# AllenNeuralDynamics/aind-exaspim-neuron-segmentation

Hardware: AMD Instinct MI355X
Metric: affinity voxels/sec on 96^3 patches over a 1024x1024x1024 volume, 1 MI355X (higher is better)
Workload: dtype fp16; 1 GPU; 1024x1024x1024 uint16 volume, 96^3 patches, overlap 32, trim 8, batch 16, fp16 (IEEE half) storage of activations and weights / fp32 accumulate (BASELINE.json configs[2]); streams=1

## Files before the change

aind_exaspim_neuron_segmentation_amd/_native.py:

```python

import ctypes
import os

_HERE = os.path.dirname(os.path.abspath(__file__))
LIB_PATH = os.path.join(_HERE, "csrc", "libexaspim_affinity.so")

DT_F32, DT_BF16, DT_F16 = 0, 1, 2
DT_BF16X3 = 3
VOX_U8, VOX_U16, VOX_I16, VOX_F32, VOX_F64 = 0, 1, 2, 3, 4
IN_F32, IN_PADDED_F32, IN_PADDED_SPLIT_F16, IN_PADDED_SPLIT_BF16 = 0, 1, 2, 3
UP_CONVT = 0x100
OPT_SEPARATE_POOL, OPT_SEPARATE_DEEP_POOLS, OPT_PLAIN_UPSAMPLE, OPT_FIRST_PER_GROUP = 1, 2, 4, 8
OPT_UPSAMPLE_PER_THREAD = 16
OPT_PER_PATCH_ENCODER = 32
OPT_SEPARATE_HEAD = 64
OPT_ROW_SEPARATE_BORDERS = 256
OPT_CARRY_MAIN_ONLY = 512
OPT_CARRY_NO_ROWS = 2048
AFF_F32, AFF_F16 = 0, 1

DTYPE_CODES = {
    "fp32": DT_F32, "float32": DT_F32, "f32": DT_F32,
    "bf16": DT_BF16, "bfloat16": DT_BF16,
    "fp16": DT_F16, "float16": DT_F16, "f16": DT_F16,
    "bf16x3": DT_BF16X3,
}


class Block(ctypes.Structure):

    _fields_ = [
        ("dims", ctypes.c_int32 * 3),
        ("origin", ctypes.c_int32 * 3),
        ("global_", ctypes.c_int32 * 3),
    ]

    @classmethod
    def make(cls, dims, origin=None, global_shape=None):
        origin = (0, 0, 0) if origin is None else origin
        global_shape = dims if global_shape is None else global_shape
        b = cls()
        b.dims[:] = [int(v) for v in dims]
        b.origin[:] = [int(v) for v in origin]
        b.global_[:] = [int(v) for v in global_shape]
        return b


class Window(ctypes.Structure):

    _fields_ = [
        ("patch", ctypes.c_int32 * 3),
        ("overlap", ctypes.c_int32 * 3),
        ("trim", ctypes.c_int32),
    ]

    @classmethod
    def make(cls, patch, overlap, trim):
        w = cls()
        w.patch[:] = [int(v) for v in patch]
        w.overlap[:] = [int(v) for v in overlap]
        w.trim = int(trim)
        return w


class ComponentsStreamDesc(ctypes.Structure):

    _fields_ = [
        ("dims", ctypes.c_int32 * 3),
        ("channels", ctypes.c_int32),
        ("threshold", ctypes.c_float),
        ("capacity", ctypes.c_int32),
        ("min_size", ctypes.c_int64),
        ("next_z", ctypes.c_int32),
        ("reserved", ctypes.c_int32),
        ("id_parent_dev", ctypes.c_void_p),
        ("id_count_dev", ctypes.c_void_p),
        ("table_dev", ctypes.c_void_p),
        ("state_dev", ctypes.c_void_p),
        ("seam_ids_dev", ctypes.c_void_p),
        ("seam_bits_dev", ctypes.c_void_p),
    ]


class RegionGraphStreamDesc(ctypes.Structure):

    _fields_ = [
        ("dims", ctypes.c_int32 * 3),
        ("id_capacity", ctypes.c_int32),
        ("edge_capacity", ctypes.c_int64),
        ("next_z", ctypes.c_int32),
        ("reserved", ctypes.c_int32),
        ("keys_dev", ctypes.c_void_p),
        ("counts_dev", ctypes.c_void_p),
        ("sums_dev", ctypes.c_void_p),
        ("sizes_by_id_dev", ctypes.c_void_p),
        ("seam_ids_dev", ctypes.c_void_p),
        ("seam_q_dev", ctypes.c_void_p),
        ("state_dev", ctypes.c_void_p),
    ]


class UNetCarry(ctypes.Structure):

    _fields_ = [
        ("own_skip", ctypes.c_void_p),
        ("own_pool", ctypes.c_void_p),
        ("in_z", ctypes.c_int32 * 2),
        ("out_skip", ctypes.c_void_p),
        ("out_pool", ctypes.c_void_p),
        ("out_z", ctypes.c_int32 * 2),
        ("out_shift", ctypes.c_int32),
        ("reserved", ctypes.c_int32),
    ]


class UNetCarry1(ctypes.Structure):

    _fields_ = [
        ("own_mid1", ctypes.c_void_p),
        ("own_skip1", ctypes.c_void_p),
        ("own_pool2", ctypes.c_void_p),
        ("in_z", ctypes.c_int32 * 2),
        ("out_mid1", ctypes.c_void_p),
        ("out_skip1", ctypes.c_void_p),
        ("out_pool2", ctypes.c_void_p),
        ("out_z", ctypes.c_int32 * 2),
        ("out_shift", ctypes.c_int32),
        ("reserved", ctypes.c_int32),
    ]


class UNetCarryY(ctypes.Structure):

    _fields_ = [
        ("in_y", ctypes.c_int32 * 2),
        ("out_skip_y", ctypes.c_void_p),
        ("out_pool_y", ctypes.c_void_p),
        ("out_skip_d", ctypes.c_void_p),
        ("out_pool_d", ctypes.c_void_p),
        ("out_y", ctypes.c_int32 * 2),
        ("out_shift_y", ctypes.c_int32),
        ("reserved", ctypes.c_int32),
        ("encoder_event", ctypes.c_void_p),
    ]


_lib = None

_I32x5 = ctypes.c_int32 * 5
_I32x3 = ctypes.c_int32 * 3
_vp = ctypes.c_void_p
_sz = ctypes.c_size_t
_i32 = ctypes.c_int32

SIGNATURES = {
    "exaspim_abi_version": (_i32, []),
    "exaspim_last_error": (ctypes.c_char_p, []),
    "exaspim_unet_param_count": (_sz, [_I32x5, _i32, _i32]),
    "exaspim_unet_packed_bytes": (_sz, [_I32x5, _i32, _i32]),
    "exaspim_unet_pack_weights": (_i32, [_I32x5, _i32, _i32, _vp, _sz, _vp, _sz]),
    "exaspim_unet_create": (_i32, [_I32x5, _i32, _i32, _i32, _vp, _sz, ctypes.POINTER(_vp)]),
    "exaspim_unet_destroy": (None, [_vp]),
    "exaspim_unet_workspace_bytes": (_sz, [_vp, _i32, _i32, _i32, _i32]),
    "exaspim_unet_forward": (_i32, [_vp, _vp, _vp, _i32, _i32, _i32, _i32, _i32, _vp, _sz, _vp]),
    "exaspim_unet_forward_trimmed": (
        _i32, [_vp, _vp, _vp, _i32, _i32, _i32, _i32, _i32, _i32, _vp, _sz, _vp]
    ),
    "exaspim_unet_input_layout": (_i32, [_vp]),
    "exaspim_unet_forward_prepared": (
        _i32, [_vp, _vp, _vp, _i32, _i32, _i32, _i32, _i32, _i32, _vp, _sz, _vp]),
    "exaspim_unet_forward_prepared_row": (
# ... 139 lines not shown
```

aind_exaspim_neuron_segmentation_amd/csrc/common.h:

```cpp
#pragma once

#include <hip/hip_runtime.h>

#include <cstdarg>
#include <cstddef>
#include <cstdint>
#include <cstdio>

#include "../../include/exaspim_affinity.h"

namespace exaspim {

void set_error(const char* fmt, ...);
const char* get_error();

#define EXA_CHECK_ARG(cond, ...)                 \
    do {                                         \
        if (!(cond)) {                           \
            ::exaspim::set_error(__VA_ARGS__);   \
            return EXASPIM_E_INVALID;            \
        }                                        \
    } while (0)

#define EXA_CHECK_HIP(expr)                                                  \
// ... 30 lines not shown
    asm volatile("s_nop 1");
    __builtin_amdgcn_sched_barrier(0);
}

__device__ __forceinline__ float sat_f16(float v) {
    return v != v ? v : __builtin_amdgcn_fmed3f(v, -65504.f, 65504.f);
}

__device__ __forceinline__ float max_nan(float a, float b) {
    return (a != a || b != b) ? __uint_as_float(0x7fc00000u) : fmaxf(a, b);
}
__device__ __forceinline__ uint4 max_nan4(const uint4& a, const uint4& b) {
    return make_uint4(__float_as_uint(max_nan(__uint_as_float(a.x), __uint_as_float(b.x))),
                      __float_as_uint(max_nan(__uint_as_float(a.y), __uint_as_float(b.y))),
                      __float_as_uint(max_nan(__uint_as_float(a.z), __uint_as_float(b.z))),
                      __float_as_uint(max_nan(__uint_as_float(a.w), __uint_as_float(b.w))));
}
typedef short s16x2 __attribute__((ext_vector_type(2)));
typedef unsigned short u16x2 __attribute__((ext_vector_type(2)));
__device__ __forceinline__ unsigned key16x2(unsigned x) {
    const s16x2 m = __builtin_bit_cast(s16x2, x) >> (short)15;
    return x ^ (__builtin_bit_cast(unsigned, m) & 0x7fff7fffu);
}
template <unsigned INF16>
__device__ __forceinline__ unsigned okey16x2(unsigned x) {
    const u16x2 mag = __builtin_bit_cast(u16x2, x & 0x7fff7fffu);
    const auto nan = mag > (u16x2){(unsigned short)INF16, (unsigned short)INF16};
    return key16x2(x & ~(__builtin_bit_cast(unsigned, nan) & 0x80008000u));
}
__device__ __forceinline__ unsigned maxkey16x2(unsigned ka, unsigned kb) {
    return __builtin_bit_cast(
        unsigned, __builtin_elementwise_max(__builtin_bit_cast(s16x2, ka), __builtin_bit_cast(s16x2, kb)));
}
__device__ __forceinline__ uint4 key16(const uint4& v) {
    return make_uint4(key16x2(v.x), key16x2(v.y), key16x2(v.z), key16x2(v.w));
}
template <unsigned INF16>
__device__ __forceinline__ uint4 okey16(const uint4& v) {
    return make_uint4(okey16x2<INF16>(v.x), okey16x2<INF16>(v.y), okey16x2<INF16>(v.z), okey16x2<INF16>(v.w));
}
__device__ __forceinline__ uint4 maxkey16(const uint4& a, const uint4& b) {
    return make_uint4(maxkey16x2(a.x, b.x), maxkey16x2(a.y, b.y), maxkey16x2(a.z, b.z), maxkey16x2(a.w, b.w));
}

template <int N>
__device__ __forceinline__ float head_dot(float acc, const float (&f)[N], const float* w) {
#pragma clang fp contract(off)
#pragma unroll
    for (int j = 0; j < N; ++j) acc = fmaf(f[j], w[j], acc);
    return acc;
}
__device__ __forceinline__ float head_activation(float r, int apply_sigmoid) {
#pragma clang fp contract(off)
    if (apply_sigmoid) r = 1.f / (1.f + expf(-r));
    return r;
}

constexpr int kChannelPad = 32;
constexpr int kNumMfmaConvs = 17;

inline int pad_channels(int c) { return (c + kChannelPad - 1) / kChannelPad * kChannelPad; }
inline size_t align_up(size_t v, size_t a) { return (v + a - 1) / a * a; }
struct MergeBound {
    uint64_t m;
    bool merge_all;
};
inline MergeBound merge_bound(float threshold) {
    const double md = __builtin_rint((1.0 - (double)threshold) * 16777216.0);
    return MergeBound{md < 0.0 ? 0 : md > 16777216.0 ? 16777216ull : (uint64_t)md, md < 0.0};
}
inline int storage_dtype(int dtype) { return dtype == EXASPIM_DT_BF16X3 ? EXASPIM_DT_F32 : dtype; }
inline int dtype_size(int dtype) { return storage_dtype(dtype) == EXASPIM_DT_F32 ? 4 : 2; }

struct ConvLayer {
    int ca_real = 0, cb_real = 0;
    int ca = 0, cb = 0;
    int cout_real = 0, cout = 0;
    size_t w_off = 0;
    size_t b_off = 0;
    size_t p_off = 0;
};

struct ConvTLayer {
    int cin_real = 0, cin = 0;
    int cout_real = 0, cout = 0;
    size_t w_off = 0;
    size_t b_off = 0;
    size_t p_off = 0;
};

struct UNetPlan {
    int channels[5] = {0, 0, 0, 0, 0};
    int out_channels = 0;
    int dtype = 0;
    bool convt = false;
    ConvTLayer up[4];
    int c0 = 0, c0p = 0;
    size_t first_p_off = 0;
    size_t first_w_off = 0;
    size_t first_b_off = 0;
    ConvLayer conv[kNumMfmaConvs];
    size_t head_p_off = 0;
    size_t head_w_off = 0;
    size_t head_b_off = 0;
    size_t packed_bytes = 0;
    size_t n_params = 0;
};

bool make_plan(const int32_t channels[5], int32_t out_channels, int32_t dtype,
               UNetPlan* plan);

int pack_weights(const UNetPlan& plan, const float* params, void* packed_host);

struct ConvArgs {
    const void* src_a;
    const void* src_b;
    int ca, cb;
    const void* weights;
    void* carry_dst = nullptr;
    void* carry_pool_dst = nullptr;
    const float* bias;
    void* dst;
    int cout;
    int n, d, h, w;
    float slope;
    const float* head_w = nullptr;
    const float* head_b = nullptr;
    float* head_out = nullptr;
    int head_oc = 0;
    int head_sigmoid = 0;
    int org[3] = {0, 0, 0};
    int ext[3] = {0, 0, 0};
    void* pool_dst = nullptr;
    int row_stride = 0;
    unsigned short in_z0 = 0, in_z1 = 0;
    float* partial = nullptr;
    size_t partial_patch_bytes = 0;
    int ksplit = 1;
    unsigned char out_z0 = 0, out_z1 = 0;
    unsigned short out_shift = 0;
#ifdef EXASPIM_TRACE
    unsigned long long* trace = nullptr;
#endif
};

struct ConvCarryY {
    void* y_dst = nullptr;
    void* y_pool_dst = nullptr;
    void* d_dst = nullptr;
    void* d_pool_dst = nullptr;
    unsigned short in_y0 = 0, in_y1 = 0;
    unsigned short out_y0 = 0, out_y1 = 0;
    unsigned short out_shift_y = 0;
};
inline bool conv_has_carry_y(const ConvCarryY& y) {
    return y.y_dst || y.y_pool_dst || y.d_dst || y.d_pool_dst || y.in_y0 || y.in_y1 || y.out_y0 || y.out_y1 || y.out_shift_y;
}

struct ConvLaunchRecord {
    const char* config = "";
    int ksplit = 0;
    bool row = false;
    bool carry_y = false;
    bool carry = false;
};
ConvLaunchRecord& last_conv_launch();
const char*& last_layer_kernel();

int launch_conv3x3x3(int dtype, const ConvArgs& a, hipStream_t stream);
int launch_conv3x3x3_thin(int dtype, const ConvArgs& a, hipStream_t stream);
int conv_zcol_main_extent(int ext, int axis);
bool conv_can_fuse_head(int cout, int w, int head_oc, int dtype = EXASPIM_DT_F32);
int launch_conv3x3x3_x3_head(const ConvArgs& a, hipStream_t stream);
bool conv_x3_can_fuse_head(int cout, int w, int head_oc);
bool conv_can_fuse_pool(int dtype, int cout, int d, int h, int w);
bool conv_row_mode_ok(int dtype, int cout, int n, int w, int row_stride, bool fused_pool_whole_patch);
constexpr int kRowStageMain = 1, kRowStageThin = 2, kRowStagePool = 4;
constexpr int kRowStagesAll = kRowStageMain | kRowStageThin | kRowStagePool;
constexpr int kRowStageBorders = 8;
constexpr int kRowStagesFused = kRowStageMain | kRowStageBorders;
constexpr int kRowStageBordersCarry = 16;
constexpr int kRowStagesCarry = kRowStageMain | kRowStageBordersCarry;
int launch_conv3x3x3_row(int dtype, const ConvArgs& a, int stages, hipStream_t stream, const ConvCarryY* y = nullptr);
int conv_zcol_tile_depth(int d);
int conv_row_borders_tile_depth(int d);
constexpr int kCarryT14TZ = 4;
int conv_carry_t14_tile_depth(int dtype, const ConvArgs& a);
void carry1_span_of_tiles(int tz, int d, int shift_z, int32_t out[2]);
#ifndef EXASPIM_TRACE
static_assert(sizeof(ConvArgs) == 184, "ConvArgs: the carry fields fill padding, the argument block keeps its size");
#endif

int launch_conv_first(int dtype, const float* x, float* xpad, const float* w, const float* bias,
                      void* dst, int n, int d, int h, int wd, int c0p, float slope,
                      hipStream_t stream, bool first_no_strips = false, int skip_z0 = 0, int skip_z1 = 0);
void conv_first_skip_planes(int d, int in_z0, int in_z1, int32_t out[2]);
int launch_convt2(int dtype, const void* src, const void* weights, const float* bias, void* dst,
                  int n, int d, int h, int w, int cin, int cout, hipStream_t stream);
int launch_maxpool2(int dtype, const void* src, void* dst, int n, int d, int h, int w,
                    int c, hipStream_t stream);
int launch_maxpool2_xcols(int dtype, const void* src, void* dst, int n, int d, int h, int w,
                          int c, int ox0, int ox1, hipStream_t stream);
int launch_upsample2(int dtype, const void* src, void* dst, int n, int d, int h, int w,
                     int c, int margin, hipStream_t stream, bool plain_kernel = false, bool per_thread = false,
                     const int* margin_hi = nullptr);
int launch_absmax(int dtype, const void* src, size_t bytes, float* out, hipStream_t stream);
int launch_head(int dtype, const void* src, const float* w, const float* bias,
                float* out, int n, int d, int h, int wd, int c0p, int out_channels,
                int apply_sigmoid, hipStream_t stream);
int launch_dbf_pass(int axis, const int32_t* labels, const int32_t* in, int32_t* out, const int32_t dims[3],
                    int black_border, hipStream_t stream);
constexpr int kFillHolesPasses = 6;
int launch_fill_holes_passes(const int32_t* labels, const int32_t dims[3], int32_t* out, int64_t* counts,
                             void* workspace, int first, int last, hipStream_t stream);

}
```

aind_exaspim_neuron_segmentation_amd/csrc/conv3d.hip:

```cpp

#include <cstdlib>

#include "common.h"
#include "conv_device.h"
#include "conv_t14.h"
#include "conv_x3.h"
#include "conv_zcol.h"

namespace exaspim {

#ifdef EXASPIM_TRACE
int g_variant = 0;
#endif

ConvLaunchRecord& last_conv_launch() {
    static thread_local ConvLaunchRecord rec;
    return rec;
}

static int resident_workgroups(int per_cu) {
    static int cus = 0;
    if (cus == 0) {
        int dev = 0, n = 0;
        if (hipGetDevice(&dev) != hipSuccess ||
            hipDeviceGetAttribute(&n, hipDeviceAttributeMultiprocessorCount, dev) != hipSuccess || n <= 0)
            n = 256;
        cus = n;
    }
    return cus * per_cu;
}

static inline int cdiv(int a, int b) { return (a + b - 1) / b; }

struct TileGrid {
    int tz, ty, tx;
    long long blocks;
};
static int tile_grid(const ConvArgs& a, int TZ, int TY, int TX, int ex, int n, TileGrid& g) {
    g.tz = cdiv(a.ext[0], TZ), g.ty = cdiv(a.ext[1], TY), g.tx = cdiv(ex, TX);
    g.blocks = (long long)g.tz * g.ty * g.tx * n;
    if (g.blocks <= 0 || g.blocks > 0x7fffffffLL) {
        set_error("conv: grid of %lld blocks out of range", g.blocks);
        return EXASPIM_E_INVALID;
    }
    return EXASPIM_OK;
}

static int choose_ksplit(const ConvArgs& a, const TileGrid& g, int slices, int units) {
    const bool whole = a.ext[0] == a.d && a.ext[1] == a.h && a.ext[2] == a.w;
    constexpr int kNominalBatch = 16;
    const long long wgs = (long long)g.tz * g.ty * g.tx * kNominalBatch * slices;
    if (!a.partial || !whole || wgs * 2 > resident_workgroups(2)) return 1;
    int ks = (int)(resident_workgroups(2) / wgs);
    if (ks > 4) ks = 4;
    if (ks > units) ks = units;
    const size_t patch_vox = (size_t)a.d * a.h * a.w;
    while (ks > 1 && (size_t)ks * patch_vox * a.cout * sizeof(float) > a.partial_patch_bytes) --ks;
    return ks;
}

static bool conv_has_carry(const ConvArgs& a) {
    return a.carry_dst || a.carry_pool_dst || a.in_z0 || a.in_z1 || a.out_z0 || a.out_z1;
}

template <typename Tag, int TZ, int TY, int TX, int MINW, int D, int HEAD = 0, bool POOL = false>
static int launch_zpipe(const ConvArgs& a, hipStream_t stream) {
    const bool row = POOL && HEAD == 0 && Tag::kG == 8 && a.row_stride > 0;
    TileGrid g;
    if (int rc = row ? tile_grid(a, TZ, TY, TX, a.n * a.row_stride + a.w - a.row_stride, 1, g)
                     : tile_grid(a, TZ, TY, TX, a.ext[2], a.n, g))
        return rc;
    const bool carry = row && conv_has_carry(a);
    if (carry) {
        g.tz -= (a.in_z1 - a.in_z0) / TZ;
        g.blocks = (long long)g.tz * g.ty * g.tx;
    }
    const int tz = g.tz, ty = g.ty, tx = g.tx;
    const long long blocks = g.blocks;
    const int slices = a.cout / 32;
    long long wgs = resident_workgroups(MINW) / slices / 8 * 8;
    if (wgs < 8) wgs = 8;
    if (wgs > blocks) wgs = blocks;
#ifdef EXASPIM_TRACE
    if (g_variant >= 10 && g_variant < 20) wgs = blocks;
    if (const char* e = getenv("EXASPIM_TRACE_WGS_PER_CU")) wgs = resident_workgroups(1) * (long long)atoi(e) / slices / 8 * 8;
#endif
    dim3 grid((unsigned)wgs, slices);
    last_conv_launch() = {__PRETTY_FUNCTION__, 1};
    if constexpr (POOL && HEAD == 0 && Tag::kG == 8) {
        if (carry) {
            last_conv_launch().carry = true;
            conv3x3x3_zpipe_rowz<Tag, TZ, TY, TX, MINW, D><<<grid, TY * TX * 2, 0, stream>>>(a, tz, ty, tx);
            EXA_CHECK_HIP(hipGetLastError());
            return EXASPIM_OK;
        }
        if (row) {
            last_conv_launch().row = true;
            conv3x3x3_zpipe_row<Tag, TZ, TY, TX, MINW, D><<<grid, TY * TX * 2, 0, stream>>>(a, tz, ty, tx);
            EXA_CHECK_HIP(hipGetLastError());
            return EXASPIM_OK;
        }
    }
    conv3x3x3_zpipe<Tag, TZ, TY, TX, MINW, D, HEAD, POOL><<<grid, TY * TX * 2, 0, stream>>>(a, tz, ty, tx);
    EXA_CHECK_HIP(hipGetLastError());
    return EXASPIM_OK;
}

template <typename Tag, int TZ>
static int launch_zpipe_rowzy(const ConvArgs& a, const ConvCarryY& y, hipStream_t stream) {
    constexpr int TY = 8, TX = 16, MINW = 2, D = 4;
    TileGrid g;
    if (int rc = tile_grid(a, TZ, TY, TX, a.n * a.row_stride + a.w - a.row_stride, 1, g)) return rc;
    g.tz -= (a.in_z1 - a.in_z0) / TZ;
    g.ty -= (y.in_y1 - y.in_y0) / TY;
    g.blocks = (long long)g.tz * g.ty * g.tx;
    const int slices = a.cout / 32;
    long long wgs = resident_workgroups(MINW) / slices / 8 * 8;
    if (wgs < 8) wgs = 8;
    if (wgs > g.blocks) wgs = g.blocks;
    dim3 grid((unsigned)wgs, slices);
    last_conv_launch() = {__PRETTY_FUNCTION__, 1};
    last_conv_launch().carry = true;
    last_conv_launch().carry_y = true;
    conv3x3x3_zpipe_rowzy<Tag, TZ, TY, TX, MINW, D><<<grid, TY * TX * 2, 0, stream>>>(a, y, g.tz, g.ty, g.tx);
    EXA_CHECK_HIP(hipGetLastError());
    return EXASPIM_OK;
}


template <typename Tag, int TZ, int TY, int TX, int WAVES_M, int WAVES_N, int MT, int NT, int MINW, int PD = 3,
          bool ZORD = false, bool POOL = false>
static int launch_cfg(const ConvArgs& a, hipStream_t stream) {
    constexpr int NWG = WAVES_N * NT * 32;
    if (a.cout % NWG != 0) {
        set_error("conv: cout %d not a multiple of the %d-channel tile", a.cout, NWG);
        return EXASPIM_E_INVALID;
    }
    TileGrid g;
    if (int rc = tile_grid(a, TZ, TY, TX, a.ext[2], a.n, g)) return rc;
    ConvArgs b = a;
    b.ksplit = a.head_out ? 1 : choose_ksplit(a, g, a.cout / NWG, (a.ca + a.cb) / (2 * Tag::kG));
    constexpr bool kCarryCfg = Tag::kG == 8 && TZ == kCarryT14TZ && TY == 8 && TX == 16 && WAVES_M == 4 && WAVES_N == 1 &&
                               MT == 4 && NT == 2 && MINW == 2 && PD == 3 && !ZORD;
    const bool carry = conv_has_carry(a);
    if (carry) {
        EXA_CHECK_ARG(kCarryCfg && b.ksplit == 1, "conv: this launch has no carried planes (tile configuration%s)",
                      b.ksplit > 1 ? ", split-K" : "");
        g.tz -= (a.in_z1 - a.in_z0) / TZ;
        g.blocks = (long long)g.tz * g.ty * g.tx * a.n;
    }
    const int tz = g.tz, ty = g.ty, tx = g.tx;
    const size_t nvox_all = (size_t)a.n * a.d * a.h * a.w;
    dim3 grid((unsigned)g.blocks, a.cout / NWG, b.ksplit);
    last_conv_launch() = {__PRETTY_FUNCTION__, b.ksplit};
    if constexpr (kCarryCfg) {
        if (carry) {
            last_conv_launch().carry = true;
            conv3x3x3_t14_carry<Tag, TZ, TY, TX, WAVES_M, WAVES_N, MT, NT, MINW, PD, POOL>
                <<<grid, WAVES_M * WAVES_N * 64, 0, stream>>>(b, tz, ty, tx);
            EXA_CHECK_HIP(hipGetLastError());
            return EXASPIM_OK;
        }
    }
    if (POOL && b.ksplit > 1) {
        b.pool_dst = nullptr;
        conv3x3x3_t14<Tag, TZ, TY, TX, WAVES_M, WAVES_N, MT, NT, MINW, PD, ZORD, false>
            <<<grid, WAVES_M * WAVES_N * 64, 0, stream>>>(b, tz, ty, tx);
    } else {
        conv3x3x3_t14<Tag, TZ, TY, TX, WAVES_M, WAVES_N, MT, NT, MINW, PD, ZORD, POOL>
            <<<grid, WAVES_M * WAVES_N * 64, 0, stream>>>(b, tz, ty, tx);
    }
    EXA_CHECK_HIP(hipGetLastError());
    if (b.ksplit > 1) {
        const size_t items = nvox_all * (a.cout / 4);
        splitk_reduce_kernel<Tag><<<(unsigned)((items + 255) / 256), 256, 0, stream>>>(
            a.partial, a.bias, a.dst, nvox_all, (size_t)a.d * a.h * a.w, a.cout, b.ksplit, a.slope);
        EXA_CHECK_HIP(hipGetLastError());
        if (POOL)
            return launch_maxpool2(Tag::kCode, a.dst, a.pool_dst, a.n, a.d, a.h, a.w, a.cout, stream);
    }
    return EXASPIM_OK;
}

template <typename Tag> struct ES_of { static constexpr int value = 16 / Tag::kG; };

template <typename Tag, int TZ, int TY, int TX, int WAVES_M, int WAVES_N, int MT, int NT, int MINW>
static int launch_cfg_pool(const ConvArgs& a, hipStream_t stream) {
    if constexpr (ES_of<Tag>::value == 2) {
        if (a.pool_dst)
            return launch_cfg<Tag, TZ, TY, TX, WAVES_M, WAVES_N, MT, NT, MINW, 3, false, true>(a, stream);
    }
    return launch_cfg<Tag, TZ, TY, TX, WAVES_M, WAVES_N, MT, NT, MINW>(a, stream);
}

template <typename Tag, int TZ, int D>
static int launch_zpipe_head(const ConvArgs& a, hipStream_t stream) {
    if (a.head_out && a.cout == 32) {
        switch (a.head_oc) {
            case 1: return launch_zpipe<Tag, TZ, 8, 16, 2, D, 1>(a, stream);
            case 2: return launch_zpipe<Tag, TZ, 8, 16, 2, D, 2>(a, stream);
            case 3: return launch_zpipe<Tag, TZ, 8, 16, 2, D, 3>(a, stream);
            case 4: return launch_zpipe<Tag, TZ, 8, 16, 2, D, 4>(a, stream);
        }
    }
    if (a.pool_dst) return launch_zpipe<Tag, TZ, 8, 16, 2, D, 0, true>(a, stream);
    return launch_zpipe<Tag, TZ, 8, 16, 2, D>(a, stream);
}

template <typename Tag, int TZ>
static int launch_zpipe_d(const ConvArgs& a, hipStream_t stream) {
#ifdef EXASPIM_TRACE
    if (g_variant % 10 == 3) return launch_zpipe_head<Tag, TZ, 3>(a, stream);
    if (g_variant % 10 == 5) return launch_zpipe_head<Tag, TZ, 5>(a, stream);
#endif
    return launch_zpipe_head<Tag, TZ, 4>(a, stream);
}

template <typename Tag>
static int launch_typed(const ConvArgs& a, hipStream_t stream) {
    if (a.w >= 16 && a.w % 16 == 0) {
#ifdef EXASPIM_TRACE
        if (g_variant >= 20) return launch_zpipe_d<Tag, 6>(a, stream);
#endif
        if (a.cout % 64 != 0) {
            if (a.head_out && a.cout == 32 && a.ext[0] % 6 != 0 && a.ext[0] % kHeadTZ == 0) {
                switch (a.head_oc) {
                    case 1: return launch_zpipe<Tag, kHeadTZ, 8, 16, 2, 4, 1>(a, stream);
                    case 2: return launch_zpipe<Tag, kHeadTZ, 8, 16, 2, 4, 2>(a, stream);
                    case 3: return launch_zpipe<Tag, kHeadTZ, 8, 16, 2, 4, 3>(a, stream);
                    case 4: return launch_zpipe<Tag, kHeadTZ, 8, 16, 2, 4, 4>(a, stream);
                }
            }
            if (conv_zcol_tile_depth(a.d) == 6) return launch_zpipe_d<Tag, 6>(a, stream);
            return launch_zpipe_d<Tag, 4>(a, stream);
        }
        if (a.pool_dst) return launch_cfg_pool<Tag, 4, 8, 16, 4, 1, 4, 2, 2>(a, stream);
        return launch_cfg<Tag, 4, 8, 16, 4, 1, 4, 2, 2>(a, stream);
    }
    if (a.w > 12) {
        if (a.cout % 64 == 0) return launch_cfg_pool<Tag, 4, 4, 24, 4, 1, 3, 2, 2>(a, stream);
        return launch_cfg_pool<Tag, 4, 4, 24, 4, 1, 3, 1, 2>(a, stream);
    }
    if (a.w > 6) {
        if (a.cout % 256 == 0) return launch_cfg_pool<Tag, 4, 4, 12, 2, 1, 3, 1, 2>(a, stream);
        if (a.cout % 128 == 0) return launch_cfg_pool<Tag, 4, 4, 12, 2, 2, 3, 2, 2>(a, stream);
        if (a.cout % 64 == 0) return launch_cfg_pool<Tag, 4, 4, 12, 2, 2, 3, 1, 2>(a, stream);
        return launch_cfg_pool<Tag, 4, 4, 12, 2, 1, 3, 1, 2>(a, stream);
    }
    return launch_cfg<Tag, 6, 6, 6, 4, 1, 2, 1, 2>(a, stream);
}

template <int TZ, int TY, int TX, int WAVES_M, int WAVES_N, int MT, int NT, int MINW, int PD>
static int launch_x3(const ConvArgs& a, hipStream_t stream) {
    constexpr int NWG = WAVES_N * NT * 32;
    if (a.cout % NWG != 0) {
        set_error("conv: cout %d not a multiple of the %d-channel tile", a.cout, NWG);
        return EXASPIM_E_INVALID;
    }
    TileGrid g;
    if (int rc = tile_grid(a, TZ, TY, TX, a.ext[2], a.n, g)) return rc;
    const int tz = g.tz, ty = g.ty, tx = g.tx;
    ConvArgs b = a;
    b.ksplit = choose_ksplit(a, g, a.cout / NWG, (a.ca + a.cb) / 16);
    const size_t patch_vox_all = (size_t)a.d * a.h * a.w;
    const size_t nvox_all = (size_t)a.n * patch_vox_all;
    dim3 grid((unsigned)g.blocks, a.cout / NWG, b.ksplit);
    last_conv_launch() = {__PRETTY_FUNCTION__, b.ksplit};
    conv3x3x3_x3<TZ, TY, TX, WAVES_M, WAVES_N, MT, NT, MINW, PD>
        <<<grid, WAVES_M * WAVES_N * 64, 0, stream>>>(b, tz, ty, tx);
    EXA_CHECK_HIP(hipGetLastError());
    if (b.ksplit > 1) {
        const size_t items = nvox_all * (a.cout / 4);
        splitk_reduce_kernel<F32Tag><<<(unsigned)((items + 255) / 256), 256, 0, stream>>>(
            a.partial, a.bias, a.dst, nvox_all, patch_vox_all, a.cout, b.ksplit, a.slope);
        EXA_CHECK_HIP(hipGetLastError());
    }
    return EXASPIM_OK;
}

static int launch_typed_x3(const ConvArgs& a, hipStream_t stream) {
    if (a.w >= 16 && a.w % 16 == 0) {
        if (a.cout % 64 == 0) return launch_x3<2, 8, 16, 4, 1, 2, 2, 2, 3>(a, stream);
        return launch_x3<4, 8, 16, 4, 1, 4, 1, 2, 3>(a, stream);
    }
    if (a.w > 12) {
        if (a.cout % 64 == 0) return launch_x3<4, 4, 24, 4, 1, 3, 2, 2, 1>(a, stream);
        return launch_x3<4, 4, 24, 4, 1, 3, 1, 2, 3>(a, stream);
    }
    if (a.w > 6) {
        if (a.cout % 256 == 0) return launch_x3<4, 4, 12, 2, 1, 3, 1, 2, 3>(a, stream);
        if (a.cout % 128 == 0) return launch_x3<4, 4, 12, 2, 2, 3, 2, 2, 2>(a, stream);
        if (a.cout % 64 == 0) return launch_x3<4, 4, 12, 2, 2, 3, 1, 2, 3>(a, stream);
        return launch_x3<4, 4, 12, 2, 1, 3, 1, 2, 3>(a, stream);
    }
    return launch_x3<6, 6, 6, 4, 1, 2, 1, 2, 3>(a, stream);
}

static int launch_thin_typed_x3(const ConvArgs& a, hipStream_t stream) {
    if (a.ext[1] <= a.ext[2]) return launch_x3<8, 2, 16, 4, 1, 2, 1, 2, 3>(a, stream);
    return launch_x3<8, 16, 2, 4, 1, 2, 1, 2, 3>(a, stream);
}

template <int HEAD>
static int launch_x3_head(const ConvArgs& a, hipStream_t stream) {
    TileGrid g;
    if (int rc = tile_grid(a, kX3HeadTZ, kX3HeadTY, kX3HeadTX, a.ext[2], a.n, g)) return rc;
    last_conv_launch() = {__PRETTY_FUNCTION__, 1};
    conv3x3x3_x3_head<HEAD><<<dim3((unsigned)g.blocks, 1, 1), 256, 0, stream>>>(a, g.tz, g.ty, g.tx);
    EXA_CHECK_HIP(hipGetLastError());
    return EXASPIM_OK;
}

bool conv_can_fuse_pool(int dtype, int cout, int d, int h, int w) {
    if (d % 2 != 0 || h % 2 != 0 || w % 2 != 0) return false;
    if (dtype == EXASPIM_DT_BF16X3) return false;
    if (cout % 64 != 0 && w >= 16 && w % 16 == 0) return true;
    return dtype != EXASPIM_DT_F32 && w > 6;
}

static bool head_shape_ok(int cout, int w, int head_oc) {
    return cout == 32 && w >= 16 && w % 16 == 0 && head_oc >= 1 && head_oc <= 4;
}
bool conv_can_fuse_head(int cout, int w, int head_oc, int dtype) {
    return dtype != EXASPIM_DT_BF16X3 && head_shape_ok(cout, w, head_oc);
}
bool conv_x3_can_fuse_head(int cout, int w, int head_oc) { return head_shape_ok(cout, w, head_oc); }

static int resolve_region(ConvArgs& a) {
    const int dims[3] = {a.d, a.h, a.w};
    for (int i = 0; i < 3; ++i) {
        if (a.ext[i] == 0 && a.org[i] == 0) a.ext[i] = dims[i];
        EXA_CHECK_ARG(a.org[i] >= 0 && a.ext[i] > 0 && a.org[i] + a.ext[i] <= dims[i],
                      "conv: region [%d, %d) outside axis %d of a %dx%dx%d patch", a.org[i],
                      a.org[i] + a.ext[i], i, a.d, a.h, a.w);
    }
    return EXASPIM_OK;
}

int conv_zcol_tile_depth(int d) { return d % 6 == 0 ? 6 : 4; }

int conv_carry_t14_tile_depth(int dtype, const ConvArgs& a) {
    if (dtype_size(dtype) != 2 || dtype == EXASPIM_DT_BF16X3 || a.head_out || a.row_stride != 0) return 0;
    if (!(a.w >= 16 && a.w % 16 == 0 && a.cout % 64 == 0 && a.d % kCarryT14TZ == 0)) return 0;
    ConvArgs b = a;
    for (int i = 0; i < 3; ++i) b.org[i] = b.ext[i] = 0;
    if (resolve_region(b) != EXASPIM_OK) return 0;
    TileGrid g;
    if (tile_grid(b, kCarryT14TZ, 8, 16, b.ext[2], b.n, g) != EXASPIM_OK) return 0;
    return choose_ksplit(b, g, b.cout / 64, (b.ca + b.cb) / 16) == 1 ? kCarryT14TZ : 0;
}

int conv_zcol_main_extent(int ext, int axis) {
    const int tile = axis == 1 ? 8 : 16;
    const int rem = ext % tile;
    return (axis != 0 && ext > tile && rem >= 1 && rem <= 4) ? ext - rem : ext;
}

bool conv_row_mode_ok(int dtype, int cout, int n, int w, int row_stride, bool fused_pool_whole_patch) {
    const int o = w - row_stride;
    return dtype_size(dtype) == 2 && fused_pool_whole_patch && cout % 64 != 0 &&
           w % 16 == 0 && n >= 2 && row_stride > 0 && o > 0 && o % 32 == 0 && row_stride >= o;
}

static int check_row_args(int dtype, const ConvArgs& a) {
    const bool whole = a.ext[0] == a.d && a.ext[1] == a.h && a.ext[2] == a.w;
    EXA_CHECK_ARG(conv_row_mode_ok(dtype, a.cout, a.n, a.w, a.row_stride,
                                   a.pool_dst && !a.head_out && whole &&
                                       conv_can_fuse_pool(dtype, a.cout, a.d, a.h, a.w)),
                  "conv: row mode needs a 16-bit fused-pool z-column layer, whole patches, n >= 2 and "
                  "an overlap that is a multiple of 32 and at most the stride (w %d, stride %d, n %d)",
                  a.w, a.row_stride, a.n);
    const int tzd = conv_zcol_tile_depth(a.d);
    EXA_CHECK_ARG(a.in_z0 <= a.in_z1 && a.in_z0 % 2 == 0 && a.in_z1 % 2 == 0 && a.in_z0 % tzd == 0 && a.in_z1 % tzd == 0 &&
                      (a.in_z0 == a.in_z1 || (a.in_z0 >= 2 && a.in_z1 <= a.d - 2)),
                  "conv: carry in [%d, %d) must be whole %d-plane tiles with even bounds inside [2, %d)", (int)a.in_z0,
                  (int)a.in_z1, tzd, a.d - 2);
    const bool out = a.carry_dst || a.carry_pool_dst || a.out_z0 || a.out_z1;
    EXA_CHECK_ARG(!out || (a.carry_dst && a.carry_pool_dst && a.out_z0 < a.out_z1 && a.out_z0 % 2 == 0 && a.out_z1 % 2 == 0 &&
                           a.out_z0 >= 2 && a.out_z1 <= a.d - 2 && a.out_shift > 0 && a.out_shift % 2 == 0 &&
                           (int)a.out_z0 - a.out_shift >= 2),
                  "conv: carry out [%d, %d) shifted by %d needs both targets, even bounds and source and target planes "
                  "inside [2, %d)", (int)a.out_z0, (int)a.out_z1, a.out_shift, a.d - 2);
    return EXASPIM_OK;
}

static int check_row_y_args(const ConvArgs& a, const ConvCarryY& y) {
    constexpr int TY = 8;
    EXA_CHECK_ARG(y.in_y0 <= y.in_y1 && y.in_y0 % TY == 0 && y.in_y1 % TY == 0 &&
                      (y.in_y0 == y.in_y1 || (y.in_y0 >= 2 && y.in_y1 <= a.h - 2)),
                  "conv: y carry in [%d, %d) must be whole %d-row tiles inside [2, %d)", (int)y.in_y0, (int)y.in_y1, TY,
                  a.h - 2);
    const bool out = y.y_dst || y.y_pool_dst || y.d_dst || y.d_pool_dst || y.out_y0 || y.out_y1 || y.out_shift_y;
    EXA_CHECK_ARG(!out || (y.y_dst && y.y_pool_dst && y.out_y0 < y.out_y1 && y.out_y0 % 2 == 0 && y.out_y1 % 2 == 0 &&
                           y.out_y0 >= 2 && y.out_y1 <= a.h - 2 && y.out_shift_y > 0 && y.out_shift_y % 2 == 0 &&
                           (int)y.out_y0 - y.out_shift_y >= 2),
                  "conv: y carry out [%d, %d) shifted by %d needs both targets, even bounds and source and target rows "
                  "inside [2, %d)", (int)y.out_y0, (int)y.out_y1, (int)y.out_shift_y, a.h - 2);
    EXA_CHECK_ARG(!out || y.in_y0 == y.in_y1 || y.out_y0 >= y.in_y1 || y.out_y1 <= y.in_y0,
                  "conv: y carry out [%d, %d) overlaps the rows carried in, [%d, %d)", (int)y.out_y0, (int)y.out_y1,
                  (int)y.in_y0, (int)y.in_y1);
    EXA_CHECK_ARG(!y.d_dst == !y.d_pool_dst && (!y.d_dst || (out && a.carry_dst)),
                  "conv: the diagonal carry out needs both targets and both the z and the y carry out");
    EXA_CHECK_ARG(!y.d_dst || a.in_z0 == a.in_z1 || a.out_z0 >= a.in_z1 || a.out_z1 <= a.in_z0,
                  "conv: carry out [%d, %d) overlaps the planes carried in, [%d, %d)", (int)a.out_z0, (int)a.out_z1,
                  (int)a.in_z0, (int)a.in_z1);
    return EXASPIM_OK;
}

static int check_carry_args(int dtype, const ConvArgs& a, bool whole) {
    const int tzd = conv_carry_t14_tile_depth(dtype, a);
    EXA_CHECK_ARG(tzd > 0 && whole,
                  "conv: carried planes need row mode or a whole-patch 16-bit 64-cout-slice layer on 16-wide rows "
                  "that is not split (%dx%dx%d, cout %d)", a.d, a.h, a.w, a.cout);
    EXA_CHECK_ARG(a.in_z0 <= a.in_z1 && a.in_z0 % 2 == 0 && a.in_z1 % 2 == 0 && a.in_z0 % tzd == 0 && a.in_z1 % tzd == 0 &&
                      (a.in_z0 == a.in_z1 || (a.in_z0 >= 2 && a.in_z1 <= a.d - 2)),
                  "conv: carry in [%d, %d) must be whole %d-plane tiles with even bounds inside [2, %d)", (int)a.in_z0,
                  (int)a.in_z1, tzd, a.d - 2);
    const bool out = a.carry_dst || a.carry_pool_dst || a.out_z0 || a.out_z1;
    EXA_CHECK_ARG(!out || (a.carry_dst && !a.carry_pool_dst == !a.pool_dst && a.out_z0 < a.out_z1 && a.out_z0 % 2 == 0 &&
                           a.out_z1 % 2 == 0 && a.out_z0 >= 2 && a.out_z1 <= a.d - 2 && a.out_shift > 0 &&
                           a.out_shift % 2 == 0 && (int)a.out_z0 - a.out_shift >= 2),
                  "conv: carry out [%d, %d) shifted by %d needs a target (a pooled one exactly with a fused max-pool), "
                  "even bounds and source and target planes inside [2, %d)", (int)a.out_z0, (int)a.out_z1, a.out_shift,
                  a.d - 2);
    return EXASPIM_OK;
}

enum : unsigned { kCheckPadded = 1, kCheckEmpty = 2, kCheckSlope = 4, kCheckPatchBytes = 8, kCheckAll = 15 };
static int check_conv_args(int dtype, const ConvArgs& a, unsigned checks) {
    const int kc = dtype == EXASPIM_DT_F32 ? 8 : 16;
    EXA_CHECK_ARG(!(checks & kCheckPadded) || (a.ca % kc == 0 && a.cb % kc == 0 && a.cout % 32 == 0 && a.ca > 0),
                  "conv: channels (%d,%d)->%d not padded", a.ca, a.cb, a.cout);
    EXA_CHECK_ARG(!(checks & kCheckEmpty) || (a.n > 0 && a.d > 0 && a.h > 0 && a.w > 0), "conv: empty input");
    EXA_CHECK_ARG(!(checks & kCheckSlope) || (a.slope >= 0.f && a.slope <= 1.f),
                  "conv: LeakyReLU slope %g outside [0, 1]", a.slope);
    const unsigned long long rec = (unsigned long long)a.d * a.h * a.w * (a.ca > a.cb ? a.ca : a.cb) * dtype_size(dtype);
    EXA_CHECK_ARG(!(checks & kCheckPatchBytes) || rec < 0x80000000ULL,
                  "conv: one patch of one source is %llu bytes (>= 2 GiB)", rec);
    return EXASPIM_OK;
}

int launch_conv3x3x3(int dtype, const ConvArgs& a_in, hipStream_t stream) {
    ConvArgs a = a_in;
    if (int rc = check_conv_args(dtype, a, kCheckAll)) return rc;
    if (int rc = resolve_region(a)) return rc;
    const bool whole = a.ext[0] == a.d && a.ext[1] == a.h && a.ext[2] == a.w;
    EXA_CHECK_ARG(!a.pool_dst || (conv_can_fuse_pool(dtype, a.cout, a.d, a.h, a.w) && !a.head_out && whole),
                  "conv: fused max-pool needs an even, untrimmed patch (16-bit modes: wider than 6 voxels; "
                  "float32: a 32-cout-slice layer)");
    EXA_CHECK_ARG(!a.head_out || conv_can_fuse_head(a.cout, a.w, a.head_oc, dtype),
                  "conv: fused head needs cout 32, w %% 16 == 0, 1..4 outputs (and not bf16x3)");
    if (a.row_stride > 0) {
        if (int rc = check_row_args(dtype, a)) return rc;
    } else if (conv_has_carry(a)) {
        if (int rc = check_carry_args(dtype, a, whole)) return rc;
    }
    switch (dtype) {
        case EXASPIM_DT_F32: return launch_typed<F32Tag>(a, stream);
        case EXASPIM_DT_BF16: return launch_typed<BF16Tag>(a, stream);
        case EXASPIM_DT_F16: return launch_typed<F16Tag>(a, stream);
        case EXASPIM_DT_BF16X3: return launch_typed_x3(a, stream);
    }
    set_error("conv: unknown dtype %d", dtype);
    return EXASPIM_E_INVALID;
}

int launch_conv3x3x3_x3_head(const ConvArgs& a_in, hipStream_t stream) {
    ConvArgs a = a_in;
    if (int rc = check_conv_args(EXASPIM_DT_BF16X3, a, kCheckAll)) return rc;
    EXA_CHECK_ARG(conv_x3_can_fuse_head(a.cout, a.w, a.head_oc),
                  "conv: bf16x3 fused head needs cout 32, w %% 16 == 0 and 1..4 outputs (cout %d, w %d, %d outputs)",
                  a.cout, a.w, a.head_oc);
    EXA_CHECK_ARG(a.head_out && a.head_w && a.head_b, "conv: bf16x3 fused head: NULL head pointer");
    EXA_CHECK_ARG(!a.pool_dst && a.row_stride == 0, "conv: bf16x3 fused head has no fused max-pool or row mode");
    if (int rc = resolve_region(a)) return rc;
    a.partial = nullptr;
    a.ksplit = 1;
    switch (a.head_oc) {
        case 1: return launch_x3_head<1>(a, stream);
        case 2: return launch_x3_head<2>(a, stream);
        case 3: return launch_x3_head<3>(a, stream);
        default: return launch_x3_head<4>(a, stream);
    }
}

template <typename Tag>
static int launch_thin_typed(const ConvArgs& a, hipStream_t stream) {
    const int ez = a.ext[0];
    auto planes = [&](int tz) { return (ez + tz - 1) / tz * tz; };
    if (a.ext[1] <= a.ext[2]) {
        const float c4 = planes(4) * 1.00f, c8 = planes(8) * 0.76f, c12 = planes(12) * 0.66f;
        if (c12 <= c8 && c12 <= c4) return launch_cfg<Tag, 12, 2, 16, 4, 1, 3, 1, 3, 3, true>(a, stream);
        if (c8 <= c4) return launch_cfg<Tag, 8, 2, 16, 4, 1, 2, 1, 4, 3, true>(a, stream);
        return launch_cfg<Tag, 4, 2, 16, 4, 1, 1, 1, 4, 3, true>(a, stream);
    }
    if (planes(8) * 0.78f <= planes(4) * 1.00f) return launch_cfg<Tag, 8, 16, 2, 4, 1, 2, 1, 4, 3, true>(a, stream);
    return launch_cfg<Tag, 4, 16, 2, 4, 1, 1, 1, 4, 3, true>(a, stream);
}

int launch_conv3x3x3_thin(int dtype, const ConvArgs& a_in, hipStream_t stream) {
    ConvArgs a = a_in;
    if (int rc = check_conv_args(dtype, a, kCheckPadded | kCheckEmpty)) return rc;
    EXA_CHECK_ARG(!a.pool_dst && !a.head_out && a.row_stride == 0 && !conv_has_carry(a),
                  "conv: thin tiles have no fused pool, head, row mode or carried planes");
    if (int rc = resolve_region(a)) return rc;
    a.partial = nullptr;
    switch (dtype) {
        case EXASPIM_DT_F32: return launch_thin_typed<F32Tag>(a, stream);
        case EXASPIM_DT_BF16: return launch_thin_typed<BF16Tag>(a, stream);
        case EXASPIM_DT_F16: return launch_thin_typed<F16Tag>(a, stream);
        case EXASPIM_DT_BF16X3: return launch_thin_typed_x3(a, stream);
    }
    set_error("conv: unknown dtype %d", dtype);
    return EXASPIM_E_INVALID;
}

template <typename Tag, int TZ, int MT>
static int launch_row_borders_cfg(const ConvArgs& a, hipStream_t stream) {
    const int tz = cdiv(a.d, TZ), ty = cdiv(a.h, 16);
    const long long blocks = (long long)tz * ty * 2 * (a.n - 1);
    if (blocks <= 0 || blocks > 0x7fffffffLL) {
        set_error("conv: grid of %lld blocks out of range", blocks);
        return EXASPIM_E_INVALID;
    }
    last_conv_launch() = {__PRETTY_FUNCTION__, 1};
    conv3x3x3_t14<Tag, TZ, 16, 2, 4, 1, MT, 1, 4, 3, true, true>
        <<<dim3((unsigned)blocks, a.cout / 32, 1), 256, 0, stream>>>(a, tz, ty, 2);
    EXA_CHECK_HIP(hipGetLastError());
    return EXASPIM_OK;
}

int conv_row_borders_tile_depth(int d) {
    auto planes = [&](int tz) { return (d + tz - 1) / tz * tz; };
    return planes(8) * 0.78f <= planes(4) * 1.00f ? 8 : 4;
}

template <typename Tag, int TZ, int MT>
static int launch_row_borders_carry_cfg(const ConvArgs& a, hipStream_t stream) {
    const int tz = cdiv(a.in_z0, TZ) + cdiv(a.d - a.in_z1, TZ), ty = cdiv(a.h, 16);
    const long long blocks = (long long)tz * ty * 2 * (a.n - 1);
    if (blocks <= 0 || blocks > 0x7fffffffLL) {
        set_error("conv: grid of %lld blocks out of range", blocks);
        return EXASPIM_E_INVALID;
    }
    last_conv_launch() = {__PRETTY_FUNCTION__, 1};
    last_conv_launch().carry = true;
    conv3x3x3_t14_borders_carry<Tag, TZ, MT>
        <<<dim3((unsigned)blocks, a.cout / 32, 1), 256, 0, stream>>>(a, tz, ty, 2);
    EXA_CHECK_HIP(hipGetLastError());
    return EXASPIM_OK;
}

template <typename Tag>
static int launch_row_borders(const ConvArgs& a_in, hipStream_t stream) {
    ConvArgs a = a_in;
    a.partial = nullptr;
    a.ksplit = 1;
    a.row_stride = 0;
    const bool deep = conv_row_borders_tile_depth(a.d) == 8;
    if (conv_has_carry(a))
        return deep ? launch_row_borders_carry_cfg<Tag, 8, 2>(a, stream) : launch_row_borders_carry_cfg<Tag, 4, 1>(a, stream);
    if (deep) return launch_row_borders_cfg<Tag, 8, 2>(a, stream);
    return launch_row_borders_cfg<Tag, 4, 1>(a, stream);
}

int launch_conv3x3x3_row(int dtype, const ConvArgs& a, int stages, hipStream_t stream, const ConvCarryY* y) {
    ConvArgs b = a;
    if (int rc = check_conv_args(dtype, a, kCheckEmpty)) return rc;
    if (int rc = resolve_region(b)) return rc;
    if (int rc = check_row_args(dtype, b)) return rc;
    const bool carry_y = y && conv_has_carry_y(*y);
    if (carry_y) {
        if (int rc = check_row_y_args(b, *y)) return rc;
    }
    EXA_CHECK_ARG(!(stages & kRowStageBordersCarry) || a.in_z0 == a.in_z1 || a.out_z0 == a.out_z1 ||
                      a.out_z0 >= a.in_z1 || a.out_z1 <= a.in_z0,
                  "conv: carry out [%d, %d) overlaps the planes carried in, [%d, %d)", (int)a.out_z0, (int)a.out_z1,
                  (int)a.in_z0, (int)a.in_z1);
    int r = EXASPIM_OK;
    if ((stages & kRowStageMain) && carry_y) {
        r = check_conv_args(dtype, a, kCheckAll);
        const bool six = conv_zcol_tile_depth(a.d) == 6;
        if (r == EXASPIM_OK)
            r = dtype == EXASPIM_DT_F16 ? (six ? launch_zpipe_rowzy<F16Tag, 6>(b, *y, stream) : launch_zpipe_rowzy<F16Tag, 4>(b, *y, stream))
                                        : (six ? launch_zpipe_rowzy<BF16Tag, 6>(b, *y, stream) : launch_zpipe_rowzy<BF16Tag, 4>(b, *y, stream));
    } else if (stages & kRowStageMain) {
        r = launch_conv3x3x3(dtype, a, stream);
    }
    b.pool_dst = nullptr;
    b.row_stride = 0;
    b.carry_dst = b.carry_pool_dst = nullptr;
    b.in_z0 = b.in_z1 = b.out_z0 = b.out_z1 = 0;
    b.out_shift = 0;
    b.n = a.n - 1;
    b.ext[2] = 2;
    if (r == EXASPIM_OK && (stages & kRowStageThin)) {
        const size_t vox = (size_t)a.d * a.h * a.w;
        b.src_a = static_cast<const char*>(a.src_a) + vox * a.ca * dtype_size(dtype);
        b.dst = static_cast<char*>(a.dst) + vox * a.cout * dtype_size(dtype);
        r = launch_conv3x3x3_thin(dtype, b, stream);
        if (r == EXASPIM_OK) {
            b.org[2] = a.w - 2;
            b.src_a = a.src_a;
            b.dst = a.dst;
            r = launch_conv3x3x3_thin(dtype, b, stream);
        }
    }
    if (r == EXASPIM_OK && (stages & kRowStagePool))
        r = launch_maxpool2_xcols(dtype, a.dst, a.pool_dst, a.n, a.d, a.h, a.w, a.cout, 0, a.w / 2 - 1, stream);
    if (r == EXASPIM_OK && (stages & kRowStageBorders)) {
        r = check_conv_args(dtype, a, kCheckPadded);
        ConvArgs c = a;
        for (int i = 0; i < 3; ++i) { c.org[i] = b.org[i]; c.ext[i] = b.ext[i]; }
        c.carry_dst = c.carry_pool_dst = nullptr;
        c.in_z0 = c.in_z1 = c.out_z0 = c.out_z1 = 0;
        c.out_shift = 0;
        c.org[2] = 0;
        if (r == EXASPIM_OK)
            r = dtype == EXASPIM_DT_F16 ? launch_row_borders<F16Tag>(c, stream) : launch_row_borders<BF16Tag>(c, stream);
    }
    if (r == EXASPIM_OK && (stages & kRowStageBordersCarry)) {
        r = check_conv_args(dtype, a, kCheckPadded);
        ConvArgs c = a;
        for (int i = 0; i < 3; ++i) { c.org[i] = b.org[i]; c.ext[i] = b.ext[i]; }
        c.org[2] = 0;
        if (r == EXASPIM_OK)
            r = dtype == EXASPIM_DT_F16 ? launch_row_borders<F16Tag>(c, stream) : launch_row_borders<BF16Tag>(c, stream);
    }
    return r;
}

}
```

aind_exaspim_neuron_segmentation_amd/csrc/conv_t14.h:

```cpp
#pragma once

#include "conv_device.h"

namespace exaspim {

template <typename Tag, int TZ, int TY, int TX, int WAVES_M, int WAVES_N, int MT, int NT, int MINW, int PD,
          bool ZORD = false, bool POOL = false>
__global__ __launch_bounds__(WAVES_M* WAVES_N * 64, MINW) void conv3x3x3_t14(
    ConvArgs a, int tiles_z, int tiles_y, int tiles_x) {
    constexpr bool CARRY = false;
#include "conv_t14_body.inc"
}

template <typename Tag, int TZ, int TY, int TX, int WAVES_M, int WAVES_N, int MT, int NT, int MINW, int PD, bool POOL>
__global__ __launch_bounds__(WAVES_M* WAVES_N * 64, MINW) void conv3x3x3_t14_carry(
    ConvArgs a, int tiles_z, int tiles_y, int tiles_x) {
    constexpr bool ZORD = false, CARRY = true;
#include "conv_t14_body.inc"
}

template <typename Tag, int TZ, int MT>
__global__ __launch_bounds__(256, 4) void conv3x3x3_t14_borders_carry(
    ConvArgs a, int tiles_z, int tiles_y, int tiles_x) {
    constexpr int TY = 16, TX = 2, WAVES_M = 4, WAVES_N = 1, NT = 1, PD = 3;
    constexpr bool ZORD = true, POOL = true, CARRY = true;
#include "conv_t14_body.inc"
}

template <typename Tag>
__global__ __launch_bounds__(256) void splitk_reduce_kernel(const float* __restrict__ partial,
                                                            const float* __restrict__ bias,
                                                            void* __restrict__ dst, size_t nvox_all,
                                                            size_t patch_vox, int cout, int ksplit,
                                                            float slope) {
    constexpr int ES = 16 / Tag::kG;
    constexpr int KC = 2 * Tag::kG;
    const size_t i = (size_t)blockIdx.x * blockDim.x + threadIdx.x;
    const int quads = cout >> 2;
    if (i >= nvox_all * quads) return;
    const size_t v = i / quads;
    const int c = (int)(i - v * quads) * 4;
    float4 s = *reinterpret_cast<const float4*>(bias + c);
    for (int k = 0; k < ksplit; ++k) {
        const float4 p = *reinterpret_cast<const float4*>(partial + ((size_t)k * nvox_all + v) * cout + c);
        s.x += p.x; s.y += p.y; s.z += p.z; s.w += p.w;
    }
    const size_t nb = v / patch_vox, vox = v - nb * patch_vox;
    char* out = static_cast<char*>(dst) + (((size_t)nb * (cout / KC) + c / KC) * patch_vox + vox) * 32 +
                (c % KC) * ES;
    store4<Tag>(out, 0, leaky(s.x, slope), leaky(s.y, slope), leaky(s.z, slope), leaky(s.w, slope));
}

}
```

aind_exaspim_neuron_segmentation_amd/csrc/conv_t14_body.inc:

```
    constexpr int G = Tag::kG;
    constexpr int KC = 2 * G;
    constexpr int ES = 16 / G;
    constexpr int HZ = TZ + 2, HY = TY + 2, HX = TX + 2;
    constexpr int HXS = TX == 24 ? 40 : HX;
    constexpr int PLS = HY * HXS;
    constexpr int HV = HZ * PLS;
    constexpr int HVD = HZ * HY * HX;
    constexpr int NWAVES = WAVES_M * WAVES_N;
    constexpr int NTHREADS = NWAVES * 64;
    constexpr int TILE_VOX = TZ * TY * TX;
    constexpr int NITEMS = (2 * HVD + NTHREADS - 1) / NTHREADS;
    constexpr int RECB = NT * 32 * ES;
    constexpr int RECP = RECB + 16;
    constexpr int EPI_UNITS = NWAVES * (POOL ? MT : 1) * 32 * RECP / 16;
    constexpr int IMG = 2 * HV;
    constexpr int LDS_UNITS = IMG > EPI_UNITS ? IMG : EPI_UNITS;
    static_assert(!POOL || (WAVES_M * MT * 32 == TZ * TY * TX && TZ % 2 == 0 && TY % 2 == 0 && TX % 2 == 0),
                  "pooled tile shape");
    constexpr int ISSUE_T = 26 - PD > 0 ? 26 - PD : 0;
    static_assert(WAVES_M * MT * 32 >= TILE_VOX, "tile not covered by the waves");

    __shared__ __attribute__((aligned(16))) uint4 lds[LDS_UNITS];

    const int tid = threadIdx.x;
    const int lane = tid & 63;
    const int wave = __builtin_amdgcn_readfirstlane(tid >> 6);
    const int wm = wave / WAVES_N;
    const int wn = wave % WAVES_N;
    const int half = lane >> 5;
    const int r = (TX == 16 && (lane & 16)) ? 16 + (((lane & 15) - HX) & 15) : (lane & 31);

    int bid;
    {
        const int nblk = gridDim.x, q = nblk >> 3, rem = nblk & 7;
        const int xcd = blockIdx.x & 7, slot = blockIdx.x >> 3;
        bid = (xcd < rem ? xcd * (q + 1) : rem * (q + 1) + (xcd - rem) * q) + slot;
    }
    const int tx = bid % tiles_x; bid /= tiles_x;
    const int ty = bid % tiles_y; bid /= tiles_y;
    int tz = bid % tiles_z; bid /= tiles_z;
    constexpr bool BORDERS = ZORD && POOL;
    constexpr bool BCARRY = CARRY && BORDERS;
    if (CARRY && !BORDERS && tz >= a.in_z0 / TZ) tz += (a.in_z1 - a.in_z0) / TZ;
    static_assert(!CARRY || (ES == 2 && (!ZORD || BORDERS)), "carry: 16-bit types, whole-patch or border tiles");
    const int nb = BORDERS && tx == 0 ? bid + 1 : bid;
    const int seg0 = BCARRY ? (a.in_z0 + TZ - 1) / TZ : 0;
    const bool low = BCARRY && tz < seg0;
    const int z0 = BCARRY && !low ? a.in_z1 + (tz - seg0) * TZ : a.org[0] + tz * TZ, y0 = a.org[1] + ty * TY;
    const int x0 = BORDERS ? (tx == 0 ? 0 : a.w - TX) : a.org[2] + tx * TX;
    const int zend = low ? (int)a.in_z0 : a.org[0] + a.ext[0], yend = a.org[1] + a.ext[1];
    const int xend = BORDERS ? x0 + TX : a.org[2] + a.ext[2];

    const int ntiles = a.cout >> 5;
    const int ntile0 = (blockIdx.y * WAVES_N + wn) * NT;

    int base[MT];
#pragma unroll
    for (int mt = 0; mt < MT; ++mt) {
        int m = (wm * MT + mt) * 32 + r;
        m = m < TILE_VOX ? m : TILE_VOX - 1;
        const int z = m / (TY * TX), y = (m / TX) % TY, x = m % TX;
        base[mt] = z * PLS + y * HXS + x + half * HV;
    }

    const size_t patch_vox = (size_t)a.d * a.h * a.w;
    unsigned voffs[NITEMS];
#pragma unroll
    for (int it = 0; it < NITEMS; ++it) {
        const int i = tid + it * NTHREADS;
        const int hv = i >> 1;
        const int hz = hv / (HY * HX), hy = (hv / HX) % HY, hx = hv % HX;
        const int gz = z0 + hz - 1, gy = y0 + hy - 1, gx = x0 + hx - 1;
        const bool ok = i < 2 * HVD && (unsigned)gz < (unsigned)a.d &&
                        (unsigned)gy < (unsigned)a.h && (unsigned)gx < (unsigned)a.w;
        voffs[it] = ok ? (unsigned)((gz * a.h + gy) * a.w + gx) * 32u + (i & 1) * 16u : kOutOfRange;
    }

    f32x16 acc[MT][NT];
#pragma unroll
    for (int nt = 0; nt < NT; ++nt)
#pragma unroll
        for (int q = 0; q < 4; ++q) {
            float4 b = *reinterpret_cast<const float4*>(a.bias + (ntile0 + nt) * 32 + 8 * q + 4 * half);
            if (a.ksplit > 1) b = make_float4(0.f, 0.f, 0.f, 0.f);
#pragma unroll
            for (int mt = 0; mt < MT; ++mt) {
                acc[mt][nt][4 * q + 0] = b.x; acc[mt][nt][4 * q + 1] = b.y;
                acc[mt][nt][4 * q + 2] = b.z; acc[mt][nt][4 * q + 3] = b.w;
            }
        }

    const int nchunks_all = (a.ca + a.cb) / KC;
    const int cbeg = (int)blockIdx.z * nchunks_all / a.ksplit;
    const int nchunks = ((int)blockIdx.z + 1) * nchunks_all / a.ksplit;
    uint4 stg[NITEMS];

    auto stage_load = [&](int c) {
        const char* src;
        int cs, ch0;
        if (c * KC < a.ca) {
            src = static_cast<const char*>(a.src_a); cs = a.ca; ch0 = c * KC;
        } else {
            src = static_cast<const char*>(a.src_b); cs = a.cb; ch0 = c * KC - a.ca;
        }
        const size_t patchb = patch_vox * cs * ES;
        const __amdgpu_buffer_rsrc_t rsrc = make_rsrc(src + (size_t)nb * patchb, patchb);
        const unsigned cbase = (unsigned)(ch0 / KC) * (unsigned)patch_vox * 32u;
#pragma unroll
        for (int it = 0; it < NITEMS; ++it) stg[it] = buf_load16(rsrc, voffs[it], cbase);
    };
    auto stage_store = [&]() {
#pragma unroll
        for (int it = 0; it < NITEMS; ++it) {
            const int i = tid + it * NTHREADS;
            const int hv = i >> 1;
            if (i < 2 * HVD) lds[(i & 1) * HV + (hv / (HY * HX)) * PLS + ((hv / HX) % HY) * HXS + hv % HX] = stg[it];
        }
    };

#ifdef EXASPIM_TRACE
    const size_t trace_rec = ((size_t)blockIdx.x * NWAVES + wave) * 16;
    if (a.trace && lane == 0)
        a.trace[trace_rec + 15] = ((unsigned long long)__builtin_amdgcn_s_getreg((31 << 11) | 20) << 32) |
                                  (unsigned)__builtin_amdgcn_s_getreg((31 << 11) | 4);
#endif
    constexpr auto tap_of = [](int t) { return ZORD ? (t % 3) * 9 + t / 3 : t; };
    uint4 wring[PD + 1][NT];
    auto prime_weights = [&](int c) {
        const uint4* wp = static_cast<const uint4*>(a.weights) + ((size_t)c * 27 * ntiles + ntile0) * 64 + lane;
#pragma unroll
        for (int t = 0; t < PD; ++t)
#pragma unroll
            for (int nt = 0; nt < NT; ++nt) wring[t][nt] = wp[((size_t)tap_of(t) * ntiles + nt) * 64];
    };
    EXA_TRACE(0);
    stage_load(cbeg);
    prime_weights(cbeg);
    EXA_TRACE(1);
    stage_store();
    __syncthreads();
    EXA_TRACE(2);

    for (int c = cbeg; c < nchunks; ++c) {
        const uint4* wp = static_cast<const uint4*>(a.weights) +
                          ((size_t)c * 27 * ntiles + ntile0) * 64 + lane;

        uint4 xf[2][MT];
        {
            constexpr int t0 = tap_of(0);
            constexpr int tapoff0 = (t0 / 9) * PLS + ((t0 / 3) % 3) * HXS + t0 % 3;
#pragma unroll
            for (int mt = 0; mt < MT; ++mt) xf[0][mt] = lds[base[mt] + tapoff0];
        }

        const bool more = c + 1 < nchunks;
        if (ES == 2) __builtin_amdgcn_s_setprio(kSetprioT14);
#pragma unroll
        for (int t = 0; t < 27; ++t) {
            if (t + PD < 27) {
#pragma unroll
                for (int nt = 0; nt < NT; ++nt)
                    wring[(t + PD) % (PD + 1)][nt] = wp[((size_t)tap_of(t + PD) * ntiles + nt) * 64];
            }
            if (t == ISSUE_T && more) stage_load(c + 1);
#ifdef EXASPIM_TRACE
            if (nchunks_all == 2 && c == cbeg && t > 0 && t % 7 == 0 && t / 7 <= 3) EXA_TRACE(8 + t / 7);
#endif
            if (t + 1 < 27) {
                const int tn = tap_of(t + 1);
                const int tapoff = (tn / 9) * PLS + ((tn / 3) % 3) * HXS + tn % 3;
#pragma unroll
                for (int mt = 0; mt < MT; ++mt) xf[(t + 1) & 1][mt] = lds[base[mt] + tapoff];
            }
#pragma unroll
            for (int mt = 0; mt < MT; ++mt)
#pragma unroll
                for (int nt = 0; nt < NT; ++nt)
                    mma<Tag>(acc[mt][nt], wring[t % (PD + 1)][nt], xf[t & 1][mt]);
            __builtin_amdgcn_sched_barrier(0);
        }
        if (ES == 2) __builtin_amdgcn_s_setprio(0);
        if (more) prime_weights(c + 1);
        if (c - cbeg < 4) EXA_TRACE(3 + 3 * (c - cbeg));
        __syncthreads();
        if (c - cbeg < 4) EXA_TRACE(4 + 3 * (c - cbeg));
        if (more) {
            stage_store();
            __syncthreads();
            if (c - cbeg < 3) EXA_TRACE(5 + 3 * (c - cbeg));
        }
    }

    if (a.ksplit > 1) {
        float* const part = a.partial + ((size_t)blockIdx.z * a.n + nb) * patch_vox * a.cout;
#pragma unroll
        for (int mt = 0; mt < MT; ++mt) {
            const int m = (wm * MT + mt) * 32 + r;
            const int z = m / (TY * TX), y = (m / TX) % TY, x = m % TX;
            const int gz = z0 + z, gy = y0 + y, gx = x0 + x;
            if (m < TILE_VOX && gz < zend && gy < yend && gx < xend) {
                float* rec = part + (((size_t)gz * a.h + gy) * a.w + gx) * a.cout;
#pragma unroll
                for (int nt = 0; nt < NT; ++nt)
#pragma unroll
                    for (int q = 0; q < 4; ++q)
                        *reinterpret_cast<float4*>(rec + (ntile0 + nt) * 32 + 8 * q + 4 * half) =
                            make_float4(acc[mt][nt][4 * q], acc[mt][nt][4 * q + 1], acc[mt][nt][4 * q + 2],
                                        acc[mt][nt][4 * q + 3]);
            }
        }
        EXA_TRACE(14);
        return;
    }

    const bool cz_on = CARRY && a.carry_dst != nullptr;
    char* wl = reinterpret_cast<char*>(lds) + wave * ((POOL ? MT : 1) * 32 * RECP);
    if (POOL) {
#pragma unroll
        for (int mt = 0; mt < MT; ++mt)
#pragma unroll
            for (int nt = 0; nt < NT; ++nt)
#pragma unroll
                for (int q = 0; q < 4; ++q) {
                    const int cl = nt * 32 + 8 * q + 4 * half;
                    store4<Tag>(wl + mt * (32 * RECP), (size_t)(r * RECP) / ES + cl,
                                leaky(acc[mt][nt][4 * q + 0], a.slope), leaky(acc[mt][nt][4 * q + 1], a.slope),
                                leaky(acc[mt][nt][4 * q + 2], a.slope), leaky(acc[mt][nt][4 * q + 3], a.slope));
                }
        __syncthreads();
        constexpr int NPL = RECB / 32;
        {
            const int vv = lane >> 1, sub = lane & 1;
            char* const dplane = static_cast<char*>(a.dst) +
                                 ((size_t)nb * (a.cout / KC) + ntile0 * (32 / KC)) * patch_vox * 32;
            char* const cplane = static_cast<char*>(a.carry_dst) - (size_t)a.out_shift * a.h * a.w * 32 +
                                 ((size_t)nb * (a.cout / KC) + ntile0 * (32 / KC)) * patch_vox * 32;
#pragma unroll
            for (int mt = 0; mt < MT; ++mt) {
                const int m = (wm * MT + mt) * 32 + vv;
                const int z = m / (TY * TX), y = (m / TX) % TY, x = m % TX;
                const int gz = z0 + z, gy = y0 + y, gx = x0 + x;
                const bool ok = gz < zend && gy < yend && gx < xend;
                const size_t vox = ((size_t)gz * a.h + gy) * a.w + gx;
#pragma unroll
                for (int ck = 0; ck < NPL; ++ck) {
                    const uint4 val = *reinterpret_cast<const uint4*>(
                        wl + mt * (32 * RECP) + vv * RECP + (ck * 2 + sub) * 16);
                    if (ok)
                        *reinterpret_cast<uint4*>(dplane + ((size_t)ck * patch_vox + vox) * 32 + sub * 16) = val;
                    if (CARRY && ok && cz_on && gz >= a.out_z0 && gz < a.out_z1)
                        *reinterpret_cast<uint4*>(cplane + ((size_t)ck * patch_vox + vox) * 32 + sub * 16) = val;
                }
            }
        }
        constexpr int PX = TX / 2, PY = TY / 2, PZ = TZ / 2;
        constexpr int NPIECE = 2 * PX * PY * PZ * NPL * WAVES_N;
        const int pd = a.d >> 1, ph = a.h >> 1, pw2 = a.w >> 1;
        const size_t pvox = (size_t)pd * ph * pw2;
        const char* const lb = reinterpret_cast<const char*>(lds);
#pragma unroll
// ... 104 lines not shown
```

aind_exaspim_neuron_segmentation_amd/csrc/conv_zcol.h:

```cpp
#pragma once

#include "conv_device.h"

namespace exaspim {

template <typename Tag, int TZ, int TY, int TX, int MINW, int D, int HEAD, bool POOL, bool ROW, bool CARRY = false,
          bool CARRYY = false>
__device__ __forceinline__ void zpipe_body(const ConvArgs& a, int tiles_z, int tiles_y, int tiles_x,
                                           const ConvCarryY& cy = ConvCarryY{}) {
    constexpr int G = Tag::kG;
    constexpr int KC = 2 * G;
    constexpr int ES = 16 / G;
    constexpr int HZ = TZ + 2, HY = TY + 2, HX = TX + 2;
    constexpr int HXP = HX;
    constexpr int PLANE = HY * HXP;
    constexpr int HVP = HZ * PLANE;
    constexpr int GS = HVP + (24 - HVP % 16) % 16;
    constexpr int NWAVES = TY * TX / 32;
    constexpr int NTHREADS = NWAVES * 64;
    constexpr int NPAIR = 2 * HY * HX;
    constexpr int REM = NPAIR > NTHREADS ? NPAIR - NTHREADS : 0;
    constexpr int SEC = (REM * HZ + NTHREADS - 1) / NTHREADS;
    constexpr int NITEMS = HZ + SEC;
    constexpr int RECB = 32 * ES;
    constexpr int RECP = RECB + 16;
    constexpr int EPI_UNITS = NWAVES * 32 * RECP / 16;
    constexpr int WUNITS = 27 * 64;
    constexpr int WITEMS = (WUNITS + NTHREADS - 1) / NTHREADS;
    constexpr int XUNITS = 2 * GS > EPI_UNITS ? 2 * GS : EPI_UNITS;
    constexpr int LDS_UNITS = XUNITS + WUNITS;
    constexpr int NS = 9 * HZ;
    constexpr int R = D + 1;
    constexpr int kLoadStride = 2;
    constexpr int LOAD_STRIDE = kLoadStride * (NITEMS + WITEMS) <= NS ? kLoadStride : 1;
    static_assert(TY * TX % 32 == 0 && NPAIR <= 2 * NTHREADS, "tile shape");
    static_assert(LOAD_STRIDE * (NITEMS + WITEMS) <= NS, "the staged pieces fit into the steps");

    __shared__ __attribute__((aligned(16))) uint4 lds[LDS_UNITS];

    const int tid = threadIdx.x;
    const int lane = tid & 63;
    const int wave = __builtin_amdgcn_readfirstlane(tid >> 6);
    const int half = lane >> 5;
    const int r = (TX == 16 && (lane & 16)) ? 16 + (((lane & 15) - HXP) & 15) : (lane & 31);

    constexpr bool row = ROW;
    static_assert(!ROW || (POOL && ES == 2 && HEAD == 0), "row mode: 16-bit fused-pool epilogue");
    static_assert(!CARRY || ROW, "carry: row mode only");
    static_assert(!CARRYY || (CARRY && TY % 2 == 0 && TX == 16), "y carry: on top of the z carry, a wave owns a row pair");
    const int total = tiles_z * tiles_y * tiles_x * (row ? 1 : a.n);
    int t_first, t_count, t_step;
    {
        const int q = total >> 3, rem = total & 7;
        const int xcd = blockIdx.x & 7, slot = blockIdx.x >> 3;
        t_first = (xcd < rem ? xcd * (q + 1) : rem * (q + 1) + (xcd - rem) * q) + slot;
        t_count = q + (xcd < rem ? 1 : 0) - slot;
        t_step = (gridDim.x + 7 - xcd) >> 3;
    }
    if (t_count <= 0) return;
    const int ntiles = a.cout >> 5;
    const int ntile0 = blockIdx.y;

    struct Tile {
        int z0, y0, x0, nb;
    };
    auto row_tile_at = [&](int id) {
        Tile t;
        const int s = a.row_stride, ho = (a.w - s) >> 1;
        const int rx = (id % tiles_x) * TX; id /= tiles_x;
        const int nb = min(max(rx - ho, 0) / s, a.n - 1);
        t.x0 = __builtin_amdgcn_readfirstlane(rx - nb * s);
        if constexpr (CARRYY) {
            int ty = id % tiles_y; id /= tiles_y;
            if (ty >= cy.in_y0 / TY) ty += (cy.in_y1 - cy.in_y0) / TY;
            t.y0 = __builtin_amdgcn_readfirstlane(ty * TY);
        } else {
            t.y0 = __builtin_amdgcn_readfirstlane((id % tiles_y) * TY); id /= tiles_y;
        }
        int tz = id % tiles_z;
        if (CARRY && tz >= a.in_z0 / TZ) tz += (a.in_z1 - a.in_z0) / TZ;
        t.z0 = __builtin_amdgcn_readfirstlane(tz * TZ);
        t.nb = __builtin_amdgcn_readfirstlane(nb);
        return t;
    };
    auto tile_at = [&](int id) {
        if (row) return row_tile_at(id);
        Tile t;
        t.x0 = __builtin_amdgcn_readfirstlane(a.org[2] + (id % tiles_x) * TX); id /= tiles_x;
        t.y0 = __builtin_amdgcn_readfirstlane(a.org[1] + (id % tiles_y) * TY); id /= tiles_y;
        t.z0 = __builtin_amdgcn_readfirstlane(a.org[0] + (id % tiles_z) * TZ); id /= tiles_z;
        id = __builtin_amdgcn_readfirstlane(id);
        t.nb = id;
        return t;
    };

    const int pos = wave * 32 + r;
    const int col = (pos / TX) * HXP + (pos % TX) + half * GS;

    const int plane_vox = a.h * a.w;
    const size_t patch_vox = (size_t)a.d * plane_vox;
    const bool p_ok = tid < NPAIR;
    const int p_hy = (tid >> 1) / HX, p_hx = (tid >> 1) % HX, p_kg = tid & 1;
    const int p_slot = p_kg * GS + p_hy * HXP + p_hx;
    unsigned p_voff;
    unsigned s_voff[SEC > 0 ? SEC : 1];
    int s_slot[SEC > 0 ? SEC : 1];
#pragma unroll
    for (int k = 0; k < SEC; ++k) {
        const int q = tid + k * NTHREADS;
        const int pr = NTHREADS + q % REM, hz = q / REM;
        const int c = pr >> 1, kg = pr & 1;
        s_slot[k] = q < REM * HZ ? kg * GS + hz * PLANE + (c / HX) * HXP + c % HX : -1;
    }
    auto set_offsets = [&](const Tile& t) {
        if constexpr (CARRY) {
            const int ft = wave * 64 + fresh_lane();
            const int gy = t.y0 + (ft >> 1) / HX - 1, gx = t.x0 + (ft >> 1) % HX - 1;
            const bool in = ft < NPAIR && (unsigned)gy < (unsigned)a.h && (unsigned)gx < (unsigned)a.w;
            p_voff = in ? (unsigned)(gy * a.w + gx) * 32u + (ft & 1) * 16u : kOutOfRange;
        } else {
            const int gy = t.y0 + p_hy - 1, gx = t.x0 + p_hx - 1;
            const bool in = p_ok && (unsigned)gy < (unsigned)a.h && (unsigned)gx < (unsigned)a.w;
            p_voff = in ? (unsigned)(gy * a.w + gx) * 32u + p_kg * 16u : kOutOfRange;
        }
#pragma unroll
        for (int k = 0; k < SEC; ++k) {
            const int q = tid + k * NTHREADS;
            const int pr = NTHREADS + q % REM, hz = q / REM;
            const int c = pr >> 1, kg = pr & 1;
            const int gz = t.z0 + hz - 1, gy = t.y0 + c / HX - 1, gx = t.x0 + c % HX - 1;
            const bool in = q < REM * HZ && (unsigned)gz < (unsigned)a.d &&
                            (unsigned)gy < (unsigned)a.h && (unsigned)gx < (unsigned)a.w;
            s_voff[k] = in ? (unsigned)((gz * a.h + gy) * a.w + gx) * 32u + kg * 16u : kOutOfRange;
        }
    };
    const unsigned wvoff = (((tid >> 6) * ntiles) * 64 + (tid & 63)) * 16u;

    __shared__ __attribute__((aligned(16))) float bias_s[32];
    if (tid < 32) bias_s[tid] = a.bias[ntile0 * 32 + tid];
    __shared__ __attribute__((aligned(16))) float head_s[HEAD > 0 ? HEAD * 32 + 4 : 4];
    if (HEAD > 0) {
        if (tid < HEAD * 32) head_s[tid] = a.head_w[tid];
        if (tid < HEAD) head_s[HEAD * 32 + tid] = a.head_b[tid];
    }

    const int nchunks = (a.ca + a.cb) / KC;
    uint4 stg[NITEMS + WITEMS];
    uint4* const wlds = lds + XUNITS;
    const __amdgpu_buffer_rsrc_t wrsrc = make_rsrc(a.weights, (size_t)nchunks * 27 * ntiles * 1024);

    struct ChunkSrc {
        __amdgpu_buffer_rsrc_t rsrc;
        __amdgpu_buffer_rsrc_t none;
        unsigned cbase;
    };
    auto chunk_src = [&](int c, int nb) {
        const char* src;
        int cs, ch0;
        if (c * KC < a.ca) {
            src = static_cast<const char*>(a.src_a); cs = a.ca; ch0 = c * KC;
        } else {
            src = static_cast<const char*>(a.src_b); cs = a.cb; ch0 = c * KC - a.ca;
        }
        const size_t patchb = patch_vox * cs * ES;
        return ChunkSrc{make_rsrc(src + (size_t)nb * patchb, patchb), make_rsrc(src + (size_t)nb * patchb, 0),
                        (unsigned)(ch0 / KC) * (unsigned)patch_vox * 32u};
    };
    auto load_piece = [&](const ChunkSrc& cs, int c, int z0, int i) {
        if (i < NITEMS) {
            if (i < HZ) {
                const int gz = z0 + i - 1;
                stg[i] = (unsigned)gz < (unsigned)a.d
                             ? buf_load16(cs.rsrc, p_voff, cs.cbase + (unsigned)gz * plane_vox * 32u)
                             : buf_load16(cs.none, p_voff, 0);
            } else {
                stg[i] = buf_load16(cs.rsrc, s_voff[i - HZ], cs.cbase);
            }
        } else {
            const int it = i - NITEMS;
            stg[i] = it * NWAVES + wave < 27
                         ? buf_load16(wrsrc, wvoff, ((c * 27 + it * NWAVES) * ntiles + ntile0) * 1024)
                         : make_uint4(0, 0, 0, 0);
        }
    };
    auto stage_store = [&]() {
        if ((EXASPIM_ABLATE & 4) && stg[0].x != 0x12345u) return;
        if (p_ok) {
#pragma unroll
            for (int hz = 0; hz < HZ; ++hz) lds[p_slot + hz * PLANE] = stg[hz];
        }
#pragma unroll
        for (int k = 0; k < SEC; ++k)
            if (s_slot[k] >= 0) lds[s_slot[k]] = stg[HZ + k];
#pragma unroll
        for (int it = 0; it < WITEMS; ++it) {
            const int i = tid + it * NTHREADS;
            if (i < WUNITS) wlds[i] = stg[NITEMS + it];
        }
    };

    int tile_id = t_first;
    Tile cur = tile_at(tile_id);
    set_offsets(cur);
    {
        const ChunkSrc cs0 = chunk_src(0, cur.nb);
#pragma unroll
        for (int i = 0; i < NITEMS + WITEMS; ++i) load_piece(cs0, 0, cur.z0, i);
    }
    stage_store();

    for (;;) {
#ifdef EXASPIM_TRACE
        const size_t trace_rec = ((size_t)tile_id * NWAVES + wave) * 16;
        if (a.trace && lane == 0)
            a.trace[trace_rec + 15] =
                ((unsigned long long)__builtin_amdgcn_s_getreg((31 << 11) | 20) << 32) |
                (unsigned)__builtin_amdgcn_s_getreg((31 << 11) | 4);
#endif
        EXA_TRACE(0);
        EXA_TRACE(1);
        __syncthreads();
        f32x16 acc[TZ];
        const int half_t = fresh_lane() >> 5;
#pragma unroll
        for (int q = 0; q < 4; ++q) {
            const float4 b = *reinterpret_cast<const float4*>(bias_s + 8 * q + 4 * half_t);
#pragma unroll
            for (int mt = 0; mt < TZ; ++mt) {
                acc[mt][4 * q + 0] = b.x; acc[mt][4 * q + 1] = b.y;
                acc[mt][4 * q + 2] = b.z; acc[mt][4 * q + 3] = b.w;
            }
        }
        EXA_TRACE(2);

        t_count -= t_step;
        const bool has_next = t_count > 0;
        Tile nxt = cur;
        for (int c = 0; c < nchunks; ++c) {
            const bool more = c + 1 < nchunks;
            const bool pre = more || has_next;
            if (!more && has_next) {
                nxt = tile_at(tile_id + t_step);
                set_offsets(nxt);
            }
            const ChunkSrc csn = chunk_src(more ? c + 1 : 0, more ? cur.nb : nxt.nb);
            const int cn = more ? c + 1 : 0, zn = more ? cur.z0 : nxt.z0;
            uint4 xr[R];
            uint4 wb[3];
#pragma unroll
            for (int dz = 0; dz < 3; ++dz) wb[dz] = wlds[(dz * 9) * 64 + lane];
#pragma unroll
            for (int s = 0; s < D; ++s)
                xr[s % R] = lds[col + (s % HZ) * PLANE + ((s / HZ) / 3) * HXP + (s / HZ) % 3];
            __builtin_amdgcn_sched_barrier(0);
            if (ES == 2) __builtin_amdgcn_s_setprio(kSetprio);
#pragma unroll
            for (int s = 0; s < NS; ++s) {
                const int g = s / HZ, zin = s % HZ;
                if (s + D < NS) {
                    const int g2 = (s + D) / HZ, z2 = (s + D) % HZ;
                    xr[(s + D) % R] = lds[col + z2 * PLANE + (g2 / 3) * HXP + g2 % 3];
                }
#ifdef EXASPIM_TRACE
                if (nchunks == 2 && c == 0 && s > 0 && s % (NS / 4) == 0 && s / (NS / 4) <= 3) EXA_TRACE(8 + s / (NS / 4));
#endif
                if (g + 1 < 9 && zin >= TZ) wb[zin - TZ] = wlds[((zin - TZ) * 9 + g + 1) * 64 + lane];
                if (g > 0 && zin == 0) wb[2] = wlds[(2 * 9 + g) * 64 + lane];
                if (!(EXASPIM_ABLATE & 1) && pre && s % LOAD_STRIDE == 0 && s / LOAD_STRIDE < NITEMS + WITEMS)
                    load_piece(csn, cn, zn, s / LOAD_STRIDE);
#pragma unroll
                for (int dz = 0; dz < 3; ++dz) {
                    const int z = zin - dz;
                    if (z >= 0 && z < TZ) mma_inplace<Tag>(acc[z], wb[dz], xr[s % R]);
                }
                __builtin_amdgcn_sched_barrier(0);
            }
            if (ES == 2) __builtin_amdgcn_s_setprio(0);
            if (ES == 2) asm volatile("s_nop 7\n\ts_nop 7\n\ts_nop 1");
            if (c < 4) EXA_TRACE(3 + 3 * c);
            __syncthreads();
            if (c < 4) EXA_TRACE(4 + 3 * c);
            if (more) {
                stage_store();
                __syncthreads();
                if (c < 3) EXA_TRACE(5 + 3 * c);
            }
        }
        if (has_next) {
#pragma unroll
            for (int i = 0; i < NITEMS + WITEMS; ++i)
                asm volatile("" : "+v"(stg[i].x), "+v"(stg[i].y), "+v"(stg[i].z), "+v"(stg[i].w));
        }

        const int lane_e = fresh_lane();
        const int half_e = lane_e >> 5;
        const int r_e = (TX == 16 && (lane_e & 16)) ? 16 + (((lane_e & 15) - HXP) & 15) : (lane_e & 31);
        const int pos_e = wave * 32 + r_e;
        if (HEAD > 0) {
            float part[TZ][HEAD > 0 ? HEAD : 1];
#pragma unroll
            for (int z = 0; z < TZ; ++z)
#pragma unroll
                for (int o = 0; o < HEAD; ++o) part[z][o] = 0.f;
#pragma unroll
            for (int q = 0; q < 4; ++q) {
                float4 hw[HEAD > 0 ? HEAD : 1];
#pragma unroll
                for (int o = 0; o < HEAD; ++o)
                    hw[o] = *reinterpret_cast<const float4*>(head_s + o * 32 + 8 * q + 4 * half_e);
#pragma unroll
                for (int z = 0; z < TZ; ++z) {
                    float v0 = acc[z][4 * q + 0], v1 = acc[z][4 * q + 1];
                    float v2 = acc[z][4 * q + 2], v3 = acc[z][4 * q + 3];
                    v0 = leaky(v0, a.slope);
                    v1 = leaky(v1, a.slope);
                    v2 = leaky(v2, a.slope);
                    v3 = leaky(v3, a.slope);
#pragma unroll
                    for (int o = 0; o < HEAD; ++o)
                        part[z][o] = fmaf(v3, hw[o].w, fmaf(v2, hw[o].z, fmaf(v1, hw[o].y, fmaf(v0, hw[o].x, part[z][o]))));
                }
            }
            const size_t plane = (size_t)a.h * a.w;
            const int gy = cur.y0 + pos_e / TX, gx = cur.x0 + pos_e % TX;
            const bool okyx = gy < a.org[1] + a.ext[1] && gx < a.org[2] + a.ext[2];
            float* const hpatch = a.head_out + (size_t)cur.nb * HEAD * a.d * plane;
            const size_t hbytes = (size_t)HEAD * a.d * plane * sizeof(float);
            const unsigned hvoff[2] = {okyx && half_e == 0 ? (unsigned)(gy * a.w + gx) * 4u : kOutOfRange,
                                       okyx && half_e == 1 ? (unsigned)(gy * a.w + gx) * 4u : kOutOfRange};
#pragma unroll
            for (int z = 0; z < TZ; ++z) {
                const int gz = cur.z0 + z;
                const __amdgpu_buffer_rsrc_t hrsrc = make_rsrc(hpatch, gz < a.org[0] + a.ext[0] ? hbytes : (size_t)0);
#pragma unroll
                for (int o = 0; o < HEAD; ++o) {
                    float t = part[z][o] + __shfl_xor(part[z][o], 32) + head_s[HEAD * 32 + o];
                    if (a.head_sigmoid) t = 1.f / (1.f + expf(-t));
                    __builtin_amdgcn_raw_buffer_store_b32(__float_as_uint(t), hrsrc, (int)hvoff[o & 1],
                                                          (int)((unsigned)(o * a.d + gz) * (unsigned)plane * 4u), 0);
                }
            }
        } else if (ES == 2 && !POOL) {
            char* const dplane = static_cast<char*>(a.dst) +
                                 ((size_t)cur.nb * (a.cout / KC) + ntile0 * 2) * patch_vox * 32;
            const int gy = cur.y0 + pos_e / TX, gx = cur.x0 + pos_e % TX;
            const bool okyx = gy < a.org[1] + a.ext[1] && gx < a.org[2] + a.ext[2];
            const unsigned ovoff = okyx ? (unsigned)(gy * a.w + gx) * 32u + half_e * 16u : kOutOfRange;
#pragma unroll
            for (int z = 0; z < TZ; ++z) {
                uint2 grp[4];
#pragma unroll
                for (int q = 0; q < 4; ++q)
                    grp[q] = pack4<Tag>(leaky(acc[z][4 * q + 0], a.slope), leaky(acc[z][4 * q + 1], a.slope),
                                        leaky(acc[z][4 * q + 2], a.slope), leaky(acc[z][4 * q + 3], a.slope));
                const int gz = cur.z0 + z;
#pragma unroll
                for (int ck = 0; ck < 2; ++ck) {
                    const uint4 rec = record_half(grp[2 * ck], grp[2 * ck + 1]);
                    const unsigned soff = ((unsigned)ck * (unsigned)patch_vox + (unsigned)gz * (unsigned)plane_vox) * 32u;
                    const __amdgpu_buffer_rsrc_t orsrc =
                        make_rsrc(dplane, gz < a.org[0] + a.ext[0] ? (size_t)2 * patch_vox * 32 : (size_t)0);
                    buf_store16(rec, orsrc, ovoff, soff);
                }
            }
        } else if (ES == 2 && POOL) {
            static_assert(!(ES == 2 && POOL) || (TZ % 2 == 0 && TY % 2 == 0 && TX == 16), "pooled tile shape");
            constexpr int CPT = 2;
            char* wl = reinterpret_cast<char*>(lds) + wave * ((TZ / 2) * 32 * RECP);
            char* const dplane = static_cast<char*>(a.dst) +
                                 ((size_t)cur.nb * (a.cout / KC) + ntile0 * 2) * patch_vox * 32;
            const int gy = cur.y0 + pos_e / TX, gx = cur.x0 + pos_e % TX;
            const bool okyx = gy < a.org[1] + a.ext[1] && gx < a.org[2] + a.ext[2];
            const unsigned ovoff = okyx ? (unsigned)(gy * a.w + gx) * 32u + half_e * 16u : kOutOfRange;
            const int rs = a.row_stride, rho = (a.w - rs) >> 1;
            const bool nnext = row && cur.x0 >= rs && cur.x0 < rs + rho && cur.nb + 1 < a.n;
            const bool nprev = row && cur.x0 >= rho && cur.x0 < 2 * rho && cur.nb >= 1;
            const bool shared = nnext || nprev;
            const int nshift = nnext ? -rs : nprev ? rs : 0;
            const int nnb = cur.nb + (nnext ? 1 : nprev ? -1 : 0);
            const int ngx = gx + nshift;
            const bool nlane = ngx >= 2 && ngx < a.w - 2;
            const int nbase = nshift * 32;
            char* const nplane = static_cast<char*>(a.dst) + nbase +
                                 ((size_t)nnb * (a.cout / KC) + ntile0 * 2) * patch_vox * 32;
            const size_t nbytes = (size_t)((long long)2 * patch_vox * 32 - nbase);
            const bool cout_on = CARRY && a.carry_dst != nullptr;
            const long long cshift = (long long)a.out_shift * plane_vox * 32;
            char* const cplane = static_cast<char*>(a.carry_dst) - cshift +
                                 ((size_t)cur.nb * (a.cout / KC) + ntile0 * 2) * patch_vox * 32;
            char* const cnplane = static_cast<char*>(a.carry_dst) - cshift + nbase +
                                  ((size_t)nnb * (a.cout / KC) + ntile0 * 2) * patch_vox * 32;
            bool y_on = false, d_on = false;
            long long yshift = 0;
            if constexpr (CARRYY) {
                const int wy = cur.y0 + 2 * wave;
                const bool yrow = wy >= cy.out_y0 && wy < cy.out_y1;
                y_on = cy.y_dst != nullptr && yrow;
                d_on = cy.d_dst != nullptr && yrow;
                yshift = (long long)cy.out_shift_y * a.w * 32;
            }
#pragma unroll
            for (int zp = 0; zp < TZ / 2; ++zp) {
                uint2 grp[2][4];
#pragma unroll
                for (int zz = 0; zz < 2; ++zz)
#pragma unroll
                    for (int q = 0; q < 4; ++q)
                        grp[zz][q] = pack4<Tag>(leaky(acc[2 * zp + zz][4 * q + 0], a.slope), leaky(acc[2 * zp + zz][4 * q + 1], a.slope),
                                                leaky(acc[2 * zp + zz][4 * q + 2], a.slope), leaky(acc[2 * zp + zz][4 * q + 3], a.slope));
#pragma unroll
                for (int q = 0; q < 4; ++q) {
                    const uint2 km = make_uint2(maxkey16x2(okey16x2<Tag::kInf16>(grp[0][q].x), okey16x2<Tag::kInf16>(grp[1][q].x)),
                                                maxkey16x2(okey16x2<Tag::kInf16>(grp[0][q].y), okey16x2<Tag::kInf16>(grp[1][q].y)));
                    *reinterpret_cast<uint2*>(wl + zp * (32 * RECP) + r_e * RECP + (8 * q + 4 * half_e) * ES) = km;
                }
#pragma unroll
                for (int zz = 0; zz < 2; ++zz) {
                    const int gz = cur.z0 + 2 * zp + zz;
                    const __amdgpu_buffer_rsrc_t orsrc =
                        make_rsrc(dplane, gz < a.org[0] + a.ext[0] ? (size_t)2 * patch_vox * 32 : (size_t)0);
                    const __amdgpu_buffer_rsrc_t nrsrc = make_rsrc(nplane, gz < a.org[0] + a.ext[0] ? nbytes : (size_t)0);
#pragma unroll
                    for (int ck = 0; ck < 2; ++ck) {
                        const uint4 rec = record_half(grp[zz][2 * ck], grp[zz][2 * ck + 1]);
                        buf_store16(rec, orsrc, ovoff, ((unsigned)ck * (unsigned)patch_vox + (unsigned)gz * (unsigned)plane_vox) * 32u);
                        if (shared)
                            buf_store16(rec, nrsrc, nlane ? ovoff : kOutOfRange, ((unsigned)ck * (unsigned)patch_vox + (unsigned)gz * (unsigned)plane_vox) * 32u);
                        if (CARRY && cout_on) {
                            const bool cz = gz >= a.out_z0 && gz < a.out_z1;
                            buf_store16(rec, make_rsrc(cplane, cz ? (size_t)2 * patch_vox * 32 : (size_t)0), ovoff,
                                        ((unsigned)ck * (unsigned)patch_vox + (unsigned)gz * (unsigned)plane_vox) * 32u);
                            if (shared)
                                buf_store16(rec, make_rsrc(cnplane, cz ? nbytes : (size_t)0), nlane ? ovoff : kOutOfRange,
                                            ((unsigned)ck * (unsigned)patch_vox + (unsigned)gz * (unsigned)plane_vox) * 32u);
                        }
                        if constexpr (CARRYY) if (y_on) {
                            const bool yz = gz < a.org[0] + a.ext[0];
                            const size_t poff = ((size_t)cur.nb * (a.cout / KC) + ntile0 * 2) * patch_vox * 32;
                            buf_store16(rec, make_rsrc(static_cast<char*>(cy.y_dst) - yshift + poff, yz ? (size_t)2 * patch_vox * 32 : (size_t)0),
                                        ovoff, ((unsigned)ck * (unsigned)patch_vox + (unsigned)gz * (unsigned)plane_vox) * 32u);
                            if (shared) {
                                const size_t npoff = ((size_t)nnb * (a.cout / KC) + ntile0 * 2) * patch_vox * 32;
                                buf_store16(rec, make_rsrc(static_cast<char*>(cy.y_dst) - yshift + nbase + npoff, yz ? nbytes : (size_t)0),
                                            nlane ? ovoff : kOutOfRange,
                                            ((unsigned)ck * (unsigned)patch_vox + (unsigned)gz * (unsigned)plane_vox) * 32u);
                            }
                        }
                        if constexpr (CARRYY) if (d_on) {
                            const bool dz = gz >= a.out_z0 && gz < a.out_z1;
                            const size_t poff = ((size_t)cur.nb * (a.cout / KC) + ntile0 * 2) * patch_vox * 32;
                            buf_store16(rec, make_rsrc(static_cast<char*>(cy.d_dst) - cshift - yshift + poff, dz ? (size_t)2 * patch_vox * 32 : (size_t)0),
                                        ovoff, ((unsigned)ck * (unsigned)patch_vox + (unsigned)gz * (unsigned)plane_vox) * 32u);
                            if (shared) {
                                const size_t npoff = ((size_t)nnb * (a.cout / KC) + ntile0 * 2) * patch_vox * 32;
                                buf_store16(rec, make_rsrc(static_cast<char*>(cy.d_dst) - cshift - yshift + nbase + npoff, dz ? nbytes : (size_t)0),
                                            nlane ? ovoff : kOutOfRange,
                                            ((unsigned)ck * (unsigned)patch_vox + (unsigned)gz * (unsigned)plane_vox) * 32u);
                            }
                        }
                    }
                }
            }
            __builtin_amdgcn_fence(__ATOMIC_RELEASE, "wavefront");
            __builtin_amdgcn_wave_barrier();
            {
                constexpr int NP = (TZ / 2) * 8 * CPT * 2;
                const int pd = a.d >> 1, ph = a.h >> 1, pw2 = a.w >> 1;
                const size_t pvox = (size_t)pd * ph * pw2;
                char* const pplane = static_cast<char*>(a.pool_dst) +
                                     ((size_t)cur.nb * (a.cout / KC) + ntile0 * CPT) * pvox * 32;
                const __amdgpu_buffer_rsrc_t prsrc = make_rsrc(pplane, (size_t)CPT * pvox * 32);
                char* const npplane = static_cast<char*>(a.pool_dst) + nbase / 2 +
                                      ((size_t)nnb * (a.cout / KC) + ntile0 * CPT) * pvox * 32;
                const __amdgpu_buffer_rsrc_t nprsrc = make_rsrc(npplane, (size_t)((long long)CPT * pvox * 32 - nbase / 2));
                const long long cpshift = (long long)(a.out_shift >> 1) * ph * pw2 * 32;
                char* const cpplane = static_cast<char*>(a.carry_pool_dst) - cpshift +
                                      ((size_t)cur.nb * (a.cout / KC) + ntile0 * CPT) * pvox * 32;
                char* const cnpplane = static_cast<char*>(a.carry_pool_dst) - cpshift + nbase / 2 +
                                       ((size_t)nnb * (a.cout / KC) + ntile0 * CPT) * pvox * 32;
#pragma unroll
                for (int p0 = 0; p0 < NP; p0 += 64) {
                    const int p = p0 + lane_e;
                    const bool live = p < NP;
                    const int pc = live ? p : 0;
                    const int zp = pc / (8 * CPT * 2), rem = pc % (8 * CPT * 2);
                    const int ck = rem / 16, xp = (rem % 16) >> 1, sb = rem & 1;
                    const char* rec = wl + zp * (32 * RECP) + (2 * xp) * RECP + (ck * 2 + sb) * 16;
                    uint4 m = *reinterpret_cast<const uint4*>(rec);
#pragma unroll
                    for (int k = 1; k < 4; ++k)
                        m = maxkey16(m, *reinterpret_cast<const uint4*>(rec + (k >> 1) * 16 * RECP + (k & 1) * RECP));
                    m = key16(m);
                    const int qz = cur.z0 / 2 + zp, qy = cur.y0 / 2 + wave, qx = cur.x0 / 2 + xp;
                    const unsigned pvoff = live && qz < pd && qy < ph && qx < pw2
                                               ? (unsigned)((ck * (int)pvox + (qz * ph + qy) * pw2 + qx) * 32 + sb * 16)
                                               : kOutOfRange;
                    buf_store16(m, prsrc, pvoff, 0u);
                    if (shared) {
                        const int nqx = qx + nshift / 2;
                        buf_store16(m, nprsrc, nqx >= 1 && nqx < pw2 - 1 ? pvoff : kOutOfRange, 0u);
                    }
                    if (CARRY && cout_on) {
                        const unsigned cpvoff = 2 * qz >= a.out_z0 && 2 * qz < a.out_z1 ? pvoff : kOutOfRange;
                        buf_store16(m, make_rsrc(cpplane, (size_t)CPT * pvox * 32), cpvoff, 0u);
                        if (shared) {
                            const int nqx = qx + nshift / 2;
                            buf_store16(m, make_rsrc(cnpplane, (size_t)((long long)CPT * pvox * 32 - nbase / 2)),
                                        nqx >= 1 && nqx < pw2 - 1 ? cpvoff : kOutOfRange, 0u);
                        }
                    }
                    if constexpr (CARRYY) if (y_on || d_on) {
                        const long long ypshift = (long long)(cy.out_shift_y >> 1) * pw2 * 32;
                        const size_t ppoff = ((size_t)cur.nb * (a.cout / KC) + ntile0 * CPT) * pvox * 32;
                        const size_t nppoff = ((size_t)nnb * (a.cout / KC) + ntile0 * CPT) * pvox * 32;
                        const int nqx = qx + nshift / 2;
                        const bool nq = nqx >= 1 && nqx < pw2 - 1;
                        if (y_on) {
                            buf_store16(m, make_rsrc(static_cast<char*>(cy.y_pool_dst) - ypshift + ppoff, (size_t)CPT * pvox * 32), pvoff, 0u);
                            if (shared)
                                buf_store16(m, make_rsrc(static_cast<char*>(cy.y_pool_dst) - ypshift + nbase / 2 + nppoff,
                                                         (size_t)((long long)CPT * pvox * 32 - nbase / 2)),
                                            nq ? pvoff : kOutOfRange, 0u);
                        }
                        if (d_on) {
                            const unsigned dpvoff = 2 * qz >= a.out_z0 && 2 * qz < a.out_z1 ? pvoff : kOutOfRange;
                            buf_store16(m, make_rsrc(static_cast<char*>(cy.d_pool_dst) - cpshift - ypshift + ppoff, (size_t)CPT * pvox * 32), dpvoff, 0u);
                            if (shared)
                                buf_store16(m, make_rsrc(static_cast<char*>(cy.d_pool_dst) - cpshift - ypshift + nbase / 2 + nppoff,
                                                         (size_t)((long long)CPT * pvox * 32 - nbase / 2)),
                                            nq ? dpvoff : kOutOfRange, 0u);
                        }
                    }
                }
            }
            __builtin_amdgcn_fence(__ATOMIC_ACQUIRE, "wavefront");
            __builtin_amdgcn_wave_barrier();
        } else {
            constexpr int CPT = RECB / 32;
            constexpr int TB_MAX = LDS_UNITS * 16 / (NWAVES * 32 * RECP);
            constexpr int TB = POOL ? ((TB_MAX >= TZ ? TZ : TB_MAX) & ~1)
                                    : (TB_MAX >= TZ ? TZ : (TB_MAX >= (TZ + 1) / 2 ? (TZ + 1) / 2 : 1));
            static_assert(!POOL || (TB >= 2 && TZ % 2 == 0 && TY % 2 == 0 && TX == 16), "pooled tile shape");
            char* wl = reinterpret_cast<char*>(lds) + wave * (TB * 32 * RECP);
            char* const dplane = static_cast<char*>(a.dst) +
                                 ((size_t)cur.nb * (a.cout / KC) + ntile0 * CPT) * patch_vox * 32;
            const int vv = lane_e >> 1, sub = lane_e & 1;
            const int po = wave * 32 + vv;
            const int ogy = cur.y0 + po / TX, ogx = cur.x0 + po % TX;
#pragma unroll
            for (int zb = 0; zb < TZ; zb += TB) {
#pragma unroll
                for (int z = zb; z < zb + TB && z < TZ; ++z) {
#pragma unroll
                    for (int q = 0; q < 4; ++q) {
                        const int cl = 8 * q + 4 * half_e;
                        float v0 = acc[z][4 * q + 0], v1 = acc[z][4 * q + 1];
                        float v2 = acc[z][4 * q + 2], v3 = acc[z][4 * q + 3];
                        v0 = leaky(v0, a.slope);
                        v1 = leaky(v1, a.slope);
                        v2 = leaky(v2, a.slope);
                        v3 = leaky(v3, a.slope);
                        store4<Tag>(wl + (z - zb) * (32 * RECP), (size_t)(r_e * RECP) / ES + cl, v0, v1, v2, v3);
                    }
                }
                __builtin_amdgcn_fence(__ATOMIC_RELEASE, "wavefront");
                __builtin_amdgcn_wave_barrier();
#pragma unroll
                for (int z = zb; z < zb + TB && z < TZ; ++z) {
                    const int gz = cur.z0 + z;
                    const bool tokyx = ogy < a.org[1] + a.ext[1] && ogx < a.org[2] + a.ext[2];
                    const unsigned tvoff = tokyx ? (unsigned)(ogy * a.w + ogx) * 32u + sub * 16u : kOutOfRange;
                    const __amdgpu_buffer_rsrc_t trsrc =
                        make_rsrc(dplane, gz < a.org[0] + a.ext[0] ? (size_t)CPT * patch_vox * 32 : (size_t)0);
#pragma unroll
                    for (int ck = 0; ck < CPT; ++ck) {
                        const uint4 val = *reinterpret_cast<const uint4*>(
                            wl + (z - zb) * (32 * RECP) + vv * RECP + (ck * 2 + sub) * 16);
                        buf_store16(val, trsrc, tvoff,
                                    ((unsigned)ck * (unsigned)patch_vox + (unsigned)gz * (unsigned)plane_vox) * 32u);
                    }
                }
                if (POOL) {
                    constexpr int NP = (TB / 2) * 8 * CPT * 2;
                    const int pd = a.d >> 1, ph = a.h >> 1, pw2 = a.w >> 1;
                    const size_t pvox = (size_t)pd * ph * pw2;
                    char* const pplane = static_cast<char*>(a.pool_dst) +
                                         ((size_t)cur.nb * (a.cout / KC) + ntile0 * CPT) * pvox * 32;
                    const __amdgpu_buffer_rsrc_t prsrc = make_rsrc(pplane, (size_t)CPT * pvox * 32);
#pragma unroll
                    for (int p0 = 0; p0 < NP; p0 += 64) {
                        const int p = p0 + lane_e;
                        const bool live0 = p < NP;
                        const int pc = live0 ? p : 0;
                        const int zp = pc / (8 * CPT * 2), rem = pc % (8 * CPT * 2);
                        const int ck = rem / 16, xp = (rem % 16) >> 1, sb = rem & 1;
                        const bool live = live0 && zb + 2 * zp + 1 < TZ;
                        const int zr = zb + 2 * zp + 1 < TZ ? zp : 0;
                        const char* rec = wl + (2 * zr) * (32 * RECP) + (2 * xp) * RECP + (ck * 2 + sb) * 16;
                        uint4 m = *reinterpret_cast<const uint4*>(rec);
                        if (ES == 2) m = okey16<Tag::kInf16>(m);
#pragma unroll
                        for (int k = 1; k < 8; ++k) {
                            const uint4 v = *reinterpret_cast<const uint4*>(
                                rec + (k >> 2) * (32 * RECP) + ((k >> 1) & 1) * 16 * RECP + (k & 1) * RECP);
                            m = ES == 2 ? maxkey16(m, okey16<Tag::kInf16>(v)) : max16<Tag>(m, v);
                        }
                        if (ES == 2) m = key16(m);
                        const int qz = (cur.z0 + zb) / 2 + zp, qy = cur.y0 / 2 + wave, qx = cur.x0 / 2 + xp;
                        const unsigned pvoff =
                            live && qz < pd && qy < ph && qx < pw2
                                ? (unsigned)((ck * (int)pvox + (qz * ph + qy) * pw2 + qx) * 32 + sb * 16)
                                : kOutOfRange;
                        buf_store16(m, prsrc, pvoff, 0u);
                    }
                }
                __builtin_amdgcn_fence(__ATOMIC_ACQUIRE, "wavefront");
                __builtin_amdgcn_wave_barrier();
            }
        }
        EXA_TRACE(14);
        if (!has_next) break;
        if (!(HEAD > 0 || (ES == 2 && !POOL))) __syncthreads();
        stage_store();
        tile_id += t_step;
        cur = nxt;
    }
}

template <typename Tag, int TZ, int TY, int TX, int MINW, int D, int HEAD = 0, bool POOL = false>
__global__ __launch_bounds__(TY* TX * 2, MINW) void conv3x3x3_zpipe(
    ConvArgs a, int tiles_z, int tiles_y, int tiles_x) {
    zpipe_body<Tag, TZ, TY, TX, MINW, D, HEAD, POOL, false>(a, tiles_z, tiles_y, tiles_x);
}

template <typename Tag, int TZ, int TY, int TX, int MINW, int D>
__global__ __launch_bounds__(TY* TX * 2, MINW) void conv3x3x3_zpipe_row(
    ConvArgs a, int tiles_z, int tiles_y, int tiles_x) {
    zpipe_body<Tag, TZ, TY, TX, MINW, D, 0, true, true>(a, tiles_z, tiles_y, tiles_x);
}

template <typename Tag, int TZ, int TY, int TX, int MINW, int D>
__global__ __launch_bounds__(TY* TX * 2, MINW) void conv3x3x3_zpipe_rowz(
    ConvArgs a, int tiles_z, int tiles_y, int tiles_x) {
    zpipe_body<Tag, TZ, TY, TX, MINW, D, 0, true, true, true>(a, tiles_z, tiles_y, tiles_x);
}

template <typename Tag, int TZ, int TY, int TX, int MINW, int D>
__global__ __launch_bounds__(TY* TX * 2, MINW) void conv3x3x3_zpipe_rowzy(
    ConvArgs a, ConvCarryY cy, int tiles_z, int tiles_y, int tiles_x) {
    zpipe_body<Tag, TZ, TY, TX, MINW, D, 0, true, true, true, true>(a, tiles_z, tiles_y, tiles_x, cy);
}

}
```

aind_exaspim_neuron_segmentation_amd/csrc/engine.hip:

```cpp

#include <algorithm>
#include <cstdlib>
#include <new>
#include <string_view>

#include "common.h"

namespace exaspim {

constexpr float kLeakySlope = 0.01f;

struct Workspace {
    size_t skip[5], a[5], b[5];
    size_t xpad;
    size_t bytes;
};

}

struct LayerTimer {
    static constexpr int kRing = 16384;
    uint32_t mask = 0;
    int next = 0, used = 0;
    hipEvent_t start[kRing], stop[kRing];
// ... 51 lines not shown
        !conv_can_fuse_pool(p.dtype, p.conv[2].cout, d >> 1, h >> 1, w >> 1))
        return 0;
    int tz = 0;
    for (int idx = 1; idx <= 2; ++idx) {
        static float scratch;
        ConvArgs a{};
        a.ca = p.conv[idx].ca; a.cb = p.conv[idx].cb; a.cout = p.conv[idx].cout;
        a.n = n; a.d = d >> 1; a.h = h >> 1; a.w = w >> 1;
        a.partial = &scratch;
        a.partial_patch_bytes = (size_t)(d + 2) * (h + 2) * (w + 2) * sizeof(float);
        const int t = conv_carry_t14_tile_depth(p.dtype, a);
        if (t == 0 || (tz != 0 && t != tz)) return 0;
        tz = t;
    }
    return tz;
}

void carry1_span_of_tiles(int tz, int d, int shift_z, int32_t out[2]) {
    out[0] = out[1] = 0;
    int32_t l0[2];
    carry_span(d, shift_z, l0);
    if (l0[0] >= l0[1] || shift_z % 4 != 0 || tz <= 0 || tz % 2 != 0) return;
    const int d1 = d / 2, s1 = shift_z / 2;
    const int lo = (3 + tz - 1) / tz * tz, hi = (d1 - s1 - 3) / tz * tz;
    if (lo < hi && hi + s1 <= 254) { out[0] = lo; out[1] = hi; }
}
static void carry1_span(const exaspim_unet* e, int n, int d, int h, int w, int shift_z, int32_t out[2]) {
    carry1_span_of_tiles(carry1_tile_depth(e, n, d, h, w), d, shift_z, out);
}

static Workspace make_workspace(const UNetPlan& p, int n, int d, int h, int w) {
    int maxc[5] = {p.c0p, 0, 0, 0, 0};
    for (int i = 0; i < kNumMfmaConvs; ++i) {
        const ConvLayer& L = p.conv[i];
        int& m = maxc[conv_level(i)];
        m = std::max(m, std::max(std::max(L.ca, L.cb), L.cout));
    }
    const size_t es = dtype_size(p.dtype);
    Workspace ws;
    size_t off = 0;
    for (int l = 0; l < 5; ++l) {
        const size_t vox = (size_t)n * (d >> l) * (h >> l) * (w >> l);
        const size_t sz = align_up(vox * maxc[l] * es, 256);
        ws.skip[l] = off; off += (l < 4 ? sz : 0);
        ws.a[l] = off; off += sz;
        ws.b[l] = off; off += sz;
    }
    ws.xpad = off;
    off += align_up((size_t)n * (d + 2) * (h + 2) * (w + 2) * sizeof(float), 256);
    ws.bytes = off;
    return ws;
}

static int forward(exaspim_unet* e, const float* x, float* out, int n, int d, int h, int w,
                   int apply_sigmoid, int trim, void* workspace, size_t workspace_bytes,
                   hipStream_t stream, const void* x_prepared = nullptr, float* absmax = nullptr,
                   int row_stride = 0, const int32_t* keep_hi = nullptr, const exaspim_unet_carry* carry = nullptr,
                   const exaspim_unet_carry1* carry1 = nullptr, const exaspim_unet_carry_y* carry_y = nullptr) {
    const UNetPlan& p = e->plan;
    const Workspace ws = make_workspace(p, n, d, h, w);
    if (workspace_bytes < ws.bytes) {
        set_error("forward: workspace %zu bytes < required %zu", workspace_bytes, ws.bytes);
        return EXASPIM_E_WORKSPACE;
    }
    char* base = static_cast<char*>(workspace);
    auto skip = [&](int l) { return (void*)(base + ws.skip[l]); };
    auto A = [&](int l) { return (void*)(base + ws.a[l]); };
    auto B = [&](int l) { return (void*)(base + ws.b[l]); };
    const int dt = p.dtype;
    int rc;

    const bool x3 = dt == EXASPIM_DT_BF16X3;
    const int last_cout = p.conv[kNumMfmaConvs - 1].cout;
    const bool fuse_head = !absmax && !(e->options & EXASPIM_OPT_SEPARATE_HEAD) &&
                           (x3 ? conv_x3_can_fuse_head(last_cout, w, p.out_channels)
                               : conv_can_fuse_head(last_cout, w, p.out_channels, dt));
    const bool trimmed = fuse_head && trim > 0 && 2 * trim < d && 2 * trim < h && 2 * trim < w;
    int khi[3] = {d - trim, h - trim, w - trim};
    if (trimmed && keep_hi)
        for (int i = 0; i < 3; ++i) khi[i] = keep_hi[i];
    const bool separate_pool = (e->options & EXASPIM_OPT_SEPARATE_POOL) != 0;
    const bool separate_deep = (e->options & EXASPIM_OPT_SEPARATE_DEEP_POOLS) != 0;
    bool fuse_pool[4];
    for (int l = 0; l < 4; ++l)
        fuse_pool[l] = !separate_pool && !(separate_deep && l > 0) && conv_can_fuse_pool(p.dtype, p.conv[2 * l].cout, d >> l, h >> l, w >> l);
    const bool row = !absmax && !(e->options & EXASPIM_OPT_PER_PATCH_ENCODER) &&
                     conv_row_mode_ok(dt, p.conv[0].cout, n, w, row_stride, fuse_pool[0]);
    if (carry) {
        int32_t span[2];
        const int shift = carry->out_skip ? carry->out_shift : 0;
        const bool in = carry->in_z[0] != 0 || carry->in_z[1] != 0;
        EXA_CHECK_ARG(row && carry->own_skip && carry->own_pool && carry->reserved == 0,
                      "forward: carried planes need row mode at this geometry and both own buffers");
        EXA_CHECK_ARG(!carry->out_skip == !carry->out_pool, "forward: carry out needs both targets or neither");
        const int tzd = conv_zcol_tile_depth(d);
        if (in)
            EXA_CHECK_ARG(carry->in_z[0] >= 2 && carry->in_z[0] < carry->in_z[1] && carry->in_z[1] <= d - 2 &&
                              carry->in_z[0] % tzd == 0 && carry->in_z[1] % tzd == 0 && carry->in_z[0] % 2 == 0 &&
                              carry->in_z[1] % 2 == 0,
                          "forward: carry in [%d, %d) is not whole %d-plane tiles with even bounds inside [2, %d)",
                          carry->in_z[0], carry->in_z[1], tzd, d - 2);
        if (shift || carry->out_skip) {
            carry_span(d, shift, span);
            EXA_CHECK_ARG(shift > 0 && span[0] < span[1] && carry->out_z[0] == span[0] + shift &&
                              carry->out_z[1] == span[1] + shift && carry->out_z[1] <= 254,
                          "forward: carry out [%d, %d) shifted by %d is not the range a forward %d planes down takes over",
                          carry->out_z[0], carry->out_z[1], shift, shift);
            EXA_CHECK_ARG(!in || carry->out_z[0] >= carry->in_z[1] || carry->out_z[1] <= carry->in_z[0],
                          "forward: carry out [%d, %d) overlaps the planes carried in, [%d, %d)", carry->out_z[0],
                          carry->out_z[1], carry->in_z[0], carry->in_z[1]);
        }
    }
    ConvCarryY cy;
    if (carry_y) {
        const bool in = carry_y->in_y[0] != 0 || carry_y->in_y[1] != 0;
        const bool out_y = carry_y->out_skip_y || carry_y->out_pool_y || carry_y->out_shift_y || carry_y->out_y[0] || carry_y->out_y[1];
        EXA_CHECK_ARG(carry && row && carry_y->reserved == 0,
                      "forward: carried rows need the first level's carry struct and row mode at this geometry");
        EXA_CHECK_ARG(!carry_y->out_skip_y == !carry_y->out_pool_y && !carry_y->out_skip_d == !carry_y->out_pool_d,
                      "forward: y and diagonal carry out need both targets or neither");
        if (in)
            EXA_CHECK_ARG(carry_y->in_y[0] >= 2 && carry_y->in_y[0] < carry_y->in_y[1] && carry_y->in_y[1] <= h - 2 &&
                              carry_y->in_y[0] % 8 == 0 && carry_y->in_y[1] % 8 == 0,
                          "forward: y carry in [%d, %d) is not whole 8-row tiles inside [2, %d)", carry_y->in_y[0],
                          carry_y->in_y[1], h - 2);
        if (out_y) {
            int32_t span[2];
            const int shift = carry_y->out_skip_y ? carry_y->out_shift_y : 0;
            carry_row_span(h, shift, span);
            EXA_CHECK_ARG(shift > 0 && span[0] < span[1] && carry_y->out_y[0] == span[0] + shift &&
                              carry_y->out_y[1] == span[1] + shift,
                          "forward: y carry out [%d, %d) shifted by %d is not the range a forward %d rows on takes over",
                          carry_y->out_y[0], carry_y->out_y[1], shift, shift);
            EXA_CHECK_ARG(!in || carry_y->out_y[0] >= carry_y->in_y[1] || carry_y->out_y[1] <= carry_y->in_y[0],
                          "forward: y carry out [%d, %d) overlaps the rows carried in, [%d, %d)", carry_y->out_y[0],
                          carry_y->out_y[1], carry_y->in_y[0], carry_y->in_y[1]);
        }
        EXA_CHECK_ARG(!carry_y->out_skip_d || (carry->out_skip && carry_y->out_skip_y),
                      "forward: the diagonal carry out needs both the z and the y carry out");
        if (!(e->options & EXASPIM_OPT_CARRY_NO_ROWS)) {
            cy.in_y0 = (unsigned short)carry_y->in_y[0];
            cy.in_y1 = (unsigned short)carry_y->in_y[1];
            if (carry_y->out_skip_y) {
                cy.y_dst = carry_y->out_skip_y;
                cy.y_pool_dst = carry_y->out_pool_y;
                cy.d_dst = carry_y->out_skip_d;
                cy.d_pool_dst = carry_y->out_pool_d;
                cy.out_y0 = (unsigned short)carry_y->out_y[0];
                cy.out_y1 = (unsigned short)carry_y->out_y[1];
                cy.out_shift_y = (unsigned short)carry_y->out_shift_y;
            }
        }
    }
    const bool carry_borders = carry && !(e->options & (EXASPIM_OPT_CARRY_MAIN_ONLY | EXASPIM_OPT_ROW_SEPARATE_BORDERS));
    int32_t first_skip[2] = {0, 0};
    if (carry_borders) conv_first_skip_planes(d, carry->in_z[0], carry->in_z[1], first_skip);
    void* const x1 = carry ? carry->own_skip : skip(0);
    void* const x1_pool = carry ? carry->own_pool : A(1);
    if (carry1) {
        EXA_CHECK_ARG(carry && carry1->own_mid1 && carry1->own_skip1 && carry1->own_pool2 && carry1->reserved == 0,
                      "forward: carried planes of the second level need those of the first and all three own buffers");
        EXA_CHECK_ARG(!carry1->out_mid1 == !carry1->out_skip1 && !carry1->out_mid1 == !carry1->out_pool2,
                      "forward: second-level carry out needs all three targets or none");
        const int tz1 = carry1_tile_depth(e, n, d, h, w);
        EXA_CHECK_ARG(tz1 > 0, "forward: down1.0 and down1.3 cannot carry planes at this geometry, dtype or option set");
        if (carry1->in_z[0] != 0 || carry1->in_z[1] != 0)
            EXA_CHECK_ARG((carry->in_z[0] != 0 || carry->in_z[1] != 0) && carry1->in_z[0] >= 3 &&
                              carry1->in_z[0] < carry1->in_z[1] && carry1->in_z[1] <= d / 2 - 3 &&
                              carry1->in_z[0] % tz1 == 0 && carry1->in_z[1] % tz1 == 0,
                          "forward: second-level carry in [%d, %d) needs a first-level carry in and whole %d-plane tiles "
                          "inside [3, %d)", carry1->in_z[0], carry1->in_z[1], tz1, d / 2 - 3);
        if (carry1->out_mid1 || carry1->out_shift) {
            int32_t span[2];
            const int shift1 = carry1->out_mid1 ? carry1->out_shift : 0;
            carry1_span(e, n, d, h, w, 2 * shift1, span);
            EXA_CHECK_ARG(shift1 > 0 && carry->out_skip && carry->out_shift == 2 * shift1 && span[0] < span[1] &&
                              carry1->out_z[0] == span[0] + shift1 && carry1->out_z[1] == span[1] + shift1,
                          "forward: second-level carry out [%d, %d) shifted by %d is not the range a forward %d planes down "
                          "takes over, or the first level does not carry out by twice the shift",
                          carry1->out_z[0], carry1->out_z[1], shift1, 2 * shift1);
            EXA_CHECK_ARG(carry1->out_z[0] >= carry1->in_z[1] || carry1->out_z[1] <= carry1->in_z[0],
                          "forward: second-level carry out [%d, %d) overlaps the planes carried in, [%d, %d)",
                          carry1->out_z[0], carry1->out_z[1], carry1->in_z[0], carry1->in_z[1]);
        }
    }
    void* const mid1 = carry1 ? carry1->own_mid1 : B(1);
    void* const skip1 = carry1 ? carry1->own_skip1 : skip(1);
    void* const pool2 = carry1 ? carry1->own_pool2 : A(2);
    auto conv = [&](int idx, const void* sa, const void* sb, void* dst, int l) -> int {
        const ConvLayer& L = p.conv[idx];
        ConvArgs a;
        a.partial = reinterpret_cast<float*>(base + ws.xpad);
        a.partial_patch_bytes = (size_t)(d + 2) * (h + 2) * (w + 2) * sizeof(float);
        if (idx <= 6 && idx % 2 == 0 && fuse_pool[idx / 2]) a.pool_dst = idx == 0 ? x1_pool : idx == 2 ? pool2 : A(idx / 2 + 1);
        const bool last = idx == kNumMfmaConvs - 1, last_but_one = idx == kNumMfmaConvs - 2;
        const int margin = !trimmed ? 0 : last ? trim : last_but_one ? trim - 1 : 0;
        const int full[3] = {d >> l, h >> l, w >> l};
        for (int i = 0; i < 3; ++i) {
            a.org[i] = margin;
            a.ext[i] = trimmed && (last || last_but_one) ? khi[i] + (last ? 0 : 1) - margin : full[i];
        }
        int rem_y = 0, rem_x = 0;
        const bool has_head = idx == kNumMfmaConvs - 1 && fuse_head;
        if (margin > 0 && !has_head && L.cout % 64 != 0 && full[2] % 16 == 0) {
            rem_y = a.ext[1] - conv_zcol_main_extent(a.ext[1], 1);
            rem_x = a.ext[2] - conv_zcol_main_extent(a.ext[2], 2);
            a.ext[1] -= rem_y;
            a.ext[2] -= rem_x;
        }
        if (idx == kNumMfmaConvs - 1 && fuse_head) {
            a.head_w = reinterpret_cast<const float*>(e->packed + p.head_w_off);
            a.head_b = reinterpret_cast<const float*>(e->packed + p.head_b_off);
            a.head_out = out;
            a.head_oc = p.out_channels;
            a.head_sigmoid = apply_sigmoid;
        }
        a.src_a = sa; a.src_b = sb; a.ca = L.ca; a.cb = L.cb;
        a.weights = e->packed + L.w_off;
        a.bias = reinterpret_cast<const float*>(e->packed + L.b_off);
        a.dst = dst; a.cout = L.cout;
        a.n = n; a.d = d >> l; a.h = h >> l; a.w = w >> l;
        a.slope = kLeakySlope;
        if (idx == 0 && row) a.row_stride = row_stride;
        if (idx == 0 && carry) {
            a.in_z0 = (unsigned short)carry->in_z[0];
            a.in_z1 = (unsigned short)carry->in_z[1];
            if (carry->out_skip) {
                a.carry_dst = carry->out_skip;
                a.carry_pool_dst = carry->out_pool;
                a.out_z0 = (unsigned char)carry->out_z[0];
                a.out_z1 = (unsigned char)carry->out_z[1];
                a.out_shift = (unsigned short)carry->out_shift;
            }
        }
        if ((idx == 1 || idx == 2) && carry1) {
            a.in_z0 = (unsigned short)carry1->in_z[0];
            a.in_z1 = (unsigned short)carry1->in_z[1];
            if (carry1->out_mid1) {
                a.carry_dst = idx == 1 ? carry1->out_mid1 : carry1->out_skip1;
                a.carry_pool_dst = idx == 1 ? nullptr : carry1->out_pool2;
                a.out_z0 = (unsigned char)carry1->out_z[0];
                a.out_z1 = (unsigned char)carry1->out_z[1];
                a.out_shift = (unsigned short)carry1->out_shift;
            }
        }
        LayerTimer* t = e->timer;
        const bool timed = t && (t->mask >> idx & 1u) && t->used < LayerTimer::kRing;
        int slot = 0;
        if (timed) {
            slot = t->next;
            EXA_CHECK_HIP(hipEventRecord(t->start[slot], stream));
        }
        int r = x3 && has_head      ? launch_conv3x3x3_x3_head(a, stream)
                : a.row_stride > 0 ? launch_conv3x3x3_row(dt, a, (e->options & EXASPIM_OPT_ROW_SEPARATE_BORDERS) ? kRowStagesAll
                                                                 : carry_borders ? kRowStagesCarry : kRowStagesFused, stream,
                                                        idx == 0 ? &cy : nullptr)
                                   : launch_conv3x3x3(dt, a, stream);
        if (timed && r == EXASPIM_OK) {
            EXA_CHECK_HIP(hipEventRecord(t->stop[slot], stream));
            t->layer[slot] = idx;
            t->next = (slot + 1) % LayerTimer::kRing;
            t->used++;
        }
        if (r == EXASPIM_OK && rem_y > 0) {
            ConvArgs b = a;
            b.org[1] = a.org[1] + a.ext[1]; b.ext[1] = rem_y;
            b.ext[2] = a.ext[2] + rem_x;
            r = launch_conv3x3x3_thin(dt, b, stream);
        }
        if (r == EXASPIM_OK && rem_x > 0) {
            ConvArgs b = a;
            b.org[2] = a.org[2] + a.ext[2]; b.ext[2] = rem_x;
            r = launch_conv3x3x3_thin(dt, b, stream);
        }
        if (r == EXASPIM_OK && absmax)
            r = launch_absmax(dt, dst, (size_t)n * (d >> l) * (h >> l) * (w >> l) * L.cout * dtype_size(dt),
                              absmax + 1 + idx, stream);
        return r;
    };
#define RUN(expr) do { rc = (expr); if (rc) return rc; } while (0)

    RUN(launch_conv_first(dt, x, x ? reinterpret_cast<float*>(base + ws.xpad)
                                   : const_cast<float*>(static_cast<const float*>(x_prepared)),
                          reinterpret_cast<const float*>(e->packed + p.first_w_off),
                          reinterpret_cast<const float*>(e->packed + p.first_b_off), A(0), n, d,
                          h, w, p.c0p, kLeakySlope, stream, (e->options & EXASPIM_OPT_FIRST_PER_GROUP) != 0,
                          first_skip[0], first_skip[1]));
    if (absmax) RUN(launch_absmax(dt, A(0), (size_t)n * d * h * w * p.c0p * dtype_size(dt), absmax, stream));
    RUN(conv(0, A(0), nullptr, x1, 0));
    if (carry_y && carry_y->encoder_event)
        EXA_CHECK_HIP(hipEventRecord(static_cast<hipEvent_t>(carry_y->encoder_event), stream));
    for (int l = 1; l <= 4; ++l) {
        const ConvLayer& L0 = p.conv[2 * l - 1];
        const void* prev = l == 1 ? x1 : l == 2 ? skip1 : skip(l - 1);
        if (!fuse_pool[l - 1])
            RUN(launch_maxpool2(dt, prev, A(l), n, d >> (l - 1), h >> (l - 1), w >> (l - 1), L0.ca,
                                stream));
        void* const mid = l == 1 ? mid1 : B(l);
        RUN(conv(2 * l - 1, l == 1 ? x1_pool : l == 2 ? pool2 : A(l), nullptr, mid, l));
        RUN(conv(2 * l, mid, nullptr, l == 1 ? skip1 : l < 4 ? skip(l) : A(l), l));
    }
    const void* prev = A(4);
    for (int l = 3; l >= 0; --l) {
        const int i0 = 9 + 2 * (3 - l);
        const ConvLayer& L0 = p.conv[i0];
        if (p.convt) {
            const ConvTLayer& U = p.up[3 - l];
            RUN(launch_convt2(dt, prev, e->packed + U.w_off,
                              reinterpret_cast<const float*>(e->packed + U.b_off), A(l), n,
                              d >> (l + 1), h >> (l + 1), w >> (l + 1), U.cin, U.cout, stream));
            if (absmax)
                RUN(launch_absmax(dt, A(l), (size_t)n * (d >> l) * (h >> l) * (w >> l) * U.cout * dtype_size(dt),
                                  absmax + 1 + kNumMfmaConvs + (3 - l), stream));
        } else {
            const bool ups_trimmed = trimmed && l == 0 && trim > 2;
            const int ups_hi[3] = {std::max(d - khi[0] - 2, 0), std::max(h - khi[1] - 2, 0), std::max(w - khi[2] - 2, 0)};
            RUN(launch_upsample2(dt, prev, A(l), n, d >> (l + 1), h >> (l + 1), w >> (l + 1), L0.cb,
                                 ups_trimmed ? trim - 2 : 0, stream,
                                 (e->options & EXASPIM_OPT_PLAIN_UPSAMPLE) != 0,
                                 (e->options & EXASPIM_OPT_UPSAMPLE_PER_THREAD) != 0, ups_trimmed ? ups_hi : nullptr));
        }
        RUN(conv(i0, l == 0 ? x1 : l == 1 ? skip1 : skip(l), A(l), B(l), l));
        RUN(conv(i0 + 1, B(l), nullptr, A(l), l));
        prev = A(l);
    }
    if (!fuse_head)
    RUN(launch_head(dt, prev, reinterpret_cast<const float*>(e->packed + p.head_w_off),
                    reinterpret_cast<const float*>(e->packed + p.head_b_off), out, n, d, h, w,
                    p.c0p, p.out_channels, apply_sigmoid, stream));
#undef RUN
    return EXASPIM_OK;
}

}

using namespace exaspim;

extern "C" int exaspim_abi_version(void) { return EXASPIM_ABI_VERSION; }
extern "C" const char* exaspim_last_error(void) { return get_error(); }

extern "C" size_t exaspim_unet_param_count(const int32_t channels[5], int32_t out_channels,
                                           int32_t dtype) {
    UNetPlan p;
    if (!make_plan(channels, out_channels, dtype, &p)) return 0;
    return p.n_params;
}

extern "C" size_t exaspim_unet_packed_bytes(const int32_t channels[5], int32_t out_channels,
                                            int32_t dtype) {
    UNetPlan p;
    if (!make_plan(channels, out_channels, dtype, &p)) return 0;
    return p.packed_bytes;
}

extern "C" int exaspim_unet_pack_weights(const int32_t channels[5], int32_t out_channels,
                                         int32_t dtype, const float* params, size_t n_params,
                                         void* packed_host, size_t packed_bytes) {
    UNetPlan p;
    if (!make_plan(channels, out_channels, dtype, &p)) return EXASPIM_E_INVALID;
    EXA_CHECK_ARG(params && packed_host, "pack_weights: NULL pointer");
    EXA_CHECK_ARG(n_params == p.n_params, "pack_weights: got %zu parameters, expected %zu",
                  n_params, p.n_params);
    EXA_CHECK_ARG(packed_bytes == p.packed_bytes, "pack_weights: buffer %zu bytes, expected %zu",
                  packed_bytes, p.packed_bytes);
    return pack_weights(p, params, packed_host);
}

extern "C" int exaspim_unet_create(const int32_t channels[5], int32_t out_channels,
                                   int32_t dtype, int32_t device, const void* packed_dev,
                                   size_t packed_bytes, exaspim_unet** out) {
    EXA_CHECK_ARG(out != nullptr && packed_dev != nullptr, "create: NULL pointer");
    UNetPlan p;
    if (!make_plan(channels, out_channels, dtype, &p)) return EXASPIM_E_INVALID;
    EXA_CHECK_ARG(packed_bytes == p.packed_bytes, "create: packed image %zu bytes, expected %zu",
                  packed_bytes, p.packed_bytes);
    int ndev = 0;
    if (hipGetDeviceCount(&ndev) != hipSuccess || ndev <= 0 || device < 0 || device >= ndev) {
        set_error("create: device %d not available (%d HIP devices visible)", device, ndev);
        return EXASPIM_E_NODEVICE;
    }
    hipDeviceProp_t prop;
    EXA_CHECK_HIP(hipGetDeviceProperties(&prop, device));
    if (std::string_view(prop.gcnArchName).substr(0, 6) != "gfx950") {
        set_error("create: device %d is %s; this library is built for gfx950 only", device,
                  prop.gcnArchName);
        return EXASPIM_E_NODEVICE;
    }
    exaspim_unet* e = new (std::nothrow) exaspim_unet;
    EXA_CHECK_ARG(e != nullptr, "create: out of host memory");
    e->plan = p;
    e->device = device;
    e->packed = static_cast<const char*>(packed_dev);
    *out = e;
    return EXASPIM_OK;
}

extern "C" void exaspim_unet_destroy(exaspim_unet* h) {
    if (!h) return;
    if (h->timer) {
        if (h->timer->created)
            for (int i = 0; i < LayerTimer::kRing; ++i) {
                (void)hipEventDestroy(h->timer->start[i]);
                (void)hipEventDestroy(h->timer->stop[i]);
            }
        delete h->timer;
    }
    delete h;
}

extern "C" int exaspim_unet_timing_begin(exaspim_unet* h, uint32_t conv_mask) {
    EXA_CHECK_ARG(h != nullptr, "timing_begin: NULL handle");
    if (!h->timer) h->timer = new (std::nothrow) LayerTimer;
    EXA_CHECK_ARG(h->timer != nullptr, "timing_begin: out of host memory");
    LayerTimer* t = h->timer;
    if (!t->created) {
        for (int i = 0; i < LayerTimer::kRing; ++i) {
            EXA_CHECK_HIP(hipEventCreate(&t->start[i]));
            EXA_CHECK_HIP(hipEventCreate(&t->stop[i]));
        }
        t->created = true;
    }
    t->mask = conv_mask;
    t->next = 0;
    t->used = 0;
    return EXASPIM_OK;
}
// ... 68 lines not shown
                                                 int32_t n, int32_t d, int32_t hgt, int32_t w,
                                                 int32_t apply_sigmoid, int32_t trim, int32_t row_stride,
                                                 void* workspace_dev, size_t workspace_bytes,
                                                 void* stream) {
    EXA_CHECK_ARG(h && x_prepared_dev && out_dev && workspace_dev, "forward: NULL pointer");
    EXA_CHECK_ARG(n > 0, "forward: empty batch");
    EXA_CHECK_ARG(trim >= 0, "forward: negative trim %d", trim);
    EXA_CHECK_ARG(row_stride >= 0, "forward: negative row stride %d", row_stride);
    EXA_CHECK_ARG(level_dims_ok(d, hgt, w),
                  "forward: patch %dx%dx%d: every dimension must be a positive multiple of 16",
                  d, hgt, w);
    return forward(h, nullptr, out_dev, n, d, hgt, w, apply_sigmoid, trim, workspace_dev,
                   workspace_bytes, (hipStream_t)stream, x_prepared_dev, nullptr, row_stride);
}

extern "C" int exaspim_unet_forward_prepared_clipped(exaspim_unet* h, const void* x_prepared_dev, float* out_dev,
                                                     int32_t n, int32_t d, int32_t hgt, int32_t w,
                                                     int32_t apply_sigmoid, int32_t trim, int32_t row_stride,
                                                     const int32_t keep_hi[3], void* workspace_dev,
                                                     size_t workspace_bytes, void* stream) {
    EXA_CHECK_ARG(h && x_prepared_dev && out_dev && workspace_dev && keep_hi, "forward: NULL pointer");
    EXA_CHECK_ARG(n > 0, "forward: empty batch");
    EXA_CHECK_ARG(trim >= 0, "forward: negative trim %d", trim);
    EXA_CHECK_ARG(row_stride >= 0, "forward: negative row stride %d", row_stride);
    EXA_CHECK_ARG(level_dims_ok(d, hgt, w),
                  "forward: patch %dx%dx%d: every dimension must be a positive multiple of 16",
                  d, hgt, w);
    const int size[3] = {d, hgt, w};
    for (int i = 0; i < 3; ++i)
        EXA_CHECK_ARG(keep_hi[i] > trim && keep_hi[i] <= size[i] - trim,
                      "forward: keep_hi[%d] = %d outside (%d, %d] (trim %d of %d voxels)", i, keep_hi[i], trim,
                      size[i] - trim, trim, size[i]);
    return forward(h, nullptr, out_dev, n, d, hgt, w, apply_sigmoid, trim, workspace_dev,
                   workspace_bytes, (hipStream_t)stream, x_prepared_dev, nullptr, row_stride, keep_hi);
}

extern "C" int exaspim_unet_carry_planes(const exaspim_unet* h, int32_t n, int32_t d, int32_t hgt, int32_t w,
                                         int32_t row_stride, int32_t shift_z, int32_t out[2]) {
    EXA_CHECK_ARG(h && out, "carry_planes: NULL pointer");
    out[0] = out[1] = 0;
    EXA_CHECK_ARG(n > 0 && level_dims_ok(d, hgt, w) && row_stride >= 0 && shift_z > 0,
                  "carry_planes: bad arguments (n %d, patch %dx%dx%d, row stride %d, shift %d)", n, d, hgt, w,
                  row_stride, shift_z);
    const UNetPlan& p = h->plan;
    const bool fused = !(h->options & EXASPIM_OPT_SEPARATE_POOL) && conv_can_fuse_pool(p.dtype, p.conv[0].cout, d, hgt, w);
    if ((h->options & EXASPIM_OPT_PER_PATCH_ENCODER) || !conv_row_mode_ok(p.dtype, p.conv[0].cout, n, w, row_stride, fused))
        return EXASPIM_OK;
    carry_span(d, shift_z, out);
    return EXASPIM_OK;
}

extern "C" int exaspim_unet_carry_rows(const exaspim_unet* h, int32_t n, int32_t d, int32_t hgt, int32_t w,
                                       int32_t row_stride, int32_t shift_y, int32_t out[2]) {
    EXA_CHECK_ARG(h && out, "carry_rows: NULL pointer");
    out[0] = out[1] = 0;
    EXA_CHECK_ARG(n > 0 && level_dims_ok(d, hgt, w) && row_stride >= 0 && shift_y > 0,
                  "carry_rows: bad arguments (n %d, patch %dx%dx%d, row stride %d, shift %d)", n, d, hgt, w,
                  row_stride, shift_y);
    const UNetPlan& p = h->plan;
    const bool fused = !(h->options & EXASPIM_OPT_SEPARATE_POOL) && conv_can_fuse_pool(p.dtype, p.conv[0].cout, d, hgt, w);
    if ((h->options & (EXASPIM_OPT_PER_PATCH_ENCODER | EXASPIM_OPT_CARRY_NO_ROWS)) ||
        !conv_row_mode_ok(p.dtype, p.conv[0].cout, n, w, row_stride, fused))
        return EXASPIM_OK;
    carry_row_span(hgt, shift_y, out);
    return EXASPIM_OK;
}

extern "C" int exaspim_unet_carry1_planes(const exaspim_unet* h, int32_t n, int32_t d, int32_t hgt, int32_t w,
                                          int32_t row_stride, int32_t shift_z, int32_t out[2]) {
    int32_t l0[2];
    EXA_CHECK_ARG(out, "carry_planes: NULL pointer");
    out[0] = out[1] = 0;
    if (int rc = exaspim_unet_carry_planes(h, n, d, hgt, w, row_stride, shift_z, l0)) return rc;
    if (l0[0] < l0[1]) carry1_span(h, n, d, hgt, w, shift_z, out);
    return EXASPIM_OK;
}

extern "C" int exaspim_unet_forward_prepared_carry(exaspim_unet* h, const void* x_prepared_dev, float* out_dev,
                                                   int32_t n, int32_t d, int32_t hgt, int32_t w,
                                                   int32_t apply_sigmoid, int32_t trim, int32_t row_stride,
                                                   const int32_t keep_hi[3], const exaspim_unet_carry* carry,
                                                   void* workspace_dev, size_t workspace_bytes, void* stream) {
    return exaspim_unet_forward_prepared_carry1(h, x_prepared_dev, out_dev, n, d, hgt, w, apply_sigmoid, trim, row_stride,
                                                keep_hi, carry, nullptr, workspace_dev, workspace_bytes, stream);
}

extern "C" int exaspim_unet_forward_prepared_carry1(exaspim_unet* h, const void* x_prepared_dev, float* out_dev,
                                                    int32_t n, int32_t d, int32_t hgt, int32_t w,
                                                    int32_t apply_sigmoid, int32_t trim, int32_t row_stride,
                                                    const int32_t keep_hi[3], const exaspim_unet_carry* carry,
                                                    const exaspim_unet_carry1* carry1, void* workspace_dev,
                                                    size_t workspace_bytes, void* stream) {
    return exaspim_unet_forward_prepared_carry_y(h, x_prepared_dev, out_dev, n, d, hgt, w, apply_sigmoid, trim, row_stride,
                                                 keep_hi, carry, carry1, nullptr, workspace_dev, workspace_bytes, stream);
}

extern "C" int exaspim_unet_forward_prepared_carry_y(exaspim_unet* h, const void* x_prepared_dev, float* out_dev,
                                                     int32_t n, int32_t d, int32_t hgt, int32_t w,
                                                     int32_t apply_sigmoid, int32_t trim, int32_t row_stride,
                                                     const int32_t keep_hi[3], const exaspim_unet_carry* carry,
                                                     const exaspim_unet_carry1* carry1,
                                                     const exaspim_unet_carry_y* carry_y, void* workspace_dev,
                                                     size_t workspace_bytes, void* stream) {
    EXA_CHECK_ARG(h && x_prepared_dev && out_dev && workspace_dev && keep_hi && carry, "forward: NULL pointer");
    EXA_CHECK_ARG(n > 0, "forward: empty batch");
    EXA_CHECK_ARG(trim >= 0, "forward: negative trim %d", trim);
    EXA_CHECK_ARG(row_stride >= 0, "forward: negative row stride %d", row_stride);
    EXA_CHECK_ARG(level_dims_ok(d, hgt, w),
                  "forward: patch %dx%dx%d: every dimension must be a positive multiple of 16",
                  d, hgt, w);
    const int size[3] = {d, hgt, w};
    for (int i = 0; i < 3; ++i)
        EXA_CHECK_ARG(keep_hi[i] > trim && keep_hi[i] <= size[i] - trim,
                      "forward: keep_hi[%d] = %d outside (%d, %d] (trim %d of %d voxels)", i, keep_hi[i], trim,
                      size[i] - trim, trim, size[i]);
    return forward(h, nullptr, out_dev, n, d, hgt, w, apply_sigmoid, trim, workspace_dev,
                   workspace_bytes, (hipStream_t)stream, x_prepared_dev, nullptr, row_stride, keep_hi, carry, carry1,
                   carry_y);
}

extern "C" int exaspim_unet_forward_trimmed(exaspim_unet* h, const float* x_dev, float* out_dev,
                                            int32_t n, int32_t d, int32_t hgt, int32_t w,
                                            int32_t apply_sigmoid, int32_t trim,
                                            void* workspace_dev, size_t workspace_bytes,
                                            void* stream) {
    EXA_CHECK_ARG(h && x_dev && out_dev && workspace_dev, "forward: NULL pointer");
    EXA_CHECK_ARG(n > 0, "forward: empty batch");
    EXA_CHECK_ARG(trim >= 0, "forward: negative trim %d", trim);
    EXA_CHECK_ARG(level_dims_ok(d, hgt, w),
                  "forward: patch %dx%dx%d: every dimension must be a positive multiple of 16",
                  d, hgt, w);
    return forward(h, x_dev, out_dev, n, d, hgt, w, apply_sigmoid, trim, workspace_dev,
                   workspace_bytes, (hipStream_t)stream);
}

extern "C" int exaspim_unet_forward_absmax(exaspim_unet* h, const float* x_dev, float* out_dev,
                                           int32_t n, int32_t d, int32_t hgt, int32_t w,
                                           int32_t apply_sigmoid, float* absmax_dev,
                                           void* workspace_dev, size_t workspace_bytes, void* stream) {
    EXA_CHECK_ARG(h && x_dev && out_dev && workspace_dev && absmax_dev, "forward_absmax: NULL pointer");
    EXA_CHECK_ARG(n > 0, "forward: empty batch");
    EXA_CHECK_ARG(level_dims_ok(d, hgt, w),
                  "forward: patch %dx%dx%d: every dimension must be a positive multiple of 16",
                  d, hgt, w);
    return forward(h, x_dev, out_dev, n, d, hgt, w, apply_sigmoid, 0, workspace_dev, workspace_bytes,
                   (hipStream_t)stream, nullptr, absmax_dev);
}

extern "C" int exaspim_unet_set_options(exaspim_unet* h, uint32_t options) {
    EXA_CHECK_ARG(h != nullptr, "set_options: NULL handle");
    EXA_CHECK_ARG((options & ~(uint32_t)(EXASPIM_OPT_SEPARATE_POOL | EXASPIM_OPT_SEPARATE_DEEP_POOLS | EXASPIM_OPT_PLAIN_UPSAMPLE | EXASPIM_OPT_FIRST_PER_GROUP |
                                          EXASPIM_OPT_UPSAMPLE_PER_THREAD | EXASPIM_OPT_PER_PATCH_ENCODER |
                                          EXASPIM_OPT_SEPARATE_HEAD | EXASPIM_OPT_ROW_SEPARATE_BORDERS |
                                          EXASPIM_OPT_CARRY_MAIN_ONLY | EXASPIM_OPT_CARRY_NO_ROWS)) == 0,
                  "set_options: unknown option bits 0x%x", options);
    h->options = options;
    return EXASPIM_OK;
}
```

aind_exaspim_neuron_segmentation_amd/csrc/layer_probe.hip:

```cpp

#include "common.h"

using namespace exaspim;

extern "C" {

const char* probe_last_error(void) { return get_error(); }

const char* probe_last_config(void) { return last_conv_launch().config; }
int probe_last_ksplit(void) { return last_conv_launch().ksplit; }
void probe_reset_config(void) {
    last_conv_launch() = ConvLaunchRecord{};
    last_layer_kernel() = "";
}
int probe_last_row(void) { return last_conv_launch().row ? 1 : 0; }
const char* probe_last_layer_kernel(void) { return last_layer_kernel(); }

int probe_conv3x3x3(int thin, int dtype, const void* src_a, const void* src_b, int ca, int cb,
                    const void* weights, const float* bias, void* dst, int cout, int n, int d, int h,
                    int w, float slope, const int32_t* region, void* pool_dst, float* partial,
                    size_t partial_patch_bytes, const float* head_w, const float* head_b,
                    float* head_out, int head_oc, int head_sigmoid, hipStream_t stream) {
    ConvArgs a{};
    a.src_a = src_a;
// ... 4 lines not shown
    a.bias = bias;
    a.dst = dst;
    a.cout = cout;
    a.n = n;
    a.d = d;
    a.h = h;
    a.w = w;
    a.slope = slope;
    for (int i = 0; i < 3; ++i) {
        a.org[i] = region ? region[i] : 0;
        a.ext[i] = region ? region[3 + i] : 0;
    }
    a.pool_dst = pool_dst;
    a.partial = partial;
    a.partial_patch_bytes = partial_patch_bytes;
    a.head_w = head_w;
    a.head_b = head_b;
    a.head_out = head_out;
    a.head_oc = head_oc;
    a.head_sigmoid = head_sigmoid;
    return thin ? launch_conv3x3x3_thin(dtype, a, stream) : launch_conv3x3x3(dtype, a, stream);
}

int probe_conv3x3x3_x3_head(int thin, int dtype, const void* src_a, const void* src_b, int ca, int cb,
                            const void* weights, const float* bias, void* dst, int cout, int n, int d, int h,
                            int w, float slope, const int32_t* region, void* pool_dst, float* partial,
                            size_t partial_patch_bytes, const float* head_w, const float* head_b,
                            float* head_out, int head_oc, int head_sigmoid, hipStream_t stream) {
    EXA_CHECK_ARG(!thin && dtype == EXASPIM_DT_BF16X3 && !partial,
                  "probe: the bf16x3 head launcher has no thin tiles, no other dtype and no split-K");
    ConvArgs a{};
    a.src_a = src_a;
    a.src_b = src_b;
    a.ca = ca;
    a.cb = cb;
    a.weights = weights;
    a.bias = bias;
    a.dst = dst;
    a.cout = cout;
    a.n = n;
    a.d = d;
    a.h = h;
    a.w = w;
    a.slope = slope;
    for (int i = 0; i < 3; ++i) {
        a.org[i] = region ? region[i] : 0;
        a.ext[i] = region ? region[3 + i] : 0;
    }
    a.pool_dst = pool_dst;
    a.head_w = head_w;
    a.head_b = head_b;
    a.head_out = head_out;
    a.head_oc = head_oc;
    a.head_sigmoid = head_sigmoid;
    return launch_conv3x3x3_x3_head(a, stream);
}

int probe_conv3x3x3_row(int dtype, const void* src, int ca, const void* weights, const float* bias, void* dst,
                        int cout, int n, int d, int h, int w, float slope, int row_stride, void* pool_dst,
                        int stages, hipStream_t stream) {
    ConvArgs a{};
    a.src_a = src;
    a.ca = ca;
    a.weights = weights;
    a.bias = bias;
    a.dst = dst;
    a.cout = cout;
    a.n = n;
    a.d = d;
    a.h = h;
    a.w = w;
    a.slope = slope;
    a.row_stride = row_stride;
    a.pool_dst = pool_dst;
    return launch_conv3x3x3_row(dtype, a, stages, stream);
}

int probe_conv3x3x3_row_carry(int dtype, const void* src, int ca, const void* weights, const float* bias, void* dst,
                              int cout, int n, int d, int h, int w, float slope, int row_stride, void* pool_dst,
                              const int32_t* carry, void* carry_dst, void* carry_pool_dst, int stages,
                              hipStream_t stream) {
    EXA_CHECK_ARG(carry != nullptr, "probe: NULL carry");
    for (int i = 0; i < 5; ++i)
        EXA_CHECK_ARG(carry[i] >= 0 && carry[i] <= (i == 2 || i == 3 ? 254 : 65534), "probe: carry[%d] = %d out of range", i, carry[i]);
    ConvArgs a{};
    a.src_a = src;
    a.ca = ca;
    a.weights = weights;
    a.bias = bias;
    a.dst = dst;
    a.cout = cout;
    a.n = n;
    a.d = d;
    a.h = h;
    a.w = w;
    a.slope = slope;
    a.row_stride = row_stride;
    a.pool_dst = pool_dst;
    a.in_z0 = (unsigned short)carry[0];
    a.in_z1 = (unsigned short)carry[1];
    a.out_z0 = (unsigned char)carry[2];
    a.out_z1 = (unsigned char)carry[3];
    a.out_shift = (unsigned short)carry[4];
    a.carry_dst = carry_dst;
    a.carry_pool_dst = carry_pool_dst;
    return launch_conv3x3x3_row(dtype, a, stages, stream);
}
int probe_last_carry(void) { return last_conv_launch().carry ? 1 : 0; }

int probe_conv3x3x3_row_carry_y(int dtype, const void* src, int ca, const void* weights, const float* bias, void* dst,
                                int cout, int n, int d, int h, int w, float slope, int row_stride, void* pool_dst,
                                const int32_t* carry, void* carry_dst, void* carry_pool_dst, const int32_t* carry_y,
                                void* const* targets, int stages, hipStream_t stream) {
    EXA_CHECK_ARG(carry != nullptr && carry_y != nullptr && targets != nullptr, "probe: NULL carry");
    for (int i = 0; i < 5; ++i) {
        EXA_CHECK_ARG(carry[i] >= 0 && carry[i] <= (i == 2 || i == 3 ? 254 : 65534), "probe: carry[%d] = %d out of range", i, carry[i]);
        EXA_CHECK_ARG(carry_y[i] >= 0 && carry_y[i] <= 65534, "probe: carry_y[%d] = %d out of range", i, carry_y[i]);
    }
    ConvArgs a{};
    a.src_a = src;
    a.ca = ca;
    a.weights = weights;
    a.bias = bias;
    a.dst = dst;
    a.cout = cout;
    a.n = n;
    a.d = d;
    a.h = h;
    a.w = w;
    a.slope = slope;
    a.row_stride = row_stride;
    a.pool_dst = pool_dst;
    a.in_z0 = (unsigned short)carry[0];
    a.in_z1 = (unsigned short)carry[1];
    a.out_z0 = (unsigned char)carry[2];
    a.out_z1 = (unsigned char)carry[3];
    a.out_shift = (unsigned short)carry[4];
    a.carry_dst = carry_dst;
    a.carry_pool_dst = carry_pool_dst;
    ConvCarryY y;
    y.in_y0 = (unsigned short)carry_y[0];
    y.in_y1 = (unsigned short)carry_y[1];
    y.out_y0 = (unsigned short)carry_y[2];
    y.out_y1 = (unsigned short)carry_y[3];
    y.out_shift_y = (unsigned short)carry_y[4];
    y.y_dst = targets[0];
    y.y_pool_dst = targets[1];
    y.d_dst = targets[2];
    y.d_pool_dst = targets[3];
    return launch_conv3x3x3_row(dtype, a, stages, stream, &y);
}
int probe_last_carry_y(void) { return last_conv_launch().carry_y ? 1 : 0; }

int probe_conv3x3x3_carry(int dtype, const void* src, int ca, const void* weights, const float* bias, void* dst,
                          int cout, int n, int d, int h, int w, float slope, void* pool_dst, float* partial,
                          size_t partial_patch_bytes, const int32_t* carry, void* carry_dst, void* carry_pool_dst,
                          hipStream_t stream) {
    EXA_CHECK_ARG(carry != nullptr, "probe: NULL carry");
    for (int i = 0; i < 5; ++i)
        EXA_CHECK_ARG(carry[i] >= 0 && carry[i] <= (i == 2 || i == 3 ? 254 : 65534), "probe: carry[%d] = %d out of range", i, carry[i]);
    ConvArgs a{};
    a.src_a = src;
    a.ca = ca;
    a.weights = weights;
    a.bias = bias;
    a.dst = dst;
    a.cout = cout;
    a.n = n;
    a.d = d;
    a.h = h;
    a.w = w;
    a.slope = slope;
    a.pool_dst = pool_dst;
    a.partial = partial;
    a.partial_patch_bytes = partial_patch_bytes;
    a.in_z0 = (unsigned short)carry[0];
    a.in_z1 = (unsigned short)carry[1];
    a.out_z0 = (unsigned char)carry[2];
    a.out_z1 = (unsigned char)carry[3];
    a.out_shift = (unsigned short)carry[4];
    a.carry_dst = carry_dst;
    a.carry_pool_dst = carry_pool_dst;
    return launch_conv3x3x3(dtype, a, stream);
}
void probe_carry1_span(int tz, int d, int shift_z, int32_t* out) { carry1_span_of_tiles(tz, d, shift_z, out); }
int probe_conv_carry_tile_depth(int dtype, int ca, int cout, int n, int d, int h, int w, size_t partial_patch_bytes) {
    ConvArgs a{};
    a.ca = ca;
    a.cout = cout;
    a.n = n;
    a.d = d;
    a.h = h;
    a.w = w;
    static float scratch;
    a.partial = partial_patch_bytes ? &scratch : nullptr;
    a.partial_patch_bytes = partial_patch_bytes;
    return conv_carry_t14_tile_depth(dtype, a);
}

int probe_conv_row_mode_ok(int dtype, int cout, int n, int w, int row_stride, int fused_pool_whole_patch) {
    return conv_row_mode_ok(dtype, cout, n, w, row_stride, fused_pool_whole_patch != 0) ? 1 : 0;
}

int probe_conv_first(int dtype, const float* x, float* xpad, const float* w, const float* bias,
                     void* dst, int n, int d, int h, int wd, int c0p, float slope, int per_group,
                     hipStream_t stream) {
    return launch_conv_first(dtype, x, xpad, w, bias, dst, n, d, h, wd, c0p, slope, stream, per_group != 0);
}

int probe_conv_first_planes(int dtype, const float* x, float* xpad, const float* w, const float* bias,
                            void* dst, int n, int d, int h, int wd, int c0p, float slope, int per_group,
                            int skip_z0, int skip_z1, hipStream_t stream) {
    return launch_conv_first(dtype, x, xpad, w, bias, dst, n, d, h, wd, c0p, slope, stream, per_group != 0, skip_z0,
                             skip_z1);
}
void probe_conv_first_skip_planes(int d, int in_z0, int in_z1, int32_t* out) { conv_first_skip_planes(d, in_z0, in_z1, out); }
void probe_row_tile_depths(int d, int32_t* out) {
    out[0] = conv_zcol_tile_depth(d);
    out[1] = conv_row_borders_tile_depth(d);
}

int probe_maxpool2(int dtype, const void* src, void* dst, int n, int d, int h, int w, int c,
                   hipStream_t stream) {
    return launch_maxpool2(dtype, src, dst, n, d, h, w, c, stream);
}

int probe_maxpool2_xcols(int dtype, const void* src, void* dst, int n, int d, int h, int w, int c, int ox0,
                         int ox1, hipStream_t stream) {
    return launch_maxpool2_xcols(dtype, src, dst, n, d, h, w, c, ox0, ox1, stream);
}

int probe_upsample2(int dtype, const void* src, void* dst, int n, int d, int h, int w, int c,
                    int margin, int plain_kernel, int per_thread, hipStream_t stream) {
    return launch_upsample2(dtype, src, dst, n, d, h, w, c, margin, stream, plain_kernel != 0,
                            per_thread != 0);
}

int probe_upsample2_hi(int dtype, const void* src, void* dst, int n, int d, int h, int w, int c,
                       int margin, const int margin_hi[3], int plain_kernel, int per_thread,
                       hipStream_t stream) {
    return launch_upsample2(dtype, src, dst, n, d, h, w, c, margin, stream, plain_kernel != 0,
                            per_thread != 0, margin_hi);
}

int probe_convt2(int dtype, const void* src, const void* weights, const float* bias, void* dst, int n,
                 int d, int h, int w, int cin, int cout, hipStream_t stream) {
    return launch_convt2(dtype, src, weights, bias, dst, n, d, h, w, cin, cout, stream);
}

int probe_head(int dtype, const void* src, const float* w, const float* bias, float* out, int n,
               int d, int h, int wd, int c0p, int out_channels, int apply_sigmoid, hipStream_t stream) {
    return launch_head(dtype, src, w, bias, out, n, d, h, wd, c0p, out_channels, apply_sigmoid, stream);
}

int probe_plan_conv(const int32_t channels[5], int32_t out_channels, int32_t dtype, int layer,
                    int64_t out[8]) {
    UNetPlan p;
    if (!make_plan(channels, out_channels, dtype, &p)) return EXASPIM_E_INVALID;
    EXA_CHECK_ARG(layer >= 0 && layer < kNumMfmaConvs, "probe: layer %d out of range", layer);
    const ConvLayer& L = p.conv[layer];
    const int64_t v[8] = {L.ca_real, L.cb_real, L.ca, L.cb, L.cout_real, L.cout, (int64_t)L.w_off,
                          (int64_t)L.b_off};
    for (int i = 0; i < 8; ++i) out[i] = v[i];
    return EXASPIM_OK;
}

int probe_dbf_pass(int axis, const int32_t* labels, const int32_t* in, int32_t* out, const int32_t dims[3],
                   int black_border, hipStream_t stream) {
    EXA_CHECK_ARG(labels && out && dims && (axis == 2 || (in && in != out)), "probe_dbf_pass: NULL or aliased buffer");
    return launch_dbf_pass(axis, labels, in, out, dims, black_border, stream);
}

int probe_fill_holes_passes(const int32_t* labels, const int32_t dims[3], int32_t* out, int64_t* counts,
                            void* workspace, int first, int last, hipStream_t stream) {
    EXA_CHECK_ARG(labels && dims && out && counts && workspace, "probe_fill_holes_passes: NULL buffer");
    EXA_CHECK_ARG(((uintptr_t)workspace & 15) == 0 && ((uintptr_t)counts & 7) == 0,
                  "probe_fill_holes_passes: misaligned buffer");
    return launch_fill_holes_passes(labels, dims, out, counts, workspace, first, last, stream);
}

}
```

include/exaspim_affinity.h:

```cpp
#ifndef EXASPIM_AFFINITY_H
#define EXASPIM_AFFINITY_H

#include <stddef.h>
#include <stdint.h>

#ifdef __cplusplus
extern "C" {
#endif

#define EXASPIM_ABI_VERSION 5

#define EXASPIM_OK 0
#define EXASPIM_E_INVALID (-1)
#define EXASPIM_E_HIP (-2)
#define EXASPIM_E_WORKSPACE (-3)
#define EXASPIM_E_NODEVICE (-4)

#define EXASPIM_DT_F32 0
#define EXASPIM_DT_BF16 1
#define EXASPIM_DT_F16 2
#define EXASPIM_DT_BF16X3 3
#define EXASPIM_UP_CONVT 0x100

#define EXASPIM_VOX_U8 0
#define EXASPIM_VOX_U16 1
#define EXASPIM_VOX_I16 2
#define EXASPIM_VOX_F32 3
#define EXASPIM_VOX_F64 4

typedef struct exaspim_unet exaspim_unet;

typedef struct exaspim_block {
    int32_t dims[3];
    int32_t origin[3];
    int32_t global[3];
} exaspim_block;

typedef struct exaspim_window {
    int32_t patch[3];
    int32_t overlap[3];
    int32_t trim;
} exaspim_window;

int exaspim_abi_version(void);
const char* exaspim_last_error(void);


size_t exaspim_unet_param_count(const int32_t channels[5], int32_t out_channels,
                                int32_t dtype);

size_t exaspim_unet_packed_bytes(const int32_t channels[5], int32_t out_channels,
                                 int32_t dtype);

int exaspim_unet_pack_weights(const int32_t channels[5], int32_t out_channels,
                              int32_t dtype, const float* params, size_t n_params,
                              void* packed_host, size_t packed_bytes);

int exaspim_unet_create(const int32_t channels[5], int32_t out_channels,
                        int32_t dtype, int32_t device, const void* packed_dev,
                        size_t packed_bytes, exaspim_unet** out);
void exaspim_unet_destroy(exaspim_unet* h);

size_t exaspim_unet_workspace_bytes(const exaspim_unet* h, int32_t n, int32_t d,
                                    int32_t hgt, int32_t w);

int exaspim_unet_forward(exaspim_unet* h, const float* x_dev, float* out_dev,
                         int32_t n, int32_t d, int32_t hgt, int32_t w,
                         int32_t apply_sigmoid, void* workspace_dev,
                         size_t workspace_bytes, void* stream);

int exaspim_unet_forward_trimmed(exaspim_unet* h, const float* x_dev, float* out_dev,
                                 int32_t n, int32_t d, int32_t hgt, int32_t w,
                                 int32_t apply_sigmoid, int32_t trim, void* workspace_dev,
                                 size_t workspace_bytes, void* stream);

int exaspim_unet_input_layout(const exaspim_unet* h);
int exaspim_unet_forward_prepared(exaspim_unet* h, const void* x_prepared_dev, float* out_dev,
                                  int32_t n, int32_t d, int32_t hgt, int32_t w,
                                  int32_t apply_sigmoid, int32_t trim, void* workspace_dev,
                                  size_t workspace_bytes, void* stream);
int exaspim_unet_forward_prepared_row(exaspim_unet* h, const void* x_prepared_dev, float* out_dev,
                                      int32_t n, int32_t d, int32_t hgt, int32_t w,
                                      int32_t apply_sigmoid, int32_t trim, int32_t row_stride,
                                      void* workspace_dev, size_t workspace_bytes, void* stream);
int exaspim_unet_forward_prepared_clipped(exaspim_unet* h, const void* x_prepared_dev, float* out_dev,
                                          int32_t n, int32_t d, int32_t hgt, int32_t w,
                                          int32_t apply_sigmoid, int32_t trim, int32_t row_stride,
                                          const int32_t keep_hi[3], void* workspace_dev,
                                          size_t workspace_bytes, void* stream);

int exaspim_unet_carry_planes(const exaspim_unet* h, int32_t n, int32_t d, int32_t hgt, int32_t w,
                              int32_t row_stride, int32_t shift_z, int32_t out[2]);
typedef struct exaspim_unet_carry {
    void* own_skip;
    void* own_pool;
    int32_t in_z[2];
    void* out_skip;
    void* out_pool;
    int32_t out_z[2];
    int32_t out_shift;
    int32_t reserved;
} exaspim_unet_carry;
int exaspim_unet_forward_prepared_carry(exaspim_unet* h, const void* x_prepared_dev, float* out_dev,
                                        int32_t n, int32_t d, int32_t hgt, int32_t w,
                                        int32_t apply_sigmoid, int32_t trim, int32_t row_stride,
                                        const int32_t keep_hi[3], const exaspim_unet_carry* carry,
                                        void* workspace_dev, size_t workspace_bytes, void* stream);

int exaspim_unet_carry1_planes(const exaspim_unet* h, int32_t n, int32_t d, int32_t hgt, int32_t w,
                               int32_t row_stride, int32_t shift_z, int32_t out[2]);
typedef struct exaspim_unet_carry1 {
    void* own_mid1;
    void* own_skip1;
    void* own_pool2;
    int32_t in_z[2];
    void* out_mid1;
    void* out_skip1;
    void* out_pool2;
    int32_t out_z[2];
    int32_t out_shift;
    int32_t reserved;
} exaspim_unet_carry1;
int exaspim_unet_forward_prepared_carry1(exaspim_unet* h, const void* x_prepared_dev, float* out_dev,
                                         int32_t n, int32_t d, int32_t hgt, int32_t w,
                                         int32_t apply_sigmoid, int32_t trim, int32_t row_stride,
                                         const int32_t keep_hi[3], const exaspim_unet_carry* carry,
                                         const exaspim_unet_carry1* carry1, void* workspace_dev,
                                         size_t workspace_bytes, void* stream);

int exaspim_unet_carry_rows(const exaspim_unet* h, int32_t n, int32_t d, int32_t hgt, int32_t w,
                            int32_t row_stride, int32_t shift_y, int32_t out[2]);
typedef struct exaspim_unet_carry_y {
    int32_t in_y[2];
    void* out_skip_y;
    void* out_pool_y;
    void* out_skip_d;
    void* out_pool_d;
    int32_t out_y[2];
    int32_t out_shift_y;
    int32_t reserved;
    void* encoder_event;
} exaspim_unet_carry_y;
int exaspim_unet_forward_prepared_carry_y(exaspim_unet* h, const void* x_prepared_dev, float* out_dev,
                                          int32_t n, int32_t d, int32_t hgt, int32_t w,
                                          int32_t apply_sigmoid, int32_t trim, int32_t row_stride,
                                          const int32_t keep_hi[3], const exaspim_unet_carry* carry,
                                          const exaspim_unet_carry1* carry1, const exaspim_unet_carry_y* carry_y,
                                          void* workspace_dev, size_t workspace_bytes, void* stream);

#define EXASPIM_ABSMAX_SLOTS 22
int exaspim_unet_forward_absmax(exaspim_unet* h, const float* x_dev, float* out_dev,
                                int32_t n, int32_t d, int32_t hgt, int32_t w,
                                int32_t apply_sigmoid, float* absmax_dev, void* workspace_dev,
                                size_t workspace_bytes, void* stream);

#define EXASPIM_OPT_SEPARATE_POOL 1u
#define EXASPIM_OPT_SEPARATE_DEEP_POOLS 2u
#define EXASPIM_OPT_PLAIN_UPSAMPLE 4u
#define EXASPIM_OPT_FIRST_PER_GROUP 8u
#define EXASPIM_OPT_UPSAMPLE_PER_THREAD 16u
#define EXASPIM_OPT_PER_PATCH_ENCODER 32u
#define EXASPIM_OPT_SEPARATE_HEAD 64u
#define EXASPIM_OPT_ROW_SEPARATE_BORDERS 256u
#define EXASPIM_OPT_CARRY_MAIN_ONLY 512u
#define EXASPIM_OPT_CARRY_NO_ROWS 2048u
int exaspim_unet_set_options(exaspim_unet* h, uint32_t options);

int exaspim_unet_timing_begin(exaspim_unet* h, uint32_t conv_mask);
int exaspim_unet_timing_read(exaspim_unet* h, double ms_sum[17], int32_t count[17]);


int exaspim_histogram(const void* vol_dev, int32_t vox_dtype, size_t n,
                      double clip, int32_t has_clip, int32_t pass,
                      uint32_t prefix, uint64_t* hist_dev, void* stream);

int exaspim_histogram_wide(const void* vol_dev, int32_t vox_dtype, size_t n,
                           double clip, int32_t has_clip, int32_t pass,
                           uint64_t prefix, uint64_t* hist_dev, void* stream);

#define EXASPIM_IN_F32 0
#define EXASPIM_IN_PADDED_F32 1
#define EXASPIM_IN_PADDED_SPLIT_F16 2
#define EXASPIM_IN_PADDED_SPLIT_BF16 3
int exaspim_gather_patches_as(const void* vol_dev, int32_t vox_dtype,
                              const exaspim_block* blk, const int32_t* starts_dev,
                              int32_t n, const int32_t patch[3], double clip,
                              int32_t has_clip, double mn, double denom, int32_t layout,
                              void* out_dev, void* stream);
int exaspim_gather_patches(const void* vol_dev, int32_t vox_dtype,
                           const exaspim_block* blk, const int32_t* starts_dev,
                           int32_t n, const int32_t patch[3], double clip,
                           int32_t has_clip, double mn, double denom,
                           float* out_dev, void* stream);


int exaspim_stitch_accumulate(const float* pred_dev, const int32_t* starts_dev,
                              int32_t n, int32_t channels,
                              const exaspim_window* win, float* accum_dev,
                              const exaspim_block* blk, void* stream);

int exaspim_stitch_finalize(float* accum_dev, int32_t channels,
                            const exaspim_window* win, const exaspim_block* blk,
                            void* stream);

int exaspim_export_f16(const float* src_dev, void* dst_dev, size_t n, void* stream);


#define EXASPIM_AFF_F32 0
#define EXASPIM_AFF_F16 1

size_t exaspim_components_workspace_bytes(const int32_t dims[3]);

int exaspim_components(const void* aff_dev, int32_t aff_dtype, int32_t channels,
                       const int32_t dims[3], float threshold, int64_t min_size,
                       int32_t* labels_dev, int32_t* n_segments_dev, void* workspace_dev,
                       size_t workspace_bytes, void* stream);

typedef struct exaspim_components_stream {
    int32_t dims[3];
    int32_t channels;
    float threshold;
    int32_t capacity;
    int64_t min_size;
    int32_t next_z;
    int32_t reserved;
    int32_t* id_parent_dev;
    int64_t* id_count_dev;
    int32_t* table_dev;
    int32_t* state_dev;
    int32_t* seam_ids_dev;
    uint8_t* seam_bits_dev;
} exaspim_components_stream;

size_t exaspim_components_stream_slab_workspace_bytes(const int32_t slab_dims[3]);

size_t exaspim_components_stream_finish_workspace_bytes(int32_t capacity);

int exaspim_components_stream_slab(exaspim_components_stream* st, const void* aff_dev, int32_t aff_dtype,
                                   const int32_t slab_dims[3], int32_t z0, int32_t* labels_dev,
                                   void* workspace_dev, size_t workspace_bytes, void* stream);

int exaspim_components_stream_finish(const exaspim_components_stream* st, void* workspace_dev,
                                     size_t workspace_bytes, void* stream);

int exaspim_components_stream_apply(const exaspim_components_stream* st, int32_t* labels_dev, size_t n,
                                    void* stream);


size_t exaspim_region_graph_workspace_bytes(const int32_t dims[3], int32_t n_labels, int64_t edge_capacity);

int exaspim_region_graph(const int32_t* labels_dev, const void* aff_dev, int32_t aff_dtype,
                         const int32_t dims[3], int32_t n_labels, int64_t edge_capacity,
                         int32_t* edges_dev, int64_t* count_dev, uint64_t* sum_dev, int64_t* sizes_dev,
                         int32_t* n_edges_dev, void* workspace_dev, size_t workspace_bytes, void* stream);

typedef struct exaspim_region_graph_stream {
    int32_t dims[3];
    int32_t id_capacity;
    int64_t edge_capacity;
    int32_t next_z;
    int32_t reserved;
    uint64_t* keys_dev;
    uint64_t* counts_dev;
    uint64_t* sums_dev;
    int64_t* sizes_by_id_dev;
    int32_t* seam_ids_dev;
    uint32_t* seam_q_dev;
    int32_t* state_dev;
} exaspim_region_graph_stream;

int exaspim_region_graph_stream_slab(exaspim_region_graph_stream* st, const int32_t* labels_dev,
                                     const void* aff_dev, int32_t aff_dtype, const int32_t slab_dims[3],
                                     int32_t z0, void* stream);

size_t exaspim_region_graph_stream_finish_workspace_bytes(int64_t edge_capacity);

int exaspim_region_graph_stream_finish(const exaspim_region_graph_stream* st, const int32_t* table_dev,
                                       int32_t table_len, int32_t n_labels, int32_t* edges_dev,
                                       int64_t* count_dev, uint64_t* sum_dev, int64_t* sizes_dev,
                                       int32_t* n_edges_dev, void* workspace_dev, size_t workspace_bytes,
                                       void* stream);

int exaspim_agglomerate(const int32_t* edges, const int64_t* counts, const uint64_t* sums, int64_t n_edges,
                        const int64_t* sizes, int32_t n_labels, float threshold, int64_t min_size,
                        int32_t* table, int32_t* n_segments);

int exaspim_apply_label_table(int32_t* labels_dev, size_t n, const int32_t* table_dev, int32_t table_len,
                              void* stream);


size_t exaspim_watershed_workspace_bytes(const int32_t dims[3]);

int exaspim_watershed_fragments(const void* aff_dev, int32_t aff_dtype, const int32_t dims[3],
                                float low, float high, int64_t min_size,
                                int32_t* labels_dev, int32_t* n_fragments_dev,
                                void* workspace_dev, size_t workspace_bytes, void* stream);


size_t exaspim_region_graph_premerge_workspace_bytes(int32_t n_labels, int64_t edge_capacity);

int exaspim_region_graph_premerge(const int32_t* edges_dev, const int64_t* count_dev, const uint64_t* sum_dev,
                                  const int64_t* sizes_dev, int64_t n_edges, int32_t n_labels,
                                  float threshold, int64_t size_floor, int64_t edge_capacity,
                                  int32_t* edges_out_dev, int64_t* count_out_dev, uint64_t* sum_out_dev,
                                  int64_t* sizes_out_dev, int32_t* map_dev, int32_t* state_dev,
                                  void* workspace_dev, size_t workspace_bytes, void* stream);


size_t exaspim_region_graph_contract_dominant_workspace_bytes(int32_t n_labels, int64_t edge_capacity);

int exaspim_region_graph_contract_dominant(const int32_t* edges_dev, const int64_t* count_dev,
                                           const uint64_t* sum_dev, const int64_t* sizes_dev, int64_t n_edges,
                                           int32_t n_labels, float threshold, int64_t edge_capacity,
                                           int32_t* edges_out_dev, int64_t* count_out_dev, uint64_t* sum_out_dev,
                                           int64_t* sizes_out_dev, int32_t* map_dev, int32_t* state_dev,
                                           void* workspace_dev, size_t workspace_bytes, void* stream);

#define EXASPIM_DBF_INF 2147483647
// ... 90 lines not shown
```

Baseline: 865.7 million voxels/s.

## Write shared overlap columns of the first layer once and redirect reads to owner

In row/carry mode, the first conv layer's output for overlap columns shared between neighbouring patches is now stored only by an owning patch (owner_only flag in the y-carry). The skip-connection consumer conv (last-but-one layer) gets new owner-read kernels (zpipe_own and t14_own variants) that redirect loads for those columns to the neighbouring patch's buffer. This removes duplicate stores of shared halo data. The cost is extra address arithmetic and cross-patch buffer resources in the decoder conv. An option bit restores the old behaviour.

```diff
diff --git a/aind_exaspim_neuron_segmentation_amd/_native.py b/aind_exaspim_neuron_segmentation_amd/_native.py
--- a/aind_exaspim_neuron_segmentation_amd/_native.py
+++ b/aind_exaspim_neuron_segmentation_amd/_native.py
@@ -17,6 +17,7 @@
 OPT_ROW_SEPARATE_BORDERS = 256
 OPT_CARRY_MAIN_ONLY = 512
 OPT_CARRY_NO_ROWS = 2048
+OPT_SHARED_TWICE = 4096
 AFF_F32, AFF_F16 = 0, 1
 
 DTYPE_CODES = {
diff --git a/aind_exaspim_neuron_segmentation_amd/csrc/common.h b/aind_exaspim_neuron_segmentation_amd/csrc/common.h
--- a/aind_exaspim_neuron_segmentation_amd/csrc/common.h
+++ b/aind_exaspim_neuron_segmentation_amd/csrc/common.h
@@ -206,9 +206,12 @@
     unsigned short in_y0 = 0, in_y1 = 0;
     unsigned short out_y0 = 0, out_y1 = 0;
     unsigned short out_shift_y = 0;
-};
+    unsigned short owner_only = 0;
+};
+static_assert(sizeof(ConvCarryY) == 48, "ConvCarryY: the owner flag fills padding");
 inline bool conv_has_carry_y(const ConvCarryY& y) {
-    return y.y_dst || y.y_pool_dst || y.d_dst || y.d_pool_dst || y.in_y0 || y.in_y1 || y.out_y0 || y.out_y1 || y.out_shift_y;
+    return y.y_dst || y.y_pool_dst || y.d_dst || y.d_pool_dst || y.in_y0 || y.in_y1 || y.out_y0 || y.out_y1 || y.out_shift_y ||
+           y.owner_only;
 }
 
 struct ConvLaunchRecord {
@@ -217,6 +220,7 @@
     bool row = false;
     bool carry_y = false;
     bool carry = false;
+    bool owner = false;
 };
 ConvLaunchRecord& last_conv_launch();
 const char*& last_layer_kernel();
@@ -236,6 +240,9 @@
 constexpr int kRowStageBordersCarry = 16;
 constexpr int kRowStagesCarry = kRowStageMain | kRowStageBordersCarry;
 int launch_conv3x3x3_row(int dtype, const ConvArgs& a, int stages, hipStream_t stream, const ConvCarryY* y = nullptr);
+bool conv_shared_once_owner(int n, int w, int row_stride, int p, int x, int* owner_p, int* owner_x);
+bool conv_shared_once_ok(int dtype, int n, int d, int h, int w, int row_stride, int ca, int cout);
+int launch_conv3x3x3_owner(int dtype, const ConvArgs& a, int row_stride, bool thin, hipStream_t stream);
 int conv_zcol_tile_depth(int d);
 int conv_row_borders_tile_depth(int d);
 constexpr int kCarryT14TZ = 4;
diff --git a/aind_exaspim_neuron_segmentation_amd/csrc/conv3d.hip b/aind_exaspim_neuron_segmentation_amd/csrc/conv3d.hip
--- a/aind_exaspim_neuron_segmentation_amd/csrc/conv3d.hip
+++ b/aind_exaspim_neuron_segmentation_amd/csrc/conv3d.hip
@@ -122,7 +122,41 @@
     last_conv_launch() = {__PRETTY_FUNCTION__, 1};
     last_conv_launch().carry = true;
     last_conv_launch().carry_y = true;
+    last_conv_launch().owner = y.owner_only != 0;
     conv3x3x3_zpipe_rowzy<Tag, TZ, TY, TX, MINW, D><<<grid, TY * TX * 2, 0, stream>>>(a, y, g.tz, g.ty, g.tx);
+    EXA_CHECK_HIP(hipGetLastError());
+    return EXASPIM_OK;
+}
+
+template <typename Tag, int TZ>
+static int launch_zpipe_own(const ConvArgs& a, int own_stride, hipStream_t stream) {
+    constexpr int TY = 8, TX = 16, MINW = 2, D = 4;
+    TileGrid g;
+    if (int rc = tile_grid(a, TZ, TY, TX, a.ext[2], a.n, g)) return rc;
+    const int slices = a.cout / 32;
+    long long wgs = resident_workgroups(MINW) / slices / 8 * 8;
+    if (wgs < 8) wgs = 8;
+    if (wgs > g.blocks) wgs = g.blocks;
+    dim3 grid((unsigned)wgs, slices);
+    last_conv_launch() = {__PRETTY_FUNCTION__, 1};
+    last_conv_launch().owner = true;
+    conv3x3x3_zpipe_own<Tag, TZ, TY, TX, MINW, D><<<grid, TY * TX * 2, 0, stream>>>(a, own_stride, g.tz, g.ty, g.tx);
+    EXA_CHECK_HIP(hipGetLastError());
+    return EXASPIM_OK;
+}
+
+template <typename Tag, int TZ, int TY, int TX, int WAVES_M, int WAVES_N, int MT, int NT, int MINW>
+static int launch_cfg_own(const ConvArgs& a, int own_stride, hipStream_t stream) {
+    static_assert(WAVES_N * NT == 1, "32-cout slices");
+    TileGrid g;
+    if (int rc = tile_grid(a, TZ, TY, TX, a.ext[2], a.n, g)) return rc;
+    ConvArgs b = a;
+    b.ksplit = 1;
+    dim3 grid((unsigned)g.blocks, a.cout / 32, 1);
+    last_conv_launch() = {__PRETTY_FUNCTION__, 1};
+    last_conv_launch().owner = true;
+    conv3x3x3_t14_own<Tag, TZ, TY, TX, WAVES_M, WAVES_N, MT, NT, MINW, 3, true>
+        <<<grid, WAVES_M * WAVES_N * 64, 0, stream>>>(b, own_stride, g.tz, g.ty, g.tx);
     EXA_CHECK_HIP(hipGetLastError());
     return EXASPIM_OK;
 }
@@ -362,6 +396,30 @@
            w % 16 == 0 && n >= 2 && row_stride > 0 && o > 0 && o % 32 == 0 && row_stride >= o;
 }
 
+bool conv_shared_once_ok(int dtype, int n, int d, int h, int w, int row_stride, int ca, int cout) {
+    if (dtype != EXASPIM_DT_F16 && dtype != EXASPIM_DT_BF16) return false;
+    if (d <= 0 || h <= 0 || ca < 32 || ca % 16 != 0 || cout <= 0 || cout % 32 != 0 || cout % 64 == 0) return false;
+    if (!conv_row_mode_ok(dtype, ca, n, w, row_stride, true)) return false;
+    if (!conv_shared_once_owner(n, w, row_stride, 0, 0, nullptr, nullptr)) return false;
+    return (unsigned long long)n * d * h * w * ca * 2 < 0x80000000ULL;
+}
+
+bool conv_shared_once_owner(int n, int w, int row_stride, int p, int x, int* owner_p, int* owner_x) {
+    if (owner_p) *owner_p = p;
+    if (owner_x) *owner_x = x;
+    const int s = row_stride, o = w - s, ho = o / 2;
+    if (!(w > 0 && w % 16 == 0 && n >= 2 && s > 0 && o > 0 && o % 32 == 0 && s >= o)) return false;
+    if (p < 0 || p >= n || x < 0 || x >= w) return false;
+    if (p > 0 && x >= 2 && x < ho) {
+        if (owner_p) *owner_p = p - 1;
+        if (owner_x) *owner_x = x + s;
+    } else if (p < n - 1 && x >= s + ho && x < w - 2) {
+        if (owner_p) *owner_p = p + 1;
+        if (owner_x) *owner_x = x - s;
+    }
+    return true;
+}
+
 static int check_row_args(int dtype, const ConvArgs& a) {
     const bool whole = a.ext[0] == a.d && a.ext[1] == a.h && a.ext[2] == a.w;
     EXA_CHECK_ARG(conv_row_mode_ok(dtype, a.cout, a.n, a.w, a.row_stride,
@@ -515,6 +573,39 @@
     return EXASPIM_E_INVALID;
 }
 
+template <typename Tag>
+static int launch_owner_typed(const ConvArgs& a, int own_stride, bool thin, hipStream_t stream) {
+    if (!thin)
+        return conv_zcol_tile_depth(a.d) == 6 ? launch_zpipe_own<Tag, 6>(a, own_stride, stream)
+                                              : launch_zpipe_own<Tag, 4>(a, own_stride, stream);
+    const int ez = a.ext[0];
+    auto planes = [&](int tz) { return (ez + tz - 1) / tz * tz; };
+    if (a.ext[1] <= a.ext[2]) {
+        const float c4 = planes(4) * 1.00f, c8 = planes(8) * 0.76f, c12 = planes(12) * 0.66f;
+        if (c12 <= c8 && c12 <= c4) return launch_cfg_own<Tag, 12, 2, 16, 4, 1, 3, 1, 3>(a, own_stride, stream);
+        if (c8 <= c4) return launch_cfg_own<Tag, 8, 2, 16, 4, 1, 2, 1, 4>(a, own_stride, stream);
+        return launch_cfg_own<Tag, 4, 2, 16, 4, 1, 1, 1, 4>(a, own_stride, stream);
+    }
+    if (planes(8) * 0.78f <= planes(4) * 1.00f) return launch_cfg_own<Tag, 8, 16, 2, 4, 1, 2, 1, 4>(a, own_stride, stream);
+    return launch_cfg_own<Tag, 4, 16, 2, 4, 1, 1, 1, 4>(a, own_stride, stream);
+}
+
+int launch_conv3x3x3_owner(int dtype, const ConvArgs& a_in, int row_stride, bool thin, hipStream_t stream) {
+    ConvArgs a = a_in;
+    if (int rc = check_conv_args(dtype, a, thin ? kCheckPadded | kCheckEmpty : kCheckAll)) return rc;
+    EXA_CHECK_ARG(!a.pool_dst && !a.head_out && a.row_stride == 0 && !conv_has_carry(a),
+                  "conv: owner reads have no fused pool, head, row mode or carried planes");
+    EXA_CHECK_ARG(conv_shared_once_ok(dtype, a.n, a.d, a.h, a.w, row_stride, a.ca, a.cout),
+                  "conv: owner reads need a 16-bit 32-cout-slice layer on 16-wide rows, a row geometry row mode accepts "
+                  "and a batch of source A below 2 GiB (w %d, stride %d, n %d, %d -> %d channels)",
+                  a.w, row_stride, a.n, a.ca, a.cout);
+    if (int rc = resolve_region(a)) return rc;
+    a.partial = nullptr;
+    a.ksplit = 1;
+    return dtype == EXASPIM_DT_F16 ? launch_owner_typed<F16Tag>(a, row_stride, thin, stream)
+                                   : launch_owner_typed<BF16Tag>(a, row_stride, thin, stream);
+}
+
 template <typename Tag, int TZ, int MT>
 static int launch_row_borders_cfg(const ConvArgs& a, hipStream_t stream) {
     const int tz = cdiv(a.d, TZ), ty = cdiv(a.h, 16);
diff --git a/aind_exaspim_neuron_segmentation_amd/csrc/conv_t14.h b/aind_exaspim_neuron_segmentation_amd/csrc/conv_t14.h
--- a/aind_exaspim_neuron_segmentation_amd/csrc/conv_t14.h
+++ b/aind_exaspim_neuron_segmentation_amd/csrc/conv_t14.h
@@ -8,14 +8,24 @@
           bool ZORD = false, bool POOL = false>
 __global__ __launch_bounds__(WAVES_M* WAVES_N * 64, MINW) void conv3x3x3_t14(
     ConvArgs a, int tiles_z, int tiles_y, int tiles_x) {
-    constexpr bool CARRY = false;
+    constexpr bool CARRY = false, OWN = false;
+    constexpr int own_stride = 0;
+#include "conv_t14_body.inc"
+}
+
+template <typename Tag, int TZ, int TY, int TX, int WAVES_M, int WAVES_N, int MT, int NT, int MINW, int PD,
+          bool ZORD = false>
+__global__ __launch_bounds__(WAVES_M* WAVES_N * 64, MINW) void conv3x3x3_t14_own(
+    ConvArgs a, int own_stride, int tiles_z, int tiles_y, int tiles_x) {
+    constexpr bool CARRY = false, OWN = true, POOL = false;
 #include "conv_t14_body.inc"
 }
 
 template <typename Tag, int TZ, int TY, int TX, int WAVES_M, int WAVES_N, int MT, int NT, int MINW, int PD, bool POOL>
 __global__ __launch_bounds__(WAVES_M* WAVES_N * 64, MINW) void conv3x3x3_t14_carry(
     ConvArgs a, int tiles_z, int tiles_y, int tiles_x) {
-    constexpr bool ZORD = false, CARRY = true;
+    constexpr bool ZORD = false, CARRY = true, OWN = false;
+    constexpr int own_stride = 0;
 #include "conv_t14_body.inc"
 }
 
@@ -23,7 +33,8 @@
 __global__ __launch_bounds__(256, 4) void conv3x3x3_t14_borders_carry(
     ConvArgs a, int tiles_z, int tiles_y, int tiles_x) {
     constexpr int TY = 16, TX = 2, WAVES_M = 4, WAVES_N = 1, NT = 1, PD = 3;
-    constexpr bool ZORD = true, POOL = true, CARRY = true;
+    constexpr bool ZORD = true, POOL = true, CARRY = true, OWN = false;
+    constexpr int own_stride = 0;
 #include "conv_t14_body.inc"
 }
 
diff --git a/aind_exaspim_neuron_segmentation_amd/csrc/conv_t14_body.inc b/aind_exaspim_neuron_segmentation_amd/csrc/conv_t14_body.inc
--- a/aind_exaspim_neuron_segmentation_amd/csrc/conv_t14_body.inc
+++ b/aind_exaspim_neuron_segmentation_amd/csrc/conv_t14_body.inc
@@ -75,6 +75,17 @@
                         (unsigned)gy < (unsigned)a.h && (unsigned)gx < (unsigned)a.w;
         voffs[it] = ok ? (unsigned)((gz * a.h + gy) * a.w + gx) * 32u + (i & 1) * 16u : kOutOfRange;
     }
+    unsigned own_code = 0;
+    if constexpr (OWN) {
+        static_assert(NITEMS <= 16, "two bits per staged piece");
+        const int ho = (a.w - own_stride) >> 1;
+#pragma unroll
+        for (int it = 0; it < NITEMS; ++it) {
+            const int gx = x0 + ((tid + it * NTHREADS) >> 1) % HX - 1;
+            const unsigned code = nb > 0 && gx >= 2 && gx < ho ? 1u : nb + 1 < a.n && gx >= own_stride + ho && gx < a.w - 2 ? 2u : 0u;
+            own_code |= code << (2 * it);
+        }
+    }
 
     f32x16 acc[MT][NT];
 #pragma unroll
@@ -106,6 +117,19 @@
         const size_t patchb = patch_vox * cs * ES;
         const __amdgpu_buffer_rsrc_t rsrc = make_rsrc(src + (size_t)nb * patchb, patchb);
         const unsigned cbase = (unsigned)(ch0 / KC) * (unsigned)patch_vox * 32u;
+        if constexpr (OWN) {
+            if (c * KC < a.ca) {
+                const __amdgpu_buffer_rsrc_t brsrc = make_rsrc(src, (size_t)a.n * patchb);
+                const unsigned own = (unsigned)nb * (unsigned)patchb, dist = (unsigned)patchb - (unsigned)own_stride * 32u;
+#pragma unroll
+                for (int it = 0; it < NITEMS; ++it) {
+                    const unsigned code = (own_code >> (2 * it)) & 3u;
+                    const unsigned sh = own + (code == 1u ? 0u - dist : code == 2u ? dist : 0u);
+                    stg[it] = buf_load16(brsrc, voffs[it] == kOutOfRange ? kOutOfRange : voffs[it] + sh, cbase);
+                }
+                return;
+            }
+        }
 #pragma unroll
         for (int it = 0; it < NITEMS; ++it) stg[it] = buf_load16(rsrc, voffs[it], cbase);
     };
diff --git a/aind_exaspim_neuron_segmentation_amd/csrc/conv_zcol.h b/aind_exaspim_neuron_segmentation_amd/csrc/conv_zcol.h
--- a/aind_exaspim_neuron_segmentation_amd/csrc/conv_zcol.h
+++ b/aind_exaspim_neuron_segmentation_amd/csrc/conv_zcol.h
@@ -5,9 +5,9 @@
 namespace exaspim {
 
 template <typename Tag, int TZ, int TY, int TX, int MINW, int D, int HEAD, bool POOL, bool ROW, bool CARRY = false,
-          bool CARRYY = false>
+          bool CARRYY = false, bool OWN = false>
 __device__ __forceinline__ void zpipe_body(const ConvArgs& a, int tiles_z, int tiles_y, int tiles_x,
-                                           const ConvCarryY& cy = ConvCarryY{}) {
+                                           const ConvCarryY& cy = ConvCarryY{}, int own_stride = 0) {
     constexpr int G = Tag::kG;
     constexpr int KC = 2 * G;
     constexpr int ES = 16 / G;
@@ -48,6 +48,7 @@
     static_assert(!ROW || (POOL && ES == 2 && HEAD == 0), "row mode: 16-bit fused-pool epilogue");
     static_assert(!CARRY || ROW, "carry: row mode only");
     static_assert(!CARRYY || (CARRY && TY % 2 == 0 && TX == 16), "y carry: on top of the z carry, a wave owns a row pair");
+    static_assert(!OWN || (!ROW && !POOL && HEAD == 0 && ES == 2), "owner reads: the plain 16-bit per-patch instantiation");
     const int total = tiles_z * tiles_y * tiles_x * (row ? 1 : a.n);
     int t_first, t_count, t_step;
     {
@@ -112,7 +113,28 @@
         const int c = pr >> 1, kg = pr & 1;
         s_slot[k] = q < REM * HZ ? kg * GS + hz * PLANE + (c / HX) * HXP + c % HX : -1;
     }
-    auto set_offsets = [&](const Tile& t) {
+    const unsigned own_patchb = OWN ? (unsigned)(patch_vox * a.ca * ES) : 0u;
+    auto own_shift = [&](int nb, int gx) {
+        const int ho = (a.w - own_stride) >> 1;
+        const unsigned dist = own_patchb - (unsigned)own_stride * 32u;
+        const unsigned sh = nb > 0 && gx >= 2 && gx < ho                          ? 0u - dist
+                            : nb + 1 < a.n && gx >= own_stride + ho && gx < a.w - 2 ? dist
+                                                                                    : 0u;
+        return (unsigned)nb * own_patchb + sh;
+    };
+    auto own_to_b = [&](int nb) {
+        const unsigned base = (unsigned)nb * own_patchb, mid = (unsigned)patch_vox * 32u;
+        const unsigned dist = own_patchb - (unsigned)own_stride * 32u;
+        auto to_b = [&](unsigned v) {
+            const int t = (int)(v - base);
+            const unsigned b = t < 0 ? (unsigned)t + dist : (unsigned)t >= mid ? (unsigned)t - dist : (unsigned)t;
+            return v == kOutOfRange ? v : b;
+        };
+        p_voff = to_b(p_voff);
+#pragma unroll
+        for (int k = 0; k < SEC; ++k) s_voff[k] = to_b(s_voff[k]);
+    };
+    auto set_offsets = [&](const Tile& t, bool own_a = false) {
         if constexpr (CARRY) {
             const int ft = wave * 64 + fresh_lane();
             const int gy = t.y0 + (ft >> 1) / HX - 1, gx = t.x0 + (ft >> 1) % HX - 1;
@@ -122,6 +144,9 @@
             const int gy = t.y0 + p_hy - 1, gx = t.x0 + p_hx - 1;
             const bool in = p_ok && (unsigned)gy < (unsigned)a.h && (unsigned)gx < (unsigned)a.w;
             p_voff = in ? (unsigned)(gy * a.w + gx) * 32u + p_kg * 16u : kOutOfRange;
+            if constexpr (OWN) {
+                if (in && own_a) p_voff += own_shift(t.nb, gx);
+            }
         }
 #pragma unroll
         for (int k = 0; k < SEC; ++k) {
@@ -132,6 +157,9 @@
             const bool in = q < REM * HZ && (unsigned)gz < (unsigned)a.d &&
                             (unsigned)gy < (unsigned)a.h && (unsigned)gx < (unsigned)a.w;
             s_voff[k] = in ? (unsigned)((gz * a.h + gy) * a.w + gx) * 32u + kg * 16u : kOutOfRange;
+            if constexpr (OWN) {
+                if (in && own_a) s_voff[k] += own_shift(t.nb, gx);
+            }
         }
     };
     const unsigned wvoff = (((tid >> 6) * ntiles) * 64 + (tid & 63)) * 16u;
@@ -163,6 +191,11 @@
             src = static_cast<const char*>(a.src_b); cs = a.cb; ch0 = c * KC - a.ca;
         }
         const size_t patchb = patch_vox * cs * ES;
+        if constexpr (OWN) {
+            if (c * KC < a.ca)
+                return ChunkSrc{make_rsrc(src, (size_t)a.n * patchb), make_rsrc(src, 0),
+                                (unsigned)(ch0 / KC) * (unsigned)patch_vox * 32u};
+        }
         return ChunkSrc{make_rsrc(src + (size_t)nb * patchb, patchb), make_rsrc(src + (size_t)nb * patchb, 0),
                         (unsigned)(ch0 / KC) * (unsigned)patch_vox * 32u};
     };
@@ -201,7 +234,7 @@
 
     int tile_id = t_first;
     Tile cur = tile_at(tile_id);
-    set_offsets(cur);
+    set_offsets(cur, true);
     {
         const ChunkSrc cs0 = chunk_src(0, cur.nb);
 #pragma unroll
@@ -241,7 +274,10 @@
             const bool pre = more || has_next;
             if (!more && has_next) {
                 nxt = tile_at(tile_id + t_step);
-                set_offsets(nxt);
+                set_offsets(nxt, true);
+            }
+            if constexpr (OWN) {
+                if (more && (c + 1) * KC == a.ca) own_to_b(cur.nb);
             }
             const ChunkSrc csn = chunk_src(more ? c + 1 : 0, more ? cur.nb : nxt.nb);
             const int cn = more ? c + 1 : 0, zn = more ? cur.z0 : nxt.z0;
@@ -376,6 +412,8 @@
             const bool nnext = row && cur.x0 >= rs && cur.x0 < rs + rho && cur.nb + 1 < a.n;
             const bool nprev = row && cur.x0 >= rho && cur.x0 < 2 * rho && cur.nb >= 1;
             const bool shared = nnext || nprev;
+            bool shared_x1 = shared;
+            if constexpr (CARRYY) shared_x1 = shared && !cy.owner_only;
             const int nshift = nnext ? -rs : nprev ? rs : 0;
             const int nnb = cur.nb + (nnext ? 1 : nprev ? -1 : 0);
             const int ngx = gx + nshift;
@@ -424,13 +462,13 @@
                     for (int ck = 0; ck < 2; ++ck) {
                         const uint4 rec = record_half(grp[zz][2 * ck], grp[zz][2 * ck + 1]);
                         buf_store16(rec, orsrc, ovoff, ((unsigned)ck * (unsigned)patch_vox + (unsigned)gz * (unsigned)plane_vox) * 32u);
-                        if (shared)
+                        if (shared_x1)
                             buf_store16(rec, nrsrc, nlane ? ovoff : kOutOfRange, ((unsigned)ck * (unsigned)patch_vox + (unsigned)gz * (unsigned)plane_vox) * 32u);
                         if (CARRY && cout_on) {
                             const bool cz = gz >= a.out_z0 && gz < a.out_z1;
                             buf_store16(rec, make_rsrc(cplane, cz ? (size_t)2 * patch_vox * 32 : (size_t)0), ovoff,
                                         ((unsigned)ck * (unsigned)patch_vox + (unsigned)gz * (unsigned)plane_vox) * 32u);
-                            if (shared)
+                            if (shared_x1)
                                 buf_store16(rec, make_rsrc(cnplane, cz ? nbytes : (size_t)0), nlane ? ovoff : kOutOfRange,
                                             ((unsigned)ck * (unsigned)patch_vox + (unsigned)gz * (unsigned)plane_vox) * 32u);
                         }
@@ -439,7 +477,7 @@
                             const size_t poff = ((size_t)cur.nb * (a.cout / KC) + ntile0 * 2) * patch_vox * 32;
                             buf_store16(rec, make_rsrc(static_cast<char*>(cy.y_dst) - yshift + poff, yz ? (size_t)2 * patch_vox * 32 : (size_t)0),
                                         ovoff, ((unsigned)ck * (unsigned)patch_vox + (unsigned)gz * (unsigned)plane_vox) * 32u);
-                            if (shared) {
+                            if (shared_x1) {
                                 const size_t npoff = ((size_t)nnb * (a.cout / KC) + ntile0 * 2) * patch_vox * 32;
                                 buf_store16(rec, make_rsrc(static_cast<char*>(cy.y_dst) - yshift + nbase + npoff, yz ? nbytes : (size_t)0),
                                             nlane ? ovoff : kOutOfRange,
@@ -451,7 +489,7 @@
                             const size_t poff = ((size_t)cur.nb * (a.cout / KC) + ntile0 * 2) * patch_vox * 32;
                             buf_store16(rec, make_rsrc(static_cast<char*>(cy.d_dst) - cshift - yshift + poff, dz ? (size_t)2 * patch_vox * 32 : (size_t)0),
                                         ovoff, ((unsigned)ck * (unsigned)patch_vox + (unsigned)gz * (unsigned)plane_vox) * 32u);
-                            if (shared) {
+                            if (shared_x1) {
                                 const size_t npoff = ((size_t)nnb * (a.cout / KC) + ntile0 * 2) * patch_vox * 32;
                                 buf_store16(rec, make_rsrc(static_cast<char*>(cy.d_dst) - cshift - yshift + nbase + npoff, dz ? nbytes : (size_t)0),
                                             nlane ? ovoff : kOutOfRange,
@@ -651,4 +689,11 @@
     zpipe_body<Tag, TZ, TY, TX, MINW, D, 0, true, true, true, true>(a, tiles_z, tiles_y, tiles_x, cy);
 }
 
+template <typename Tag, int TZ, int TY, int TX, int MINW, int D>
+__global__ __launch_bounds__(TY* TX * 2, MINW) void conv3x3x3_zpipe_own(
+    ConvArgs a, int own_stride, int tiles_z, int tiles_y, int tiles_x) {
+    zpipe_body<Tag, TZ, TY, TX, MINW, D, 0, false, false, false, false, true>(a, tiles_z, tiles_y, tiles_x, ConvCarryY{},
+                                                                              own_stride);
 }
+
+}
diff --git a/aind_exaspim_neuron_segmentation_amd/csrc/engine.hip b/aind_exaspim_neuron_segmentation_amd/csrc/engine.hip
--- a/aind_exaspim_neuron_segmentation_amd/csrc/engine.hip
+++ b/aind_exaspim_neuron_segmentation_amd/csrc/engine.hip
@@ -227,6 +227,10 @@
             }
         }
     }
+    const ConvLayer& up40 = p.conv[kNumMfmaConvs - 2];
+    const bool shared_once = carry && row && !(e->options & EXASPIM_OPT_SHARED_TWICE) && up40.ca == p.conv[0].cout &&
+                             conv_shared_once_ok(dt, n, d, h, w, row_stride, up40.ca, up40.cout);
+    if (shared_once) cy.owner_only = 1;
     const bool carry_borders = carry && !(e->options & (EXASPIM_OPT_CARRY_MAIN_ONLY | EXASPIM_OPT_ROW_SEPARATE_BORDERS));
     int32_t first_skip[2] = {0, 0};
     if (carry_borders) conv_first_skip_planes(d, carry->in_z[0], carry->in_z[1], first_skip);
@@ -326,7 +330,9 @@
             slot = t->next;
             EXA_CHECK_HIP(hipEventRecord(t->start[slot], stream));
         }
+        const bool owner_reads = last_but_one && shared_once;
         int r = x3 && has_head      ? launch_conv3x3x3_x3_head(a, stream)
+                : owner_reads      ? launch_conv3x3x3_owner(dt, a, row_stride, false, stream)
                 : a.row_stride > 0 ? launch_conv3x3x3_row(dt, a, (e->options & EXASPIM_OPT_ROW_SEPARATE_BORDERS) ? kRowStagesAll
                                                                  : carry_borders ? kRowStagesCarry : kRowStagesFused, stream,
                                                         idx == 0 ? &cy : nullptr)
@@ -341,12 +347,12 @@
             ConvArgs b = a;
             b.org[1] = a.org[1] + a.ext[1]; b.ext[1] = rem_y;
             b.ext[2] = a.ext[2] + rem_x;
-            r = launch_conv3x3x3_thin(dt, b, stream);
+            r = owner_reads ? launch_conv3x3x3_owner(dt, b, row_stride, true, stream) : launch_conv3x3x3_thin(dt, b, stream);
         }
         if (r == EXASPIM_OK && rem_x > 0) {
             ConvArgs b = a;
             b.org[2] = a.org[2] + a.ext[2]; b.ext[2] = rem_x;
-            r = launch_conv3x3x3_thin(dt, b, stream);
+            r = owner_reads ? launch_conv3x3x3_owner(dt, b, row_stride, true, stream) : launch_conv3x3x3_thin(dt, b, stream);
         }
         if (r == EXASPIM_OK && absmax)
             r = launch_absmax(dt, dst, (size_t)n * (d >> l) * (h >> l) * (w >> l) * L.cout * dtype_size(dt),
@@ -721,7 +727,7 @@
     EXA_CHECK_ARG((options & ~(uint32_t)(EXASPIM_OPT_SEPARATE_POOL | EXASPIM_OPT_SEPARATE_DEEP_POOLS | EXASPIM_OPT_PLAIN_UPSAMPLE | EXASPIM_OPT_FIRST_PER_GROUP |
                                           EXASPIM_OPT_UPSAMPLE_PER_THREAD | EXASPIM_OPT_PER_PATCH_ENCODER |
                                           EXASPIM_OPT_SEPARATE_HEAD | EXASPIM_OPT_ROW_SEPARATE_BORDERS |
-                                          EXASPIM_OPT_CARRY_MAIN_ONLY | EXASPIM_OPT_CARRY_NO_ROWS)) == 0,
+                                          EXASPIM_OPT_CARRY_MAIN_ONLY | EXASPIM_OPT_CARRY_NO_ROWS | EXASPIM_OPT_SHARED_TWICE)) == 0,
                   "set_options: unknown option bits 0x%x", options);
     h->options = options;
     return EXASPIM_OK;
diff --git a/aind_exaspim_neuron_segmentation_amd/csrc/layer_probe.hip b/aind_exaspim_neuron_segmentation_amd/csrc/layer_probe.hip
--- a/aind_exaspim_neuron_segmentation_amd/csrc/layer_probe.hip
+++ b/aind_exaspim_neuron_segmentation_amd/csrc/layer_probe.hip
@@ -180,6 +180,85 @@
 }
 int probe_last_carry_y(void) { return last_conv_launch().carry_y ? 1 : 0; }
 
+int probe_conv3x3x3_row_owner(int dtype, const void* src, int ca, const void* weights, const float* bias, void* dst,
+                              int cout, int n, int d, int h, int w, float slope, int row_stride, void* pool_dst,
+                              const int32_t* carry, void* carry_dst, void* carry_pool_dst, const int32_t* carry_y,
+                              void* const* targets, int owner_only, int stages, hipStream_t stream) {
+    EXA_CHECK_ARG(carry != nullptr && carry_y != nullptr && targets != nullptr, "probe: NULL carry");
+    for (int i = 0; i < 5; ++i) {
+        EXA_CHECK_ARG(carry[i] >= 0 && carry[i] <= (i == 2 || i == 3 ? 254 : 65534), "probe: carry[%d] = %d out of range", i, carry[i]);
+        EXA_CHECK_ARG(carry_y[i] >= 0 && carry_y[i] <= 65534, "probe: carry_y[%d] = %d out of range", i, carry_y[i]);
+    }
+    ConvArgs a{};
+    a.src_a = src;
+    a.ca = ca;
+    a.weights = weights;
+    a.bias = bias;
+    a.dst = dst;
+    a.cout = cout;
+    a.n = n;
+    a.d = d;
+    a.h = h;
+    a.w = w;
+    a.slope = slope;
+    a.row_stride = row_stride;
+    a.pool_dst = pool_dst;
+    a.in_z0 = (unsigned short)carry[0];
+    a.in_z1 = (unsigned short)carry[1];
+    a.out_z0 = (unsigned char)carry[2];
+    a.out_z1 = (unsigned char)carry[3];
+    a.out_shift = (unsigned short)carry[4];
+    a.carry_dst = carry_dst;
+    a.carry_pool_dst = carry_pool_dst;
+    ConvCarryY y;
+    y.in_y0 = (unsigned short)carry_y[0];
+    y.in_y1 = (unsigned short)carry_y[1];
+    y.out_y0 = (unsigned short)carry_y[2];
+    y.out_y1 = (unsigned short)carry_y[3];
+    y.out_shift_y = (unsigned short)carry_y[4];
+    y.y_dst = targets[0];
+    y.y_pool_dst = targets[1];
+    y.d_dst = targets[2];
+    y.d_pool_dst = targets[3];
+    y.owner_only = owner_only ? 1 : 0;
+    return launch_conv3x3x3_row(dtype, a, stages, stream, &y);
+}
+int probe_last_owner(void) { return last_conv_launch().owner ? 1 : 0; }
+
+int probe_conv3x3x3_owner(int thin, int dtype, const void* src_a, const void* src_b, int ca, int cb,
+                          const void* weights, const float* bias, void* dst, int cout, int n, int d, int h, int w,
+                          float slope, const int32_t* region, int row_stride, hipStream_t stream) {
+    ConvArgs a{};
+    a.src_a = src_a;
+    a.src_b = src_b;
+    a.ca = ca;
+    a.cb = cb;
+    a.weights = weights;
+    a.bias = bias;
+    a.dst = dst;
+    a.cout = cout;
+    a.n = n;
+    a.d = d;
+    a.h = h;
+    a.w = w;
+    a.slope = slope;
+    for (int i = 0; i < 3; ++i) {
+        a.org[i] = region ? region[i] : 0;
+        a.ext[i] = region ? region[3 + i] : 0;
+    }
+    return launch_conv3x3x3_owner(dtype, a, row_stride, thin != 0, stream);
+}
+int probe_shared_once_owner(int n, int w, int row_stride, int p, int x, int32_t* out) {
+    int op = 0, ox = 0;
+    const bool ok = conv_shared_once_owner(n, w, row_stride, p, x, &op, &ox);
+    out[0] = op;
+    out[1] = ox;
+    return ok ? 1 : 0;
+}
+int probe_shared_once_ok(int dtype, int n, int d, int h, int w, int row_stride, int ca, int cout) {
+    return conv_shared_once_ok(dtype, n, d, h, w, row_stride, ca, cout) ? 1 : 0;
+}
+
 int probe_conv3x3x3_carry(int dtype, const void* src, int ca, const void* weights, const float* bias, void* dst,
                           int cout, int n, int d, int h, int w, float slope, void* pool_dst, float* partial,
                           size_t partial_patch_bytes, const int32_t* carry, void* carry_dst, void* carry_pool_dst,
diff --git a/include/exaspim_affinity.h b/include/exaspim_affinity.h
--- a/include/exaspim_affinity.h
+++ b/include/exaspim_affinity.h
@@ -164,6 +164,7 @@
 #define EXASPIM_OPT_ROW_SEPARATE_BORDERS 256u
 #define EXASPIM_OPT_CARRY_MAIN_ONLY 512u
 #define EXASPIM_OPT_CARRY_NO_ROWS 2048u
+#define EXASPIM_OPT_SHARED_TWICE 4096u
 int exaspim_unet_set_options(exaspim_unet* h, uint32_t options);
 
 int exaspim_unet_timing_begin(exaspim_unet* h, uint32_t conv_mask);
```

Result: no change. 871.4 million voxels/s (median of 6 runs) (+0.7%).
